# KittyMac/ponyc

Hardware: AMD Instinct MI355X
Metric: actor msgs/sec (node), message-ubench & ring (higher is better)
Workload: dtype u64; 1 GPU; message-ubench C2: 1,048,576 pingers per GPU x 5 initial pings, steady state; actors_per_gpu=1048576, actors_total=1048576, initial_pings=5, mailbox_cap=16, batch=100, parallelism=actor partition id % 1 over 1 rank(s), exchange=none

## Files before the change

### ponyc_amd/csrc/engine.hip

```cpp
#include <hip/hip_runtime.h>
#include <hip/hip_ext.h>
#include <hipcub/hipcub.hpp>
#include <rccl/rccl.h>

#include <algorithm>
#include <cstdio>
#include <cstdlib>
#include <cstring>
#include <atomic>
#include <condition_variable>
#include <map>
#include <mutex>
#include <new>
#include <thread>
#include <vector>

#include "../../include/gpu_actor_host.h"
#include "engine_dev.h"
#include "zone_dev.h"
#include "sparse_dev.h"
#include "hot_dev.h"
#include "step_entry.h"
#include "jit_host.h"
#include "dev_buf.h"
// ... 102 lines not shown

__global__ void __launch_bounds__(kLandThreads) k_spawn_land(const uint64_t* key, const uint64_t* arg,
  uint32_t n, const uint32_t* tstart, const unsigned long long* live, uint32_t cur)
{
  __shared__ uint32_t s_hist[kMaxZones];
  __shared__ uint32_t s_base[kMaxZones];
  LandRec r[kLandPer];
#pragma unroll
  for(int u = 0; u < kLandPer; ++u)
  {
    const uint64_t i = (uint64_t)blockIdx.x * kLandRecs + (uint64_t)u * kLandThreads + threadIdx.x;
    r[u].valid = false;
    if(i < n)
    {
      const uint64_t k = key[i];
      const uint32_t t = (uint32_t)(k >> 52);
      const TypeDev& T = c_types[t];
      const uint64_t slot = live[t] + (i - tstart[t]);
      if(slot < T.count)
      {
        r[u].valid = c_eng.nranks == 1 || (T.first + slot) % c_eng.nranks == c_eng.rank;
        r[u].to = T.first + (uint32_t)slot;
        r[u].w = (uint32_t)(((k >> 4) & 0xFFFFull) << 16) | (uint32_t)((k & 0xFu) << 12);
        r[u].from = (uint32_t)(k >> 20);
        r[u].arg = arg[i];
      }
      else if(c_eng.rank == 0)
        atomicAdd(&c_eng.stats[ST_DROPPED], 1ull);
    }
  }
  land_records(r, cur, s_hist, s_base);
}

__global__ void k_spawn_commit(const uint32_t* tcnt, unsigned long long* live)
{
  const uint32_t t = threadIdx.x;
  if(t >= GPU_ACTOR_MAX_TYPES || tcnt[t] == 0) return;
  const unsigned long long room = c_types[t].count - live[t];
  live[t] += tcnt[t] < room ? tcnt[t] : room;
}

__global__ void k_host_begin(uint64_t* step_word, uint64_t v)
{
  *step_word = v;
}

struct HostOff { uint32_t off[kHostShards + 1]; };
__global__ void __launch_bounds__(kBlock) k_host_compact(const uint64_t* key, HostOff o, uint32_t seg,
  uint64_t* key_out, uint32_t* idx_out)
{
  const uint32_t i = blockIdx.x * kBlock + threadIdx.x;
  if(i >= o.off[kHostShards]) return;
  uint32_t lo = 0, hi = kHostShards - 1;
  while(lo < hi)
  {
    const uint32_t mid = (lo + hi + 1) / 2;
    if(o.off[mid] <= i) lo = mid; else hi = mid - 1;
  }
  const uint32_t at = lo * seg + (i - o.off[lo]);
  key_out[i] = key[at];
  idx_out[i] = at;
}

__global__ void __launch_bounds__(kBlock) k_host_gather(const uint64_t* key, const uint32_t* idx,
  const uint4* rec, gpu_host_msg_t* out, uint32_t n, uint64_t base, uint32_t kshift)
{
  const uint32_t i = blockIdx.x * kBlock + threadIdx.x;
  if(i >= n) return;
  const uint64_t k = key[i];
  const uint4 r = rec[idx[i]];
  const uint64_t step = base + (k >> kshift);
  const uint32_t from = (uint32_t)((k & ((1ull << kshift) - 1ull)) >> 16);
  uint4* o = reinterpret_cast<uint4*>(out + i);
  o[0] = make_uint4((uint32_t)step, (uint32_t)(step >> 32), from, (uint32_t)(k & 0xFFFFull));
  o[1] = r;
}
static_assert(sizeof(gpu_host_msg_t) == 32, "gpu_host_msg_t is 32 B");

__global__ void k_host_lost(unsigned long long n)
{
  c_eng.stats[ST_DROPPED] += n;
}

__global__ void __launch_bounds__(kBlock) k_spill_need(const SpillRec* s, uint32_t n, uint32_t* need)
{
  const uint32_t i = blockIdx.x * kBlock + threadIdx.x;
  if(i >= n) return;
  atomicMax(&need[s[i].z], (s[i].tag & kSpillPosMask) + 1u);
}

__global__ void __launch_bounds__(kBlock) k_spill_place(const SpillRec* s, uint32_t n, uint32_t p)
{
  const uint32_t i = blockIdx.x * kBlock + threadIdx.x;
  if(i >= n) return;
  const SpillRec r = s[i];
  ZRec* base = (r.tag & kSpillCarry) ? c_eng.carry[p] : c_eng.land[p];
  base[c_eng.zoff[r.z] + (r.tag & kSpillPosMask)] = r.rec;
}

constexpr uint32_t kBigCopyCap = 4096;
constexpr uint32_t kBigCopyBlocks = 512;
__global__ void __launch_bounds__(kBlock) k_carry_big(uint32_t cur)
{
  const bool halt_now = c_eng.nranks == 1 ? (c_eng.spill_n[cur] != 0u || *c_eng.halt != 0u)
                                          : (*c_eng.spill_flag != 0u);
  if(halt_now) return;
  const unsigned long long v = c_eng.bigc_n[cur];
  const uint32_t n = min((uint32_t)(v >> 32), c_eng.bigc_cap);
  if(n == 0) return;
  const uint32_t total = c_eng.bigc[n - 1].base + c_eng.bigc[n - 1].rem;
  const uint32_t per = (total + gridDim.x - 1) / gridDim.x;
  const uint32_t c0 = blockIdx.x * per, c1 = min(c0 + per, total);
  if(c0 < c1)
  {
    uint32_t lo = 0, hi = n - 1;
    while(lo < hi)
    {
      const uint32_t mid = (lo + hi + 1) / 2;
      if(c_eng.bigc[mid].base <= c0) lo = mid; else hi = mid - 1;
    }
    for(uint32_t d = lo; d < n; ++d)
    {
      const BigCopy b = c_eng.bigc[d];
      if(b.base >= c1) break;
      const uint32_t j0 = c0 > b.base ? c0 - b.base : 0u;
      const uint32_t j1 = min(c1 - b.base, b.rem);
      for(uint32_t j = j0 + threadIdx.x; j < j1; j += kBlock)
      {
        const uint32_t k = b.from + j;
        const uint32_t q = k - b.ncc;
        const uint4 r = k < b.ncc ? *reinterpret_cast<const uint4*>(b.c + k)
                      : *reinterpret_cast<const uint4*>(b.p + (b.perm ? (uint32_t)(b.perm[q] & 0xFFFFFull) : q));
        *reinterpret_cast<uint4*>(b.dst + j) = r;
      }
    }
  }
}


namespace {

constexpr uint32_t kChunk = 16;
constexpr uint32_t kPendSlots = 4096;
constexpr uint32_t kPendPre = kPendSlots - 1;

struct HostType {
  bool registered = false, created = false;
  uint32_t words = 0, ht = 0, batch = 0, cap = 0;
  uint64_t params[GPU_ACTOR_MAX_PARAMS] = {};
  uint64_t first = 0, count = 0;
  uint32_t lfirst = 0, lcount = 0;
  uint64_t reserve = 0;
  int32_t priority = 0;
  DevBuf<uint64_t> d_state;
  DevBuf<uint64_t> d_prog;
  uint32_t prog_n = 0;
  bool prog_yields = false;
  std::vector<uint64_t> prog_host;
};

struct SpillStat {
  unsigned int spill_n[2];
  unsigned int halt;
  unsigned int pad;
  unsigned long long skipped;
};

struct HotLayout {
  size_t prep = 0;
  size_t slot = prep + kMaxZones;
  size_t cnt = slot + kMaxZones;
  size_t aux = cnt + (size_t)kMaxHot * kHotActors;
  size_t hist = aux + (size_t)kMaxHot * 3 * kHotActors;
  size_t bcnt = hist + kHotBins;
  size_t cur = bcnt + kHotBins;
  size_t bar = cur + kHotBins + kHotActors;
  size_t words = bar + 64;
};
constexpr HotLayout kHotLayout{};

struct Process {
  std::mutex mu;
  std::mutex wmu;
  std::thread worker;
  std::vector<std::thread> detached;
  std::atomic<bool> async_busy{false};
  std::atomic<bool> async_started{false};
  int async_rc = 0;
  uint64_t async_steps = 0;
  gpu_actor_alltoallv_fn xp_a2a = nullptr;
  gpu_actor_allreduce_fn xp_ar = nullptr;
  void* xp_ctx = nullptr;
};

struct Session {
  bool init = false;
  gpu_actor_config_t cfg{};
  int device = 0;
  hipStream_t stream = nullptr;
  HostType types[GPU_ACTOR_MAX_TYPES];
  uint32_t n_types = 0;
  uint64_t n_actors = 0;
  uint32_t n_local = 0;
  uint32_t n_zones = 0;
  uint64_t zone_records = 0;
  DevBuf<uint64_t> d_zoff;
  DevBuf<uint32_t> d_zcap;
  DevBuf<ZRec> d_land[2], d_carry[2];
  DevBuf<uint32_t> d_land_n[2], d_carry_n[2];
  DevBuf<ZRec> d_S;
  DevBuf<ORec> d_O;
  uint32_t par = 0;
  DevBuf<unsigned long long> d_stats;
  DevBuf<unsigned long long> d_pend;
  DevBuf<unsigned long long> d_pend_sh;
  DevBuf<unsigned long long> d_stats_sh;
  DevBuf<uint32_t> d_hot;
  bool hot_on = false;
  int hot_fits = -1;
  DevBuf<unsigned long long> d_dbg;
  PinBuf<gpu_msg_t> h_msgs;
  std::vector<gpu_msg_t> deferred;
  DevBuf<gpu_msg_t> d_msgs;
  uint64_t host_seq = 0;
  uint64_t steps_total = 0;
  int sticky = 0;
  jit::Module jit;
  uint64_t jit_set = 0;
  uint64_t jit_failed = 0;
  uint32_t jit_builds = 0;
  bool jit_used = false;
  TypeDev td_host[GPU_ACTOR_MAX_TYPES] = {};
  EngDev eng_host = {};
  bool consts_host = false;
  DevBuf<uint64_t> d_gups_list;
  DevBuf<unsigned int> d_gups_n;
  DevBuf<uint64_t> d_gups_jump;
  DevBuf<unsigned long long> d_gups_stat;
  uint64_t gups_jump_host[65] = {};
  int gups_type = -1;
  DevBuf<uint64_t> d_gups_send;
  DevBuf<uint64_t> d_gups_all;
  uint32_t gups_parts = 0;
  uint64_t gups_in_total = 0, gups_out_total = 0;
  uint64_t dev_epoch = 1, sstat_epoch = 0, sticky_epoch = 0;
  hipError_t last_hip = hipSuccess;
  std::vector<hipEvent_t> ev;
  double last_drain_ms = 0.0;
  ncclComm_t comm = nullptr;
  DevBuf<XRec> d_xout;
  DevBuf<XRec> d_xin;
  DevBuf<unsigned long long> d_xc;
  unsigned long long* d_xcount = nullptr;
  unsigned long long* d_xrecv = nullptr;
  PinBuf<unsigned long long> h_xc;
  DevBuf<unsigned int> d_spill_flag;
  uint32_t xcap = 0;
  DevBuf<XSpillRec> d_xspill;
  DevBuf<unsigned int> d_xspill_n;
  uint32_t xspill_cap = 0;
  std::vector<unsigned long long> h_xcount, h_xrecv;
  uint64_t remote_total = 0;
  bool peer_write = false;
  DevBuf<XRec> d_pin;
  XRec* peer_ptr[kMaxRanks] = {};
  DevBuf<unsigned long long> d_hx;
  PinBuf<uint8_t> h_sbuf, h_rbuf;
  uint32_t spawn_cap = 0;
  DevBuf<uint64_t> d_skey[2], d_sarg[2];
  DevBuf<unsigned int> d_spawn_n;
  DevBuf<uint32_t> d_tstart, d_tcnt;
  DevBuf<unsigned long long> d_live;
  DevBuf<uint8_t> d_sort_tmp;
  DevBuf<uint8_t> d_trig[2], d_trig_own[2];
  uint64_t trig_bytes = 0;
  bool trig_stale[2] = {false, false};
  DevBuf<uint32_t> d_muted_on;
  DevBuf<uint32_t> d_ztrig[2];
  DevBuf<unsigned int> d_trig_n;
  DevBuf<uint32_t> d_zplan;
  bool split_plan = true;
  bool fuse = true;
  uint32_t sidx = 0;
  DevBuf<BigCopy> d_bigc;
  DevBuf<unsigned long long> d_bigc_n;
  bool defer_big = false;
  DevBuf<SpillRec> d_spill[2];
  uint32_t spill_cap = 0;
  DevBuf<SpillStat> d_sstat;
  PinBuf<SpillStat> h_sstat;
  DevBuf<uint32_t> d_need;
  std::vector<uint32_t> zcap_min, zcap_host;
// ... 108 lines not shown
    (void)hipGetLastError();
    cached = 0;
    return false;
  }
  cached = (uint64_t)std::max(per_cu - 1, per_cu > 0 ? 1 : 0) * (uint64_t)cus >= kHotBlocks ? 1 : 0;
  return cached != 0;
}

constexpr uint32_t kGupsBlocks = 1024;
constexpr uint32_t kGupsPackBlocks = 256;
__global__ void __launch_bounds__(256) k_gups_apply();
__global__ void __launch_bounds__(256) k_gups_pack(uint64_t* out, unsigned long long* count);
__global__ void __launch_bounds__(256) k_gups_apply_ranks(const uint64_t* list, uint64_t n,
  uint64_t own_lo, uint64_t own_n);

int gups_setup(EngDev& e)
{
  g.gups_type = -1;
  e.gups_type = -1;
  const char* f = getenv("PONYC_AMD_GUPS_DEFER");
  if(f && atoi(f) == 0) return 0;
  int t_def = -1;
  for(uint32_t t = 0; t < GPU_ACTOR_MAX_TYPES && t_def < 0; ++t)
    if(g.types[t].created && g.types[t].ht == GPU_ACTOR_HT_GUPS_STREAMER && g.types[t].params[0] > 0 &&
       g.types[t].params[0] <= 0xFFFFFFFFull)
      t_def = (int)t;
  if(t_def < 0) return 0;
  const HostType& h = g.types[t_def];
  const uint64_t chunk = h.params[0];
  const uint64_t L = std::max<uint64_t>(16, (chunk + 63) / 64);
  const uint64_t parts = (chunk + L - 1) / L;
  const uint64_t cap = std::min<uint64_t>(std::max<uint64_t>(1ull << 22, 2ull * h.lcount), 1ull << 28);
  if(cap > g.d_gups_list.size())
  {
    HIPCK(hipStreamSynchronize(g.stream));
    HIPCK(g.d_gups_list.alloc(cap));
    g.d_gups_send.reset();
  }
  if(R() > 1 && !g.d_gups_send)
    HIPCK(g.d_gups_send.alloc(g.d_gups_list.size()));
  if(!g.d_gups_n)
  {
    HIPCK(g.d_gups_n.alloc(kGupsShards + 1));
    HIPCK(hipMemsetAsync(g.d_gups_n, 0, (kGupsShards + 1) * sizeof(unsigned int), g.stream));
    HIPCK(g.d_gups_jump.alloc(65));
    HIPCK(g.d_gups_stat.alloc(3 * kGupsBlocks));
    HIPCK(hipMemsetAsync(g.d_gups_stat, 0, 3 * kGupsBlocks * sizeof(unsigned long long), g.stream));
  }
  uint64_t jump[65] = {};
  for(uint64_t p = 0; p < parts; ++p) jump[p] = gpa::polyrand_xpow(p * L);
  jump[parts] = gpa::polyrand_xpow(chunk);
  if(memcmp(jump, g.gups_jump_host, sizeof(jump)) != 0)
  {
    HIPCK(hipStreamSynchronize(g.stream));
    memcpy(g.gups_jump_host, jump, sizeof(jump));
    HIPCK(hipMemcpyAsync(g.d_gups_jump, g.gups_jump_host, sizeof(jump), hipMemcpyHostToDevice,
      g.stream));
  }
  e.gups_list = g.d_gups_list; e.gups_n = g.d_gups_n; e.gups_jump = g.d_gups_jump;
  e.gups_stat = g.d_gups_stat;
  e.gups_seg = (uint32_t)(g.d_gups_list.size() / kGupsShards);
  {
    const char* sg = getenv("PONYC_AMD_GUPS_SEG");
    if(sg && atoi(sg) > 0) e.gups_seg = std::min<uint32_t>(e.gups_seg, (uint32_t)atoi(sg));
  }
  e.gups_l = (uint32_t)L; e.gups_parts = (uint32_t)parts;
  e.gups_type = t_def;
  g.gups_type = t_def;
  g.gups_parts = (uint32_t)parts;
  return 0;
}

int gups_apply_launch(hipEvent_t e1)
{
  if(g.gups_type < 0 || R() > 1) return 0;
  if(e1)
    hipExtLaunchKernelGGL(k_gups_apply, dim3(kGupsBlocks), dim3(256), 0, g.stream, nullptr, e1, 0u);
  else
    hipLaunchKernelGGL(k_gups_apply, dim3(kGupsBlocks), dim3(256), 0, g.stream);
  HIPCK(hipGetLastError());
  return 0;
}

int upload_types()
{
  TypeDev td[GPU_ACTOR_MAX_TYPES];
  memset(td, 0, sizeof(td));
  for(uint32_t t = 0; t < GPU_ACTOR_MAX_TYPES; ++t)
  {
    const HostType& h = g.types[t];
    TypeDev& d = td[t];
    if(!h.created) continue;
    d.first = (uint32_t)h.first; d.count = (uint32_t)h.count;
    d.lfirst = h.lfirst; d.lcount = h.lcount;
    d.ht = h.ht; d.words = h.words; d.batch = h.batch; d.cap = h.cap;
    d.reducible = reducible_ht(h.ht);
    d.prio = h.priority > 0 ? 1u : 0u;
    d.state = h.d_state;
    memcpy(d.params, h.params, sizeof(d.params));
    d.prog = h.d_prog;
    d.prog_n = h.prog_n;
    d.prog_pad = h.prog_yields ? 1u : 0u;
  }
  HIPCK(hipMemcpyToSymbolAsync(HIP_SYMBOL(c_types), td, sizeof(td), 0,
    hipMemcpyHostToDevice, g.stream));
  EngDev e;
  memset(&e, 0, sizeof(e));
  e.n_types = g.n_types; e.rank = rank(); e.nranks = R(); e.n_local = g.n_local;
  e.n_zones = g.n_zones; e.zoff = g.d_zoff; e.zcapz = g.d_zcap;
  e.n_ids = (uint32_t)std::min<uint64_t>(g.n_actors, 0xFFFFFFFFull);
  e.r_magic = R() > 1 ? ~0ull / R() + 1 : 0;
  for(int p = 0; p < 2; ++p)
  {
    e.land[p] = g.d_land[p]; e.carry[p] = g.d_carry[p];
    e.land_n[p] = g.d_land_n[p]; e.carry_n[p] = g.d_carry_n[p];
  }
  e.S = g.d_S; e.O = g.d_O;
  e.stats = g.d_stats; e.pend = g.d_pend;
  e.pend_sh = g.d_pend_sh; e.stats_sh = g.d_stats_sh;
  {
    uint32_t* h = g.d_hot;
    const HotLayout& L = kHotLayout;
    e.hot_prep = h + L.prep; e.hot_slot = h + L.slot; e.hot_cnt = h + L.cnt; e.hot_aux = h + L.aux;
    e.hot_hist = h + L.hist; e.hot_bcnt = h + L.bcnt; e.hot_cur = h + L.cur; e.hot_bar = h + L.bar;
  }
  e.xout = g.d_xout; e.xcount = g.d_xcount; e.xcap = g.xcap;
  e.peer_write = g.peer_write ? 1u : 0u;
  for(uint32_t p = 0; p < R() && p < kMaxRanks; ++p)
    e.xdst[p] = g.peer_write ? (g.peer_ptr[p] ? g.peer_ptr[p] + (size_t)rank() * g.xcap : nullptr)
                             : (g.d_xout ? g.d_xout + (size_t)p * g.xcap : nullptr);
  e.seq_max = R() > 1 ? kXSeqMax : kSeqMax;
  e.dbg = g.d_dbg;
  e.spawn_key = g.d_skey[0]; e.spawn_arg = g.d_sarg[0];
  e.spawn_n = g.d_spawn_n; e.spawn_cap = g.spawn_cap;
  for(int p = 0; p < 2; ++p)
  {
    e.trig[p] = g.d_trig[p];
    e.trig_own[p] = R() > 1 ? g.d_trig_own[p] : g.d_trig[p];
    e.ztrig[p] = g.d_ztrig[p];
  }
  e.muted_on = g.d_muted_on;
  e.spill_flag = g.d_spill_flag;
  e.trig_n = g.d_trig_n;
  e.spill[0] = g.d_spill[0]; e.spill[1] = g.d_spill[1];
  e.spill_n = g.d_sstat ? g.d_sstat->spill_n : nullptr;
  e.halt = g.d_sstat ? &g.d_sstat->halt : nullptr;
  e.skipped = g.d_sstat ? &g.d_sstat->skipped : nullptr;
  e.spill_cap = g.spill_cap;
  e.xspill = g.d_xspill; e.xspill_n = g.d_xspill_n; e.xspill_cap = g.xspill_cap;
  e.zbits = g.zbits;
  g.defer_big = defer_big_wanted();
  {
    const char* f = getenv("PONYC_AMD_HOT");
    g.hot_on = pick_step_entry().hot && (f ? atoi(f) != 0 : g.defer_big) && hot_resident();
    e.hot_on = g.hot_on ? 1u : 0u;
    const char* t = getenv("PONYC_AMD_HOT_TEST");
    e.hot_test = (t && atoi(t) != 0) ? 1u : 0u;
  }
  e.bigc = g.d_bigc; e.bigc_n = g.d_bigc_n; e.bigc_cap = kBigCopyCap;
  e.defer_big = g.defer_big ? 1u : 0u;
  {
    const char* f = getenv("PONYC_AMD_TWO_PASS");
    e.two_pass = (f && atoi(f) == 0) ? 0u : 1u;
    const char* sp = getenv("PONYC_AMD_SPLIT_PLAN");
    g.split_plan = !(sp && atoi(sp) == 0);
    const char* fu = getenv("PONYC_AMD_FUSE");
    g.fuse = !(fu && atoi(fu) == 0);
  }
  e.zplan = g.d_zplan;
  if(g.host_ports && g.host_seg)
  {
    uint64_t lo = ~0ull, hi = 0;
    for(uint32_t t = 0; t < GPU_ACTOR_MAX_TYPES; ++t)
    {
      const HostType& h = g.types[t];
      if(!h.created || h.ht != GPU_ACTOR_HT_HOST_PORT) continue;
      e.host_rng[e.host_nrng].first = (uint32_t)h.first;
      e.host_rng[e.host_nrng].count = (uint32_t)h.count;
      e.host_rng[e.host_nrng].type = t;
      e.host_nrng++;
      lo = std::min(lo, h.first);
      hi = std::max(hi, h.first + h.count);
    }
    e.host_first = e.host_nrng ? (uint32_t)lo : 0u;
    e.host_span = e.host_nrng ? (uint32_t)(hi - lo) : 0u;
    e.host_seg = g.host_seg;
    e.host_key = g.hl.d_host_key; e.host_rec = g.hl.d_host_rec; e.host_n = g.d_host_n;
    e.host_step = g.d_host_step;
  }
  {
    const int rc = gups_setup(e);
    if(rc) return rc;
  }
  HIPCK(hipMemcpyToSymbolAsync(HIP_SYMBOL(c_eng), &e, sizeof(e), 0,
    hipMemcpyHostToDevice, g.stream));
  for(const StepEntry& se : step_entries())
    HIPCK(se.upload(td, &e, g.stream));
  memcpy(g.td_host, td, sizeof(td));
  g.eng_host = e;
  g.consts_host = true;
  if(g.jit.mod)
  {
    HIPCK(hipMemcpyHtoDAsync(g.jit.types, g.td_host, sizeof(g.td_host), g.stream));
    HIPCK(hipMemcpyHtoDAsync(g.jit.eng, &g.eng_host, sizeof(g.eng_host), g.stream));
  }
  return 0;
}

int ensure_spill(uint64_t cap)
{
  cap = std::min<uint64_t>(cap, 0x7FFFFFFFull);
  if(cap <= g.spill_cap) return 0;
  g.spill_cap = 0;
  for(int p = 0; p < 2; ++p) HIPCK(g.d_spill[p].alloc(cap));
  g.spill_cap = (uint32_t)cap;
  return 0;
}

int relayout_zones(bool geometry = false);
StepEntry step_entry_for(bool z12);
bool step_fits(const StepEntry& se, uint64_t nb);
int upload_types();
int pend_read(uint32_t first, uint32_t n, std::vector<unsigned long long>& out);

inline uint64_t spill_cap_for_zones()
{
  return std::max<uint64_t>(1u << 20, g.zone_records / 4);
}

int read_sstat()
{
  HIPCK(hipMemcpyAsync(g.h_sstat, g.d_sstat, sizeof(SpillStat), hipMemcpyDeviceToHost,
    g.stream));
  HIPCK(hipStreamSynchronize(g.stream));
  g.sstat_epoch = g.dev_epoch;
  return 0;
}

inline bool spill_pending()
{
  return g.h_sstat->spill_n[0] || g.h_sstat->spill_n[1] || g.h_sstat->halt;
}

int fixup_spill()
{
  const SpillStat st = *g.h_sstat;
  g.dev_epoch++;
  if(R() == 1 && !st.spill_n[0] && !st.spill_n[1] && !st.halt) return 0;
  uint32_t n[2], most = 0;
  for(int p = 0; p < 2; ++p)
  {
    n[p] = std::min(st.spill_n[p], g.spill_cap);
    most = std::max(most, st.spill_n[p]);
  }
  if(n[0] || n[1])
  {
    const uint32_t nz = g.n_zones;
    HIPCK(hipMemsetAsync(g.d_need, 0, nz * sizeof(uint32_t), g.stream));
    for(int p = 0; p < 2; ++p)
      if(n[p])
        hipLaunchKernelGGL(k_spill_need, dim3(blocks_for(n[p])), dim3(kBlock), 0, g.stream,
          (const SpillRec*)g.d_spill[p], n[p], g.d_need);
    HIPCK(hipGetLastError());
    std::vector<uint32_t> need(nz);
    HIPCK(hipMemcpyAsync(need.data(), g.d_need, nz * sizeof(uint32_t), hipMemcpyDeviceToHost,
      g.stream));
    HIPCK(hipStreamSynchronize(g.stream));
    bool grow = false;
    for(uint32_t z = 0; z < nz; ++z)
      if(need[z] > g.zcap_host[z])
      {
        const uint64_t want = std::max<uint64_t>(2ull * g.zcap_host[z], need[z] + need[z] / 2);
        g.zcap_min[z] = (uint32_t)std::min<uint64_t>((want + 15) & ~15ull, kSpillPosMask);
        grow = true;
      }
    if(grow)
    {
      int rc = relayout_zones();
      if(rc) return rc;
      rc = upload_types();
      if(rc) return rc;
    }
    for(int p = 0; p < 2; ++p)
      if(n[p])
        hipLaunchKernelGGL(k_spill_place, dim3(blocks_for(n[p])), dim3(kBlock), 0, g.stream,
          (const SpillRec*)g.d_spill[p], n[p], (uint32_t)p);
    HIPCK(hipGetLastError());
  }
  HIPCK(hipMemsetAsync(g.d_sstat, 0, sizeof(SpillStat), g.stream));
  HIPCK(hipMemsetAsync(g.d_spill_flag, 0, sizeof(unsigned int), g.stream));
  HIPCK(hipStreamSynchronize(g.stream));
  memset(g.h_sstat, 0, sizeof(SpillStat));
  g.fixups++;
  const uint64_t want = std::max<uint64_t>(spill_cap_for_zones(),
                                           most > g.spill_cap ? 2ull * most : 0ull);
  if(want > g.spill_cap)
  {
    const int rc = ensure_spill(want);
    if(rc) return rc;
    return upload_types();
  }
  return 0;
}

uint32_t pick_zone_bits(uint64_t n)
{
  const uint64_t rb = R() > 1 ? R() : 0;
  const uint64_t nz11 = (n + 2047) / 2048, nz12 = (n + 4095) / 4096;
  if(const char* f = getenv("PONYC_AMD_ZONE_BITS"))
    return atoi(f) == 12 ? 12u : 11u;
  return (nz11 + rb > 640 && step_fits(step_entry_for(true), nz12 + rb)) ? 12u : 11u;
}

bool zones_empty()
{
  if(g.n_zones == 0) return true;
  std::vector<uint32_t> v(g.n_zones);
  for(int p = 0; p < 2; ++p)
    for(const uint32_t* src : {g.d_land_n[p].get(), g.d_carry_n[p].get()})
    {
      if(hipMemcpy(v.data(), src, g.n_zones * sizeof(uint32_t), hipMemcpyDeviceToHost) != hipSuccess)
        return false;
      for(uint32_t x : v)
        if(x) return false;
    }
  return true;
}

int relayout_zones(bool geometry)
{
  bool fresh = false;
  {
    const uint32_t want = pick_zone_bits((g.n_actors + R() - 1) / R());
    if(geometry && want != g.zbits && g.steps_total == 0 && g.sparse_launches == 0)
    {
      HIPCK(hipStreamSynchronize(g.stream));
      bool empty = zones_empty();
      if(R() > 1)
      {
        const unsigned long long mine = empty ? 0ull : 1ull;
        HIPCK(hipMemcpyAsync(g.d_pend + kPendPre, &mine, sizeof(mine), hipMemcpyHostToDevice,
          g.stream));
        std::vector<unsigned long long> pv;
        const int rc = pend_read(kPendPre, 1, pv);
        if(rc) return rc;
        empty = pv[0] == 0;
      }
      if(empty)
      {
        g.zbits = want;
        g.zcap_min.clear();
        fresh = true;
      }
    }
  }
  const uint32_t za = zone_actors();
  const uint32_t nz = (uint32_t)((g.n_local + za - 1) / za);
  if(nz > kMaxZones) return GPU_ACTOR_ERANGE;
  std::vector<uint64_t> cap64(nz, 0);
  for(const HostType& t : g.types)
  {
    if(!t.created || reducible_ht(t.ht)) continue;
    for(uint64_t L = t.lfirst; L < (uint64_t)t.lfirst + t.lcount; )
    {
      const uint64_t z = L / za;
      const uint64_t hi = std::min<uint64_t>((z + 1) * za, (uint64_t)t.lfirst + t.lcount);
      cap64[z] += (hi - L) * t.cap;
      L = hi;
    }
  }
  std::vector<uint32_t> cap(nz);
  std::vector<uint64_t> off(nz);
  uint64_t total = 0;
  if(g.zcap_min.size() < nz) g.zcap_min.resize(nz, 0);
  for(uint32_t z = 0; z < nz; ++z)
  {
    cap64[z] = std::max<uint64_t>(cap64[z], g.zcap_min[z]);
    if(cap64[z] > (uint64_t)kSpillPosMask) return GPU_ACTOR_ERANGE;
    cap[z] = (uint32_t)cap64[z];
    off[z] = total;
    total += (cap[z] + 15u) & ~15u;
  }
  const size_t recs = std::max<uint64_t>(total, 16), nzn = std::max<size_t>(nz, 1);
  DevBuf<uint64_t> d_off;
  DevBuf<uint32_t> d_cap, ln[2], cn[2], mo;
  DevBuf<ZRec> land[2], carry[2], S;
  DevBuf<ORec> O;
  HIPCK(d_off.alloc(nzn));
  HIPCK(d_cap.alloc(nzn));
  HIPCK(hipMemcpyAsync(d_off, off.data(), nz * sizeof(uint64_t), hipMemcpyHostToDevice, g.stream));
  HIPCK(hipMemcpyAsync(d_cap, cap.data(), nz * sizeof(uint32_t), hipMemcpyHostToDevice, g.stream));
  for(int p = 0; p < 2; ++p)
  {
    HIPCK(land[p].alloc(recs));
    HIPCK(carry[p].alloc(recs));
    HIPCK(ln[p].alloc(nzn));
    HIPCK(cn[p].alloc(nzn));
    HIPCK(hipMemsetAsync(ln[p], 0, nzn * sizeof(uint32_t), g.stream));
    HIPCK(hipMemsetAsync(cn[p], 0, nzn * sizeof(uint32_t), g.stream));
    if(g.n_zones && !fresh)
    {
      hipLaunchKernelGGL(k_zone_copy, dim3(g.n_zones), dim3(kBlock), 0, g.stream,
        (const ZRec*)g.d_land[p], g.d_zoff, g.d_zcap, land[p], (const uint64_t*)d_off);
      hipLaunchKernelGGL(k_zone_copy, dim3(g.n_zones), dim3(kBlock), 0, g.stream,
        (const ZRec*)g.d_carry[p], g.d_zoff, g.d_zcap, carry[p], (const uint64_t*)d_off);
      HIPCK(hipGetLastError());
      HIPCK(hipMemcpyAsync(ln[p], g.d_land_n[p], g.n_zones * sizeof(uint32_t),
        hipMemcpyDeviceToDevice, g.stream));
      HIPCK(hipMemcpyAsync(cn[p], g.d_carry_n[p], g.n_zones * sizeof(uint32_t),
        hipMemcpyDeviceToDevice, g.stream));
    }
    HIPCK(hipStreamSynchronize(g.stream));
  }
  HIPCK(S.alloc(3 * recs));
  HIPCK(O.alloc(recs));
  const uint64_t slots = (uint64_t)nz * za;
  if(slots > g.d_muted_on.size())
  {
    HIPCK(mo.alloc(slots));
    HIPCK(hipMemsetAsync(mo, 0, slots * sizeof(uint32_t), g.stream));
    if(g.d_muted_on)
    {
      HIPCK(hipMemcpyAsync(mo, g.d_muted_on, g.d_muted_on.size() * sizeof(uint32_t),
        hipMemcpyDeviceToDevice, g.stream));
      HIPCK(hipStreamSynchronize(g.stream));
    }
    g.d_muted_on.swap(mo);
  }
  for(int p = 0; p < 2; ++p)
  {
    g.d_land[p].swap(land[p]); g.d_carry[p].swap(carry[p]);
    g.d_land_n[p].swap(ln[p]); g.d_carry_n[p].swap(cn[p]);
  }
  g.d_S.swap(S);
  g.d_O.swap(O);
  g.d_zoff.swap(d_off);
  g.d_zcap.swap(d_cap);
  g.zone_records = total;
  g.n_zones = nz;
  g.zcap_host = cap;
  return 0;
}

uint32_t required_words(uint32_t ht)
{
  switch(ht)
  {
    case GPU_ACTOR_HT_RING: return 4;
    case GPU_ACTOR_HT_PINGER: return 3;
    case GPU_ACTOR_HT_PINGER_DET: return 2;
    case GPU_ACTOR_HT_FANIN_SENDER: return 4;
    case GPU_ACTOR_HT_FANIN_ANALYZER: return 2;
    case GPU_ACTOR_HT_GUPS_STREAMER: return 2;
    case GPU_ACTOR_HT_GUPS_UPDATER: return 1;
    case GPU_ACTOR_HT_STORM: return 2;
    case GPU_ACTOR_HT_FIFO_SRC: return 3;
    case GPU_ACTOR_HT_FIFO_SINK: return 11;
    case GPU_ACTOR_HT_SPREADER: return 5;
    case GPU_ACTOR_HT_PROGRAM: return 8;
    case GPU_ACTOR_HT_HOST_PORT: return 1;
    default: return 0;
  }
}

__global__ void __launch_bounds__(kBlock) k_fold(uint32_t first, uint32_t n)
{
  for(uint32_t s = first + threadIdx.x; s < first + n; s += kBlock)
  {
    unsigned long long* sh = c_eng.pend_sh + (size_t)s * kShards;
    unsigned long long v = 0;
    for(uint32_t k = 0; k < kShards; ++k) { v += sh[k]; sh[k] = 0; }
    if(v) c_eng.pend[s] += v;
  }
  for(uint32_t i = threadIdx.x; i < ST_COUNT; i += kBlock)
  {
    unsigned long long* sh = c_eng.stats_sh + (size_t)i * kShards;
    unsigned long long v = 0;
    for(uint32_t k = 0; k < kShards; ++k) { v += sh[k]; sh[k] = 0; }
    if(v) c_eng.stats[i] += v;
  }
}

int fold_counters(uint32_t first, uint32_t n)
{
  hipLaunchKernelGGL(k_fold, dim3(1), dim3(kBlock), 0, g.stream, first, n);
  HIPCK(hipGetLastError());
  return 0;
}

int pend_clear(uint32_t first, uint32_t n)
{
  HIPCK(hipMemsetAsync(g.d_pend + first, 0, n * sizeof(unsigned long long), g.stream));
  HIPCK(hipMemsetAsync(g.d_pend_sh + (size_t)first * kShards, 0,
    (size_t)n * kShards * sizeof(unsigned long long), g.stream));
  return 0;
}

void sticky_from(const unsigned long long* st)
{
  if(st[ST_DROPPED] || st[ST_XCHG_OVERFLOW]) g.sticky = GPU_ACTOR_EMAILBOX;
  else if(st[ST_SEQ_OVERFLOW]) g.sticky = GPU_ACTOR_ERANGE;
}

int check_sticky()
{
  if(R() == 1 && g.sticky_epoch == g.dev_epoch) return g.sticky;
  unsigned long long st[ST_COUNT];
  {
    const int rc = fold_counters(0, 0);
    if(rc) return rc;
  }
  HIPCK(hipMemcpyAsync(st, g.d_stats, sizeof(st), hipMemcpyDeviceToHost, g.stream));
  HIPCK(hipStreamSynchronize(g.stream));
  g.sticky_epoch = g.dev_epoch;
  sticky_from(st);
  return g.sticky;
}

__global__ void k_spill_flag(unsigned int* flag)
{
  *flag = c_eng.spill_n[0] + c_eng.spill_n[1];
}

__global__ void __launch_bounds__(256) k_gups_apply()
{
  __shared__ uint32_t s_pre[kGupsShards + 1];
  if(threadIdx.x < kGupsShards)
  {
    uint32_t c = min(__atomic_load_n(&c_eng.gups_n[threadIdx.x], __ATOMIC_RELAXED), c_eng.gups_seg);
    for(int off = 1; off < (int)kGupsShards; off <<= 1)
    {
      const uint32_t o = __shfl_up(c, off);
      if((int)threadIdx.x >= off) c += o;
    }
    s_pre[threadIdx.x + 1] = c;
    if(threadIdx.x == 0) s_pre[0] = 0;
  }
  __syncthreads();
  const uint32_t n = s_pre[kGupsShards];
  const TypeDev& S = c_types[c_eng.gups_type];
  const uint64_t chunk = S.params[0], shift = S.params[1], mask = S.params[2];
  const uint32_t ubase = (uint32_t)S.params[3];
  const uint32_t L = c_eng.gups_l, parts = c_eng.gups_parts, per_wave = 64u / parts;
  const uint32_t lane = threadIdx.x & 63u, sub = lane / parts, p = lane - sub * parts;
  const uint64_t jump = c_eng.gups_jump[p];
  const uint64_t first = (uint64_t)p * L;
  const uint32_t cnt = first < chunk ? (uint32_t)min<uint64_t>(L, chunk - first) : 0u;
  const uint64_t wave = (uint64_t)blockIdx.x * (blockDim.x >> 6) + (threadIdx.x >> 6);
  const uint64_t waves = (uint64_t)gridDim.x * (blockDim.x >> 6);
  uint32_t u_first = 0, u_count = 0, u_lfirst = 0, u_lcount = 0;
  uint64_t* u_state = nullptr;
  uint64_t u_mask = 0;
  uint32_t made = 0, issued = 0;
  for(uint64_t e0 = wave * per_wave; e0 < n; e0 += waves * per_wave)
  {
    const uint64_t e = e0 + sub;
    const bool live = sub < per_wave && e < n;
    uint64_t v = 0;
    if(live)
    {
      uint32_t lo = 0, hi = kGupsShards;
      while(hi - lo > 1u)
      {
        const uint32_t mid = (lo + hi) >> 1;
        if(s_pre[mid] <= e) lo = mid; else hi = mid;
      }
      v = c_eng.gups_list[(size_t)lo * c_eng.gups_seg + (e - s_pre[lo])];
    }
    if(live && p) v = polyrand_mulmod(v, jump);
    for(uint32_t j = 0; j < L; ++j)
    {
      unsigned long long* w = nullptr;
      if(live && j < cnt)
      {
        (void)polyrand_next(v);
        ++made;
        const uint32_t to = ubase + (uint32_t)((v >> shift) & mask);
        if(to - u_first >= u_count)
        {
          const int t = type_of_global(to);
          if(t >= 0)
          {
            const TypeDev& U = c_types[t];
            u_first = U.first; u_count = U.count; u_lfirst = U.lfirst; u_lcount = U.lcount;
            u_state = U.state; u_mask = U.params[0] - 1;
          }
        }
        if(to - u_first < u_count)
          w = reinterpret_cast<unsigned long long*>(&u_state[(v & u_mask) * u_lcount + (to - u_lfirst)]);
      }
      const uint64_t wa = reinterpret_cast<uint64_t>(w);
      uint64_t left = __ballot(w != nullptr);
      for(int round = 0; round < 2 && left; ++round)
      {
        const uint32_t lead = (uint32_t)__ffsll((long long)left) - 1u;
        const uint64_t lw = __shfl(wa, (int)lead);
        const uint64_t peers = __ballot(((left >> lane) & 1ull) && wa == lw);
        uint64_t r = ((peers >> lane) & 1ull) ? v : 0ull;
        if(__popcll(peers) > 1)
          for(int off = 32; off; off >>= 1) r ^= __shfl_xor(r, off);
        if(lane == lead && r != 0)
        {
          atomicXor(w, (unsigned long long)r);
          ++issued;
// ... 72 lines not shown
  const uint64_t first = (uint64_t)p * L;
  const uint32_t cnt = first < chunk ? (uint32_t)min<uint64_t>(L, chunk - first) : 0u;
  const uint64_t wave = (uint64_t)blockIdx.x * (blockDim.x >> 6) + (threadIdx.x >> 6);
  const uint64_t waves = (uint64_t)gridDim.x * (blockDim.x >> 6);
  uint32_t u_first = 0, u_count = 0, u_lfirst = 0, u_lcount = 0;
  uint64_t* u_state = nullptr;
  uint64_t u_mask = 0;
  uint32_t made = 0, issued = 0, far = 0;
  for(uint64_t e0 = wave * per_wave; e0 < n; e0 += waves * per_wave)
  {
    const uint64_t e = e0 + sub;
    const bool live = sub < per_wave && e < n;
    const uint32_t peer = e - own_lo >= own_n ? 1u : 0u;
    uint64_t v = live ? list[e] : 0ull;
    if(live && p) v = polyrand_mulmod(v, jump);
    for(uint32_t j = 0; j < L; ++j)
    {
      unsigned long long* w = nullptr;
      if(live && j < cnt)
      {
        (void)polyrand_next(v);
        const uint32_t to = ubase + (uint32_t)((v >> shift) & mask);
        if(!is_remote(to))
        {
          ++made;
          far += peer;
          if(to - u_first >= u_count)
          {
            const int t = type_of_global(to);
            if(t >= 0)
            {
              const TypeDev& U = c_types[t];
              u_first = U.first; u_count = U.count; u_lfirst = U.lfirst; u_lcount = U.lcount;
              u_state = U.state; u_mask = U.params[0] - 1;
            }
          }
          if(to - u_first < u_count)
            w = reinterpret_cast<unsigned long long*>(
              &u_state[(v & u_mask) * u_lcount + (rdiv(to) - u_lfirst)]);
        }
      }
      const uint64_t wa = reinterpret_cast<uint64_t>(w);
      uint64_t left = __ballot(w != nullptr);
      for(int round = 0; round < 2 && left; ++round)
      {
        const uint32_t lead = (uint32_t)__ffsll((long long)left) - 1u;
        const uint64_t lw = __shfl(wa, (int)lead);
        const uint64_t peers = __ballot(((left >> lane) & 1ull) && wa == lw);
        uint64_t r = ((peers >> lane) & 1ull) ? v : 0ull;
        if(__popcll(peers) > 1)
          for(int off = 32; off; off >>= 1) r ^= __shfl_xor(r, off);
        if(lane == lead && r != 0)
        {
          atomicXor(w, (unsigned long long)r);
          ++issued;
        }
        left &= ~peers;
      }
      if(((left >> lane) & 1ull) && v != 0)
      {
        atomicXor(w, (unsigned long long)v);
        ++issued;
      }
    }
  }
  __shared__ uint32_t s_sum[3];
  if(threadIdx.x < 3) s_sum[threadIdx.x] = 0;
  __syncthreads();
  if(made) atomicAdd(&s_sum[0], made);
  if(issued) atomicAdd(&s_sum[1], issued);
  if(far) atomicAdd(&s_sum[2], far);
  __syncthreads();
  if(threadIdx.x == 0)
  {
    c_eng.gups_stat[blockIdx.x] += s_sum[0];
    c_eng.gups_stat[kGupsBlocks + blockIdx.x] += s_sum[1];
    c_eng.gups_stat[2 * kGupsBlocks + blockIdx.x] += s_sum[2];
  }
}

__global__ void k_spill_local(unsigned long long* out)
{
  *out = (unsigned long long)c_eng.spill_n[0] + c_eng.spill_n[1] + *c_eng.halt +
         (c_eng.nranks > 1 ? *c_eng.spill_flag : 0u);
}

__global__ void k_xprep()
{
  const unsigned int xs = *c_eng.xspill_n;
  if(xs <= c_eng.xspill_cap) return;
  const uint32_t p = threadIdx.x;
  if(p < c_eng.nranks)
    c_eng.xcount[p] = min(c_eng.xcount[p], (unsigned long long)c_eng.xcap);
  if(p == 0) atomicAdd(&c_eng.stats[ST_XCHG_OVERFLOW], (unsigned long long)c_eng.xspill_cap);
}

__global__ void __launch_bounds__(kBlock) k_xspill_place(uint32_t n)
{
  const uint32_t i = blockIdx.x * kBlock + threadIdx.x;
  if(i >= n) return;
  const XSpillRec r = c_eng.xspill[i];
  xrec_put(c_eng.xdst[r.peer] + r.pos, r.rec);
}

int alloc_xspill(uint32_t cap)
{
  g.xspill_cap = 0;
  HIPCK(g.d_xspill.alloc(cap));
  g.xspill_cap = cap;
  return 0;
}

int peer_room(uint64_t max_send, uint64_t xs);
int exchange_room(uint64_t max_send, uint64_t total_recv, uint64_t xs)
{
  if(g.peer_write) return peer_room(max_send, xs);
  const bool lost = xs > g.xspill_cap;
  if(max_send > g.xcap || lost)
  {
    uint64_t cap = std::max<uint64_t>(2ull * g.xcap, max_send + max_send / 2);
    cap = std::min<uint64_t>((cap + 63) & ~63ull, 0x40000000ull);
    DevBuf<XRec> nx;
    HIPCK(nx.alloc((size_t)R() * cap));
    HIPCK(hipMemcpy2DAsync(nx, cap * sizeof(XRec), g.d_xout, (size_t)g.xcap * sizeof(XRec),
      (size_t)g.xcap * sizeof(XRec), R(), hipMemcpyDeviceToDevice, g.stream));
    HIPCK(hipStreamSynchronize(g.stream));
    g.d_xout = std::move(nx);
    g.xcap = (uint32_t)cap;
    const int rc = upload_types();
    if(rc) return rc;
  }
  if(xs)
  {
    if(!lost)
    {
      hipLaunchKernelGGL(k_xspill_place, dim3(blocks_for(xs)), dim3(kBlock), 0, g.stream,
        (uint32_t)xs);
      HIPCK(hipGetLastError());
    }
    HIPCK(hipMemsetAsync(g.d_xspill_n, 0, sizeof(unsigned int), g.stream));
    if(xs > g.xspill_cap / 2)
    {
      HIPCK(hipStreamSynchronize(g.stream));
      const int rc = alloc_xspill((uint32_t)std::min<uint64_t>(4ull * std::max<uint64_t>(xs,
        g.xspill_cap), 1ull << 27));
      if(rc) return rc;
      const int rc2 = upload_types();
      if(rc2) return rc2;
    }
  }
  if(total_recv > g.d_xin.size())
  {
    const uint64_t cap = std::max<uint64_t>(2ull * g.d_xin.size(), total_recv + total_recv / 2);
    HIPCK(hipStreamSynchronize(g.stream));
    HIPCK(g.d_xin.alloc(cap));
  }
  return 0;
}

enum XcType { XC_U8 = 0, XC_U32 = 1, XC_U64 = 2 };

int stage_room(uint64_t sbytes, uint64_t rbytes)
{
  if(sbytes > g.h_sbuf.size()) HIPCK(g.h_sbuf.alloc(std::max<uint64_t>(sbytes, 2 * g.h_sbuf.size())));
  if(rbytes > g.h_rbuf.size()) HIPCK(g.h_rbuf.alloc(std::max<uint64_t>(rbytes, 2 * g.h_rbuf.size())));
  return 0;
}
// ... 554 lines not shown
  HIPCK(hipMemsetAsync(g.d_host_n, 0, kHostShards * sizeof(unsigned int), g.stream));
  HIPCK(hipStreamSynchronize(g.stream));
  if(g.host_fn)
    g.host_fn(g.host_ctx, g.hl.h_host_out, keep);
  else
  {
    if(g.hostq_head == g.hostq.size()) { g.hostq.clear(); g.hostq_head = 0; }
    try { g.hostq.insert(g.hostq.end(), g.hl.h_host_out.get(), g.hl.h_host_out + keep); }
    catch(...) { return GPU_ACTOR_ENOMEM; }
  }
  return 0;
}

int step_after_launch(uint32_t slot, hipEvent_t e0, hipEvent_t e1);
int jit_ensure(const StepEntry& se)
{
  const char* f = getenv("PONYC_AMD_JIT");
  if((f && atoi(f) == 0) || !g.consts_host) return 0;
  const bool z12 = g.zbits == 12;
  std::vector<jit::Prog> progs;
  uint32_t mask = 0;
  bool all_prog = true;
  for(uint32_t t = 0; t < GPU_ACTOR_MAX_TYPES; ++t)
  {
    const HostType& h = g.types[t];
    if(!h.created || reducible_ht(h.ht)) continue;
    mask |= 1u << h.ht;
    if(h.ht != GPU_ACTOR_HT_PROGRAM || h.prog_host.empty()) all_prog = false;
    else progs.push_back({t, h.prog_host});
  }
  int kind = 0;
  uint64_t want = jit::fnv1a(z12 ? "z12" : "z11");
  if(all_prog && !progs.empty() && g.split_plan)
  {
    kind = 1;
    for(const jit::Prog& p : progs)
      want = jit::fnv1a(std::string(reinterpret_cast<const char*>(p.code.data()), p.code.size() * 8),
                        jit::fnv1a(std::to_string(p.type), want));
  }
  else if(se.kernel == step_entry_for_any(z12).kernel && mask)
  {
    kind = 2;
    want = jit::fnv1a("mix" + std::to_string(mask), want);
  }
  if(!kind) return 0;
  if(g.jit.mod && g.jit_set == want) return kind;
  if(g.jit_failed == want) return 0;
  jit::unload(g.jit);
  hipDeviceProp_t prop;
  if(hipGetDeviceProperties(&prop, g.device) != hipSuccess) { (void)hipGetLastError(); return 0; }
  std::string arch = prop.gcnArchName;
  arch = arch.substr(0, arch.find(':'));
  std::string log;
  const int rc = kind == 1 ? jit::build(progs, z12, arch, g.jit, log)
                           : jit::build_mix(mask, z12, arch, g.jit, log);
  if(getenv("PONYC_AMD_JIT_LOG"))
    fprintf(stderr, "gpu_actor jit: %s %s%s (rc %d) %s\n", kind == 1 ? "programs" : "mix",
            kind == 2 ? ("mask " + std::to_string(mask) + " ").c_str() : "", z12 ? "z12" : "z11", rc,
            log.c_str());
  if(rc != 0)
  {
    g.jit_failed = want;
    return 0;
  }
  g.jit_set = want;
  g.jit_builds++;
  if(hipMemcpyHtoDAsync(g.jit.types, g.td_host, sizeof(g.td_host), g.stream) != hipSuccess ||
     hipMemcpyHtoDAsync(g.jit.eng, &g.eng_host, sizeof(g.eng_host), g.stream) != hipSuccess)
  {
    (void)hipGetLastError();
    jit::unload(g.jit);
    g.jit_failed = want;
    return 0;
  }
  return kind;
}

int launch_step(uint32_t slot, hipEvent_t e0, hipEvent_t e1)
{
  if(g.n_zones == 0) return 0;
  g.dev_epoch++;
  const StepEntry se = pick_step_entry();
  if(se.stub) return GPU_ACTOR_EINVAL;
  const uint64_t nb = g.n_zones + (R() > 1 ? R() : 0);
  if(!step_fits(se, nb)) return GPU_ACTOR_ERANGE;
  const size_t dyn = step_dyn_bytes(se, nb);
  if(g.host_ports)
  {
    if(!g.host_seg) return GPU_ACTOR_ENOMEM;
    if(!g.host_dirty) { g.host_base = g.sidx; g.host_dirty = true; }
    hipLaunchKernelGGL(k_host_begin, dim3(1), dim3(1), 0, g.stream, g.d_host_step,
      (uint64_t)(g.sidx - g.host_base) << g.host_kshift);
    HIPCK(hipGetLastError());
  }
  g.jit_used = false;
  const int jk = jit_ensure(se);
  if(jk && g.jit.static_lds + dyn <= kLdsPerWorkgroup)
  {
    g.jit_used = true;
    uint32_t a_cur = g.par, a_slot = slot, a_sidx = g.sidx;
    void* args[] = {&a_cur, &a_slot, &a_sidx};
    if(e0) HIPCK(hipEventRecord(e0, g.stream));
    if(jk == 2 && g.hot_on)
      hipLaunchKernelGGL(k_hot, dim3(kHotBlocks), dim3(kHotThreads), 5u * zone_actors() * sizeof(uint32_t),
        g.stream, g.par, g.sidx);
    HIPCK(hipModuleLaunchKernel(g.jit.plan, g.n_zones, 1, 1, se.threads, 1, 1, (unsigned)dyn, g.stream,
      args, nullptr));
    if(jk == 1)
      HIPCK(hipModuleLaunchKernel(g.jit.rest, g.n_zones, 1, 1, se.threads, 1, 1, (unsigned)dyn, g.stream,
        args, nullptr));
    if(g.defer_big)
      hipLaunchKernelGGL(k_carry_big, dim3(kBigCopyBlocks), dim3(kBlock), 0, g.stream, g.par);
    const int grc = gups_apply_launch(nullptr);
    if(grc) return grc;
    if(e1 && !(g.gups_type >= 0 && R() > 1)) HIPCK(hipEventRecord(e1, g.stream));
    return step_after_launch(slot, e0, e1);
  }
  const bool fused = se.plan && g.split_plan && g.fuse && se.fused;
  const bool split = se.plan && g.split_plan && !fused;
  step_kernel_t kern = fused ? se.fused : split ? se.plan : se.kernel;
  const size_t hot_lds = 5u * zone_actors() * sizeof(uint32_t);
  if(e0)
  {
    const bool gups = g.gups_type >= 0;
    const bool more = split || g.defer_big || gups;
    if(g.hot_on)
      hipExtLaunchKernelGGL(k_hot, dim3(kHotBlocks), dim3(kHotThreads), (uint32_t)hot_lds, g.stream,
        e0, nullptr, 0u, g.par, g.sidx);
    hipExtLaunchKernelGGL(kern, dim3(g.n_zones), dim3(se.threads), (uint32_t)dyn, g.stream,
      g.hot_on ? nullptr : e0, more ? nullptr : e1, 0u, g.par, slot, g.sidx);
    if(split)
      hipExtLaunchKernelGGL(se.rest, dim3(g.n_zones), dim3(se.threads), (uint32_t)dyn, g.stream,
        nullptr, (g.defer_big || gups) ? nullptr : e1, 0u, g.par, slot, g.sidx);
    if(g.defer_big)
      hipExtLaunchKernelGGL(k_carry_big, dim3(kBigCopyBlocks), dim3(kBlock), 0, g.stream,
        nullptr, gups ? nullptr : e1, 0u, g.par);
    HIPCK(hipGetLastError());
    const int grc = gups_apply_launch(e1);
    if(grc) return grc;
  }
  else
  {
    if(g.hot_on)
      hipLaunchKernelGGL(k_hot, dim3(kHotBlocks), dim3(kHotThreads), hot_lds, g.stream, g.par, g.sidx);
    hipLaunchKernelGGL(kern, dim3(g.n_zones), dim3(se.threads), dyn, g.stream, g.par, slot, g.sidx);
    if(split)
      hipLaunchKernelGGL(se.rest, dim3(g.n_zones), dim3(se.threads), dyn, g.stream, g.par, slot, g.sidx);
    if(g.defer_big)
      hipLaunchKernelGGL(k_carry_big, dim3(kBigCopyBlocks), dim3(kBlock), 0, g.stream, g.par);
    HIPCK(hipGetLastError());
    const int grc = gups_apply_launch(nullptr);
    if(grc) return grc;
  }
  HIPCK(hipGetLastError());
  return step_after_launch(slot, e0, e1);
}

int gups_gather_apply(hipEvent_t e1)
{
  const uint32_t n = R();
  const unsigned long long* cnt = g.h_xc + 2 * n + 3;
  std::vector<uint64_t> off(n);
  uint64_t total = 0;
  for(uint32_t p = 0; p < n; ++p)
  {
    off[p] = total;
// ... 563 lines not shown
  const unsigned long long live_ull = live;
  HIPCK(hipMemcpyAsync(g.d_live + type_id, &live_ull, sizeof(live_ull), hipMemcpyHostToDevice,
    g.stream));
  if(t.reserve)
  {
    HIPCK(hipStreamSynchronize(g.stream));
    const uint32_t cap = g.spawn_cap + (uint32_t)t.reserve;
    for(int p = 0; p < 2; ++p)
    {
      HIPCK(g.d_skey[p].alloc((size_t)cap * R()));
      HIPCK(g.d_sarg[p].alloc((size_t)cap * R()));
    }
    g.spawn_cap = cap;
    rc = upload_types();
    if(rc) return rc;
  }
  HIPCK(hipStreamSynchronize(g.stream));
  if(first_id) *first_id = t.first;
  return 0;
}

GPU_ACTOR_API int gpu_actor_type_reserve(uint32_t type_id, uint64_t n)
{
  std::lock_guard<std::mutex> lk(gp.mu);
  if(!g.init) return GPU_ACTOR_ESTATE;
  if(type_id >= GPU_ACTOR_MAX_TYPES || !g.types[type_id].registered ||
    g.types[type_id].created) return GPU_ACTOR_EINVAL;
  if(n > g.cfg.max_actors) return GPU_ACTOR_ERANGE;
  g.types[type_id].reserve = n;
  return 0;
}

GPU_ACTOR_API int gpu_actor_type_live(uint32_t type_id, uint64_t* live)
{
  std::lock_guard<std::mutex> lk(gp.mu);
  if(!g.init) return GPU_ACTOR_ESTATE;
  if(type_id >= GPU_ACTOR_MAX_TYPES || !live || !g.types[type_id].created)
    return GPU_ACTOR_EINVAL;
  unsigned long long v = 0;
  HIPCK(hipMemcpyAsync(&v, g.d_live + type_id, sizeof(v), hipMemcpyDeviceToHost, g.stream));
  HIPCK(hipStreamSynchronize(g.stream));
  *live = v;
  return 0;
}

GPU_ACTOR_API int gpu_actor_alloc_msgs(uint64_t n, gpu_msg_t** buf)
{
  std::lock_guard<std::mutex> lk(gp.mu);
  if(!g.init) return GPU_ACTOR_ESTATE;
  if(!buf) return GPU_ACTOR_EINVAL;
  if(n > g.h_msgs.size()) HIPCK(g.h_msgs.alloc(n));
  *buf = g.h_msgs;
  return 0;
}

GPU_ACTOR_API int gpu_actor_sendv(const gpu_msg_t* first, uint64_t n)
{
  std::lock_guard<std::mutex> lk(gp.mu);
  if(!g.init) return GPU_ACTOR_ESTATE;
  return sendv_locked(first, n);
}

GPU_ACTOR_API int gpu_actor_send(uint64_t to, uint32_t behaviour, uint64_t arg)
{
  std::lock_guard<std::mutex> lk(gp.mu);
  if(!g.init) return GPU_ACTOR_ESTATE;
  gpu_msg_t m;
  m.to = (uint32_t)to; m.behaviour = behaviour; m.arg = arg;
  if(to >= g.n_actors || !host_msg_ok(m)) return GPU_ACTOR_EINVAL;
  if(g.host_seq + g.deferred.size() + 1 >= (1ull << 40)) return GPU_ACTOR_ERANGE;
  try { g.deferred.push_back(m); } catch(...) { return GPU_ACTOR_ENOMEM; }
  return 0;
}

bool sparse_ok()
{
  const char* e = getenv("GPA_NO_SPARSE");
  return !(e && atoi(e) != 0) && R() == 1 && g.spawn_cap == 0 && g.n_zones > 0 && !g.host_ports;
}

int run_sparse(uint64_t max_steps, SparseCtl& out)
{
  g.dev_epoch++;
  bool prog = false, gups = false;
  for(const HostType& t : g.types)
  {
    prog |= t.created && t.ht == GPU_ACTOR_HT_PROGRAM;
    gups |= t.created && t.ht == GPU_ACTOR_HT_GUPS_STREAMER;
  }
#define GPA_SPARSE_LAUNCH(P, G)                                                         \
  hipLaunchKernelGGL((k_sparse<P, G>), dim3(1), dim3(kSpThreads), 0, g.stream, g.par,   \
    (unsigned long long)max_steps, g.d_ctl, g.sidx)
  if(prog && gups) GPA_SPARSE_LAUNCH(true, true);
  else if(prog) GPA_SPARSE_LAUNCH(true, false);
  else if(gups) GPA_SPARSE_LAUNCH(false, true);
  else GPA_SPARSE_LAUNCH(false, false);
#undef GPA_SPARSE_LAUNCH
  HIPCK(hipGetLastError());
  {
    const int rc = gups_apply_launch(nullptr);
    if(rc) return rc;
  }
  HIPCK(hipMemcpyAsync(g.h_ctl, g.d_ctl, sizeof(SparseCtl), hipMemcpyDeviceToHost, g.stream));
  HIPCK(hipMemcpyAsync(g.h_sstat, g.d_sstat, sizeof(SpillStat), hipMemcpyDeviceToHost,
    g.stream));
  HIPCK(hipStreamSynchronize(g.stream));
  out = *g.h_ctl;
  g.par = out.par;
  g.sidx += (uint32_t)out.steps;
  g.sparse_launches++;
  g.sparse_steps += out.steps;
  return 0;
}

int pending_now(unsigned long long& out)
{
  int rc = pend_clear(kPendPre, 1);
  if(rc) return rc;
  rc = launch_pending(kPendPre);
  if(rc) return rc;
  std::vector<unsigned long long> pv;
  rc = pend_read(kPendPre, 1, pv);
  if(rc) return rc;
  out = pv[0];
  return 0;
}

int settle_spills()
{
  if(R() == 1)
  {
    if(g.sstat_epoch == g.dev_epoch) return spill_pending() ? fixup_spill() : 0;
    const int rc = read_sstat();
    if(rc) return rc;
    return spill_pending() ? fixup_spill() : 0;
  }
  hipLaunchKernelGGL(k_spill_local, dim3(1), dim3(1), 0, g.stream, g.d_pend + kPendPre);
  HIPCK(hipGetLastError());
  HIPCK(hipMemcpyAsync(g.h_sstat, g.d_sstat, sizeof(SpillStat), hipMemcpyDeviceToHost,
    g.stream));
  std::vector<unsigned long long> pv;
  const int rc = pend_read(kPendPre, 1, pv);
  if(rc) return rc;
  return pv[0] ? fixup_spill() : 0;
}

int run_locked(uint64_t max_steps, uint64_t* steps_done)
{
  if(!g.init) return GPU_ACTOR_ESTATE;
  {
    const int frc = observe();
    if(frc) return frc;
  }
  uint64_t done = 0;
  if(g.n_zones)
  {
    int rc = settle_spills();
    if(rc) return rc;
    unsigned long long before = 0;
    rc = pending_now(before);
    if(rc) return rc;
    std::vector<unsigned long long> pv;
    std::vector<uint32_t> par_at(kChunk + 1), sidx_at(kChunk + 1);
    const bool sp = sparse_ok();
    while(before > 0 && (max_steps == 0 || done < max_steps))
    {
// ... 352 lines not shown
  rc = host_alloc();
  if(rc)
  {
    g.host_reserve = old;
    if(host_alloc() != 0)
    {
      (void)upload_types();
      return GPU_ACTOR_ENOMEM;
    }
  }
  const int urc = upload_types();
  return rc ? rc : urc;
}

GPU_ACTOR_API int gpu_actor_recv(gpu_host_msg_t* out, uint64_t cap, uint64_t* n)
{
  std::lock_guard<std::mutex> lk(gp.mu);
  if(!g.init) return GPU_ACTOR_ESTATE;
  if(!n || (cap && !out)) return GPU_ACTOR_EINVAL;
  *n = 0;
  const int rc = observe();
  if(rc) return rc;
  const uint64_t k = std::min<uint64_t>(cap, g.hostq.size() - g.hostq_head);
  if(k) memcpy(out, g.hostq.data() + g.hostq_head, k * sizeof(gpu_host_msg_t));
  g.hostq_head += k;
  if(g.hostq_head == g.hostq.size())
  {
    g.hostq.clear();
    g.hostq_head = 0;
  }
  *n = k;
  return 0;
}

GPU_ACTOR_API int gpu_actor_recv_pending(uint64_t* n)
{
  std::lock_guard<std::mutex> lk(gp.mu);
  if(!g.init) return GPU_ACTOR_ESTATE;
  if(!n) return GPU_ACTOR_EINVAL;
  *n = 0;
  const int rc = observe();
  if(rc) return rc;
  *n = g.hostq.size() - g.hostq_head;
  return 0;
}

GPU_ACTOR_API int gpu_actor_host_notify(gpu_actor_host_fn fn, void* ctx)
{
  std::lock_guard<std::mutex> lk(gp.mu);
  if(!g.init) return GPU_ACTOR_ESTATE;
  g.host_fn = fn;
  g.host_ctx = fn ? ctx : nullptr;
  return 0;
}

GPU_ACTOR_API int gpu_actor_debug_info(uint64_t* out, uint64_t n)
{
  std::lock_guard<std::mutex> lk(gp.mu);
  if(!g.init || !out) return GPU_ACTOR_ESTATE;
  unsigned int tn[3] = {0, 0, 0};
  if(g.d_trig_n)
  {
    HIPCK(hipMemcpyAsync(tn, g.d_trig_n, sizeof(tn), hipMemcpyDeviceToHost, g.stream));
    HIPCK(hipStreamSynchronize(g.stream));
  }
  uint32_t hb[4] = {0, 0, 0, 0};
  if(g.d_hot)
  {
    HIPCK(hipMemcpyAsync(hb, hot_bar_words(), sizeof(hb), hipMemcpyDeviceToHost, g.stream));
    HIPCK(hipStreamSynchronize(g.stream));
  }
  uint64_t gu[3] = {0, 0, 0};
  {
    const int rc = gups_stat_read(gu);
    if(rc) return rc;
  }
  unsigned long long st[ST_COUNT];
  {
    const int rc = fold_counters(0, 0);
    if(rc) return rc;
  }
  HIPCK(hipMemcpyAsync(st, g.d_stats, sizeof(st), hipMemcpyDeviceToHost, g.stream));
  HIPCK(hipStreamSynchronize(g.stream));
  const uint64_t v[21] = {g.fixups, g.sparse_launches, g.sparse_steps, g.zone_records, g.spill_cap,
                          g.n_zones, tn[0], tn[1], tn[2], g.zbits, hb[3], g.hot_on ? 1u : 0u,
                          g.jit_used ? 1u : 0u, g.jit_builds, gu[0], gu[1], g.peer_write ? 1u : 0u,
                          g.gups_in_total, g.gups_out_total, gu[2], st[ST_PLAN_ZONES]};
  for(uint64_t i = 0; i < n && i < 21; ++i) out[i] = v[i];
  return 0;
}

GPU_ACTOR_API void gpu_actor_debug_live_buffers(uint64_t out[2])
{
  if(!out) return;
  out[0] = buf_live.count.load();
  out[1] = buf_live.bytes.load();
}

GPU_ACTOR_API int gpu_actor_debug_jit_compile(const uint32_t* types, const uint64_t* words,
  const uint32_t* lens, uint32_t nprog, int z12, const char* arch)
{
  if(!types || !words || !lens || nprog == 0 || nprog > GPU_ACTOR_MAX_TYPES) return GPU_ACTOR_EINVAL;
  std::vector<jit::Prog> progs;
  uint64_t off = 0;
  for(uint32_t k = 0; k < nprog; ++k)
  {
    if(lens[k] <= GPU_ACTOR_PROG_ENTRIES || lens[k] > jit::kMaxWords) return GPU_ACTOR_EINVAL;
    progs.push_back({types[k], std::vector<uint64_t>(words + off, words + off + lens[k])});
    off += lens[k];
  }
  const std::string src = jit::unit_source(progs, z12 != 0);
  const std::string a = arch && *arch ? arch : "gfx950";
  std::string log;
  const std::string co = jit::code_object(src, a, jit::key_of(src, a), log);
  if(co.empty())
  {
    fprintf(stderr, "gpu_actor jit: %s\n", log.c_str());
    return GPU_ACTOR_EINVAL;
  }
  return 0;
}

GPU_ACTOR_API int64_t gpu_actor_debug_jit_source(const uint32_t* types, const uint64_t* words,
  const uint32_t* lens, uint32_t nprog, int z12, char* buf, uint64_t cap)
{
  if(!types || !words || !lens || nprog == 0 || nprog > GPU_ACTOR_MAX_TYPES) return GPU_ACTOR_EINVAL;
  std::vector<jit::Prog> progs;
  uint64_t off = 0;
  for(uint32_t k = 0; k < nprog; ++k)
  {
    if(lens[k] <= GPU_ACTOR_PROG_ENTRIES || lens[k] > jit::kMaxWords) return GPU_ACTOR_EINVAL;
    progs.push_back({types[k], std::vector<uint64_t>(words + off, words + off + lens[k])});
    off += lens[k];
  }
  const std::string src = jit::unit_source(progs, z12 != 0);
  if(buf && src.size() < cap) memcpy(buf, src.c_str(), src.size() + 1);
  return (int64_t)src.size();
}

GPU_ACTOR_API int gpu_actor_debug_jit_compile_mix(uint32_t mask, int z12, const char* arch)
{
  if(mask == 0) return GPU_ACTOR_EINVAL;
  const std::string src = jit::mix_source(mask, z12 != 0);
  const std::string a = arch && *arch ? arch : "gfx950";
  std::string log;
  if(jit::code_object(src, a, jit::key_of(src, a), log).empty())
  {
    fprintf(stderr, "gpu_actor jit: %s\n", log.c_str());
    return GPU_ACTOR_EINVAL;
  }
  return 0;
}

GPU_ACTOR_API int gpu_actor_debug_stamps(uint64_t* out, uint64_t n)
{
  std::lock_guard<std::mutex> lk(gp.mu);
  if(!g.init || !out) return GPU_ACTOR_ESTATE;
  n = std::min<uint64_t>(n, (uint64_t)kMaxZones * kDbgSlots);
  HIPCK(hipMemcpyAsync(out, g.d_dbg, n * sizeof(uint64_t), hipMemcpyDeviceToHost, g.stream));
  HIPCK(hipStreamSynchronize(g.stream));
  return 0;
}

GPU_ACTOR_API int gpu_actor_debug_rccl_selftest(uint64_t* out, uint64_t n)
{
  std::lock_guard<std::mutex> lk(gp.mu);
  if(!g.init || !out || n < 23) return GPU_ACTOR_EINVAL;
  if(R() != 1 || g.comm || gp.xp_ar || gp.xp_a2a) return GPU_ACTOR_ESTATE;
  ncclComm_t comm = nullptr;
  int dev = g.device;
  NCCLCK(ncclCommInitAll(&comm, 1, &dev));
// ... 45 lines not shown
```

### ponyc_amd/csrc/engine_dev.h

```cpp
#pragma once
#ifndef __HIPCC_RTC__
#include <hip/hip_runtime.h>
#endif
#include <stdint.h>
#ifdef __HIPCC_RTC__
#include "gpu_actor.h"
#else
#include "../../include/gpu_actor.h"
#endif
#include "rng_dev.h"

namespace gpa {

constexpr int      kBlock = 256;
constexpr int      kWaves = kBlock / 64;
#ifndef GPA_ZONE_BITS
#define GPA_ZONE_BITS 11
#endif
#ifndef GPA_ZONE_THREADS
#define GPA_ZONE_THREADS 512
#endif
constexpr int      kZoneBits = GPA_ZONE_BITS;
static_assert(kZoneBits <= 12, "to_local is 12 bits of a ZRec's w0");
constexpr uint32_t kZone = 1u << kZoneBits;
constexpr uint32_t kZoneMask = kZone - 1;
constexpr int      kZoneThreads = GPA_ZONE_THREADS;
constexpr int      kZoneWaves = kZoneThreads / 64;
constexpr uint32_t kMaxZones = 4096;
constexpr uint32_t kMaxRanks = 64;
constexpr uint32_t kHostFrom = 0xFF000000u;
constexpr uint32_t kSeqMax = 0xFFFEu;
constexpr uint32_t kSeqApply = 0xFFFFu;
constexpr uint32_t kFanLds = 256;
constexpr uint32_t kDbgSlots = 24;

enum Stat : int {
  ST_DELIVERED = 0, ST_SENT = 1, ST_DROPPED = 2, ST_REMOTE_OUT = 3, ST_REMOTE_IN = 4,
  ST_SEQ_OVERFLOW = 5, ST_XCHG_OVERFLOW = 6, ST_ACTIVE = 7,
  ST_ATOMICS = 8,
  ST_PLAN_ZONES = 9,
  ST_BY_TYPE = 16, ST_COUNT = 32
};

struct ZRec {
  uint32_t w0;
  uint32_t from;
  uint64_t arg;
};

struct ORec {
  uint32_t to;
  uint32_t w;
  uint64_t arg;
};

struct XRec {
  uint32_t w0;
  uint32_t w1;
  uint64_t arg;
};
struct SpillRec {
  ZRec     rec;
  uint32_t z;
  uint32_t tag;
  uint32_t pad[2];
};
static_assert(sizeof(SpillRec) == 32, "SpillRec is 32 B");
constexpr uint32_t kSpillCarry = 1u << 30;
constexpr uint32_t kSpillPosMask = kSpillCarry - 1;
constexpr unsigned long long kPendSkipped = ~0ull;

constexpr uint32_t kXSeqApply = 0x3FFFu;
constexpr uint32_t kXSeqMax = 0x3FFEu;
static_assert(sizeof(XRec) == 16, "XRec is 16 B");
struct XSpillRec {
  XRec     rec;
  uint32_t peer;
  uint32_t pos;
  uint32_t pad[2];
};
static_assert(sizeof(XSpillRec) == 32, "XSpillRec is 32 B");

__device__ __forceinline__ uint64_t zkey(const ZRec& r)
{
  return ((uint64_t)r.from << 16) | (r.w0 >> 16);
}

struct TypeDev {
  uint32_t first, count;
  uint32_t lfirst, lcount;
  uint32_t ht, words, batch, cap;
  uint32_t reducible, prio;
  uint64_t* state;
  uint64_t  params[GPU_ACTOR_MAX_PARAMS];
  const uint64_t* prog;
  uint32_t  prog_n, prog_pad;
};

struct BigCopy {
  const ZRec* c;
  const ZRec* p;
  ZRec* dst;
  const uint64_t* perm;
  uint32_t ncc, from, rem, base;
};
static_assert(sizeof(BigCopy) == 48, "BigCopy is 48 B");

struct EngDev {
  uint32_t n_types, rank, nranks, n_local;
  uint32_t n_zones;
  uint32_t n_ids;
  uint64_t r_magic;
  const uint64_t* zoff;
  const uint32_t* zcapz;
  ZRec* land[2];
  ZRec* carry[2];
  uint32_t* land_n[2];
  uint32_t* carry_n[2];
  ZRec* S;
  ORec* O;
  unsigned long long* stats;
  unsigned long long* pend;
  XRec*  xout;
  unsigned long long* xcount;
  uint32_t xcap;
  uint32_t seq_max;
  unsigned long long* dbg;
  uint64_t* spawn_key;
  uint64_t* spawn_arg;
  unsigned int* spawn_n;
  uint32_t spawn_cap, pad3;
  uint8_t* trig[2];
  uint8_t* trig_own[2];
  uint32_t* muted_on;
  unsigned int* spill_flag;
  uint32_t* ztrig[2];
  unsigned int* trig_n;
  SpillRec* spill[2];
  unsigned int* spill_n;
  unsigned int* halt;
  unsigned long long* skipped;
  uint32_t spill_cap, pad4;
  XSpillRec* xspill;
  unsigned int* xspill_n;
  uint32_t xspill_cap, pad5;
  uint32_t zbits, pad6;
  BigCopy* bigc;
  unsigned long long* bigc_n;
  uint32_t bigc_cap, defer_big;
  uint32_t two_pass, pad7;
  uint32_t* zplan;
  unsigned long long* pend_sh;
  unsigned long long* stats_sh;
  uint32_t hot_on, hot_test;
  uint32_t* hot_prep;
  uint32_t* hot_slot;
  uint32_t* hot_cnt;
  uint32_t* hot_aux;
  uint32_t* hot_hist;
  uint32_t* hot_bcnt;
  uint32_t* hot_cur;
  uint32_t* hot_bar;
  uint64_t* gups_list;
  unsigned int* gups_n;
  const uint64_t* gups_jump;
  unsigned long long* gups_stat;
  uint32_t gups_seg, gups_l, gups_parts;
  int32_t gups_type;
  XRec* xdst[kMaxRanks];
  uint32_t peer_write, pad9;
  uint32_t host_first, host_span;
  uint32_t host_nrng, host_seg;
  struct HostRng { uint32_t first, count, type, pad; } host_rng[GPU_ACTOR_MAX_TYPES];
  uint64_t* host_key;
  uint4* host_rec;
  unsigned int* host_n;
  const uint64_t* host_step;
};
constexpr uint32_t kHostShards = 64;
constexpr uint32_t kGupsShards = 64;
constexpr uint32_t kShards = 32;
constexpr uint32_t kHotMin = 32768;


__constant__ TypeDev c_types[GPU_ACTOR_MAX_TYPES];
__constant__ EngDev  c_eng;

__device__ __forceinline__ uint32_t rdiv(uint32_t x)
{
  return c_eng.nranks == 1 ? x : (uint32_t)__umul64hi(c_eng.r_magic, (uint64_t)x);
}

__device__ __forceinline__ uint32_t rmod(uint32_t x)
{
  return x - rdiv(x) * c_eng.nranks;
}

__device__ __forceinline__ int type_of_local(uint32_t L)
{
  for(uint32_t t = 0; t < c_eng.n_types; ++t)
    if(L - c_types[t].lfirst < c_types[t].lcount) return (int)t;
  return -1;
}

__device__ __forceinline__ int type_of_global(uint32_t id)
{
  for(uint32_t t = 0; t < c_eng.n_types; ++t)
    if(id - c_types[t].first < c_types[t].count) return (int)t;
  return -1;
}

__device__ __forceinline__ uint32_t zone_capacity(uint32_t z)
{
  return c_eng.zcapz[z];
}

__device__ __forceinline__ uint32_t zone_cap_s(uint32_t z)
{
  return __builtin_amdgcn_readfirstlane(c_eng.zcapz[z]);
}

__device__ __forceinline__ uint64_t zone_off_s(uint32_t z)
{
  const uint64_t o = c_eng.zoff[z];
  return ((uint64_t)__builtin_amdgcn_readfirstlane((uint32_t)(o >> 32)) << 32) |
         __builtin_amdgcn_readfirstlane((uint32_t)o);
}

__device__ __forceinline__ uint32_t zone_of_local(uint32_t L) { return L >> c_eng.zbits; }
__device__ __forceinline__ uint32_t slot_in_zone(uint32_t L) { return L & ((1u << c_eng.zbits) - 1u); }

__device__ __forceinline__ uint32_t bucket_of(uint32_t to)
{
  const uint32_t R = c_eng.nranks;
  if(R > 1)
  {
    const uint32_t owner = rmod(to);
    if(owner != c_eng.rank) return c_eng.n_zones + owner;
  }
  return zone_of_local(rdiv(to));
}

__device__ __forceinline__ XRec xpack(uint32_t to, uint32_t w, uint32_t from, uint64_t arg)
{
  const uint32_t seq = (w >> 16) == kSeqApply ? kXSeqApply : (w >> 16);
  XRec x;
  x.w0 = (seq >> 9) << 27 | ((w >> 12) & 0xFu) << 23 | rdiv(to);
  x.w1 = (seq & 0x1FFu) << 23 | rdiv(from);
  x.arg = arg;
  return x;
}

struct ActorBase {
  uint32_t self;
  uint32_t li;
  uint32_t src_local;
  uint32_t seq;
  uint32_t sent;
  uint32_t applied;
  int      applied_type;
  int      type;
// ... 43 lines not shown
  const uint32_t li = rdiv(to) - T.lfirst;
  switch(T.ht)
  {
    case GPU_ACTOR_HT_FANIN_ANALYZER:
      atomicAdd(reinterpret_cast<unsigned long long*>(&T.state[li]), 1ull);
      atomicXor(reinterpret_cast<unsigned long long*>(&T.state[(size_t)T.lcount + li]),
        (unsigned long long)arg);
      break;
    case GPU_ACTOR_HT_GUPS_UPDATER: {
      const uint64_t k = arg & (T.params[0] - 1);
      if(arg != 0)
        atomicXor(reinterpret_cast<unsigned long long*>(&T.state[k * T.lcount + li]),
          (unsigned long long)arg);
      break;
    }
    default:
      break;
  }
  (void)beh;
}

__device__ __forceinline__ void pend_add_z(uint32_t slot, uint32_t z, unsigned long long v)
{
  atomicAdd(&c_eng.pend_sh[(size_t)slot * kShards + (z & (kShards - 1u))], v);
}
__device__ __forceinline__ void stat_add_z(int idx, uint32_t z, unsigned long long v)
{
  atomicAdd(&c_eng.stats_sh[(size_t)idx * kShards + (z & (kShards - 1u))], v);
}

__device__ __forceinline__ void spill_rec(uint32_t p, uint32_t kind, uint32_t z, uint32_t pos,
  const uint4& v)
{
  const unsigned int i = atomicAdd(&c_eng.spill_n[p], 1u);
  if(i < c_eng.spill_cap)
  {
    uint32_t* d = reinterpret_cast<uint32_t*>(c_eng.spill[p] + i);
    *reinterpret_cast<uint4*>(d) = v;
    *reinterpret_cast<uint4*>(d + 4) = make_uint4(z, pos | kind, 0u, 0u);
  }
  else
    atomicAdd(&c_eng.stats[ST_DROPPED], 1ull);
}

__device__ __forceinline__ void xrec_put(XRec* d, const XRec& x)
{
  if(c_eng.peer_write)
  {
    uint64_t* q = reinterpret_cast<uint64_t*>(d);
    __hip_atomic_store(q, (uint64_t)x.w1 << 32 | x.w0, __ATOMIC_RELAXED, __HIP_MEMORY_SCOPE_SYSTEM);
    __hip_atomic_store(q + 1, x.arg, __ATOMIC_RELAXED, __HIP_MEMORY_SCOPE_SYSTEM);
  }
  else
    *d = x;
}

__device__ __forceinline__ XRec xrec_get(const XRec* s)
{
  if(!c_eng.peer_write) return *s;
  const uint64_t* q = reinterpret_cast<const uint64_t*>(s);
  const uint64_t a = __hip_atomic_load(q, __ATOMIC_RELAXED, __HIP_MEMORY_SCOPE_SYSTEM);
  XRec x;
  x.w0 = (uint32_t)a;
  x.w1 = (uint32_t)(a >> 32);
  x.arg = __hip_atomic_load(q + 1, __ATOMIC_RELAXED, __HIP_MEMORY_SCOPE_SYSTEM);
  return x;
}

__device__ __forceinline__ uint32_t xout_store(uint32_t peer, uint32_t pos, const XRec& x)
{
  if(pos < c_eng.xcap)
  {
    xrec_put(c_eng.xdst[peer] + pos, x);
    return 0;
  }
  const unsigned int i = atomicAdd(c_eng.xspill_n, 1u);
  if(i >= c_eng.xspill_cap) return 1;
  uint32_t* d = reinterpret_cast<uint32_t*>(c_eng.xspill + i);
  *reinterpret_cast<uint4*>(d) = make_uint4(x.w0, x.w1, (uint32_t)x.arg, (uint32_t)(x.arg >> 32));
  *reinterpret_cast<uint4*>(d + 4) = make_uint4(peer, pos, 0u, 0u);
  return 0;
}

__device__ __forceinline__ void land_store(uint32_t p, uint32_t z, uint32_t pos, const uint4& v)
{
  if(pos < zone_capacity(z))
    *reinterpret_cast<uint4*>(c_eng.land[p] + c_eng.zoff[z] + pos) = v;
  else
    spill_rec(p, 0u, z, pos, v);
}

__device__ __forceinline__ void send_direct(uint32_t nxt, uint32_t self, uint32_t to, uint32_t w, uint64_t arg)
{
  const uint32_t R = c_eng.nranks;
  const uint32_t nz = c_eng.n_zones;
  const uint32_t b = bucket_of(to);
  if(b < nz)
  {
    const uint32_t pos = atomicAdd(&c_eng.land_n[nxt][b], 1u);
    uint4 v;
    v.x = w | slot_in_zone(rdiv(to));
    v.y = self;
    v.z = (uint32_t)arg;
    v.w = (uint32_t)(arg >> 32);
    land_store(nxt, b, pos, v);
  }
  else
  {
    const unsigned long long pos = atomicAdd(&c_eng.xcount[b - nz], 1ull);
    if(pos > 0x3FFFFFFFull || xout_store(b - nz, (uint32_t)pos, xpack(to, w, self, arg)))
      atomicAdd(&c_eng.stats[ST_XCHG_OVERFLOW], 1ull);
  }
}

__device__ __forceinline__ void outbox_put(ZoneCtx& a, uint32_t to, uint32_t w, uint64_t arg)
{
  const uint32_t idx = atomicAdd(a.s_nout, 1u);
  if(idx >= a.ocap)
  {
    send_direct(a.nxt, a.self, to, w, arg);
    return;
  }
  ORec r;
  r.to = to; r.w = w | a.src_local; r.arg = arg;
  *reinterpret_cast<uint4*>(a.out + idx) = *reinterpret_cast<const uint4*>(&r);
  atomicAdd(&a.s_hist[bucket_of(to)], 1u);
}

template <class A>
__device__ __forceinline__ void send_serial(A& a, uint32_t to, uint32_t beh, uint64_t arg)
{
  a.sent++;
  if constexpr(!A::kPlain)
    if(a.seq >= c_eng.seq_max)
    {
      atomicAdd(&c_eng.stats[ST_SEQ_OVERFLOW], 1ull);
      return;
    }
  a.put(to, (a.seq << 16) | (beh << 12), arg);
  a.seq++;
  if constexpr(!A::kPlain)
    if(a.trig && !a.prev_o && !a.mute_hit && to != a.self && a.trig[to] != 0)
    {
      a.mute_hit = 1;
      a.mute_to = to;
    }
}

template <class A>
__device__ __forceinline__ void actor_yield(A& a)
{
  a.yield_req = 1;
}

template <class A>
__device__ __forceinline__ void spawn_actor(A& a, uint32_t type, uint32_t beh, uint64_t arg)
{
  a.sent++;
  if(a.seq >= c_eng.seq_max)
  {
    atomicAdd(&c_eng.stats[ST_SEQ_OVERFLOW], 1ull);
    return;
  }
  const unsigned int pos = atomicAdd(c_eng.spawn_n, 1u);
  if(pos < c_eng.spawn_cap)
  {
    c_eng.spawn_key[pos] = ((uint64_t)type << 52) | ((uint64_t)a.self << 20) |
                           ((uint64_t)a.seq << 4) | (beh & 0xFu);
    c_eng.spawn_arg[pos] = arg;
  }
  else
    atomicAdd(&c_eng.stats[ST_DROPPED], 1ull);
  a.seq++;
}

__device__ __forceinline__ bool is_remote(uint32_t to)
{
  return c_eng.nranks > 1 && rmod(to) != c_eng.rank;
}

template <class A>
__device__ __forceinline__ bool send_host(A& a, uint32_t to, uint32_t beh, uint64_t arg)
// ... 424 lines not shown
```

### ponyc_amd/csrc/sparse_dev.h

```cpp
#pragma once
#include "engine_dev.h"

namespace gpa {

constexpr int kSpThreads = 1024;
constexpr int kSpWaves = kSpThreads / 64;
#ifndef GPA_SP_CAP
#define GPA_SP_CAP 1024
#endif
constexpr uint32_t kSpCap = GPA_SP_CAP;

enum SpReason : uint32_t { SP_QUIESCENT = 0, SP_MAX_STEPS = 1, SP_DENSE = 2 };

struct SparseCtl {
  unsigned long long steps;
  unsigned long long pending;
  uint32_t reason;
  uint32_t par;
};

struct SpList {
  uint64_t* K;
  uint32_t* W;
  uint64_t* A;
};

__shared__ uint32_t sp_cnt[2];

static_assert(kSpCap <= 1024, "packed rank counts hold 10-bit fields");
static_assert(kSpCap <= kSpThreads, "one record per thread in the distinct-receiver check");
constexpr uint32_t kSpHashBits = 13;
constexpr uint32_t kSpHash = 1u << kSpHashBits;

constexpr uint32_t kSpNoRun = 1u;
struct SpType {
  uint32_t lfirst, lcount, batch, flags;
};

__device__ __forceinline__ int sp_type(const SpType* ti, uint32_t n_types, uint32_t L)
{
  for(uint32_t t = 0; t < n_types; ++t)
    if(L - ti[t].lfirst < ti[t].lcount) return (int)t;
  return -1;
}

struct SparseCtx : ActorBase {
  static constexpr bool kHostPorts = false;
  SpList nx;
  uint32_t q;
  uint32_t* s_over;
  uint32_t nxt;
  __device__ __forceinline__ void put(uint32_t to, uint32_t w, uint64_t arg)
  {
    const uint32_t i = atomicAdd(&sp_cnt[__builtin_amdgcn_readfirstlane(q)], 1u);
    if(i < kSpCap)
    {
      nx.K[i] = ((uint64_t)rdiv(to) << 32) | self; nx.W[i] = w; nx.A[i] = arg;
    }
    else
    {
      *s_over = 1u;
      send_direct(nxt, self, to, w, arg);
    }
  }
};

__device__ void sp_land(const SpList& l, uint32_t n, uint32_t p)
{
  for(uint32_t i = threadIdx.x; i < n; i += kSpThreads)
  {
    const uint32_t L = (uint32_t)(l.K[i] >> 32);
    const uint32_t z = zone_of_local(L);
    const uint32_t pos = atomicAdd(&c_eng.land_n[p][z], 1u);
    uint4 v;
    v.x = l.W[i] | slot_in_zone(L);
    v.y = (uint32_t)l.K[i];
    v.z = (uint32_t)l.A[i];
    v.w = (uint32_t)(l.A[i] >> 32);
    land_store(p, z, pos, v);
  }
}

template <int HT>
__device__ __forceinline__ void sp_drain(const TypeDev& T, SparseCtx& a, const SpList& s,
  uint32_t i, uint32_t g)
{
  constexpr int NW = HT_Words<HT>::W;
  uint64_t st[NW];
#pragma unroll
  for(int k = 0; k < NW; ++k) st[k] = T.state[(size_t)k * T.lcount + a.li];
  for(uint32_t k = 0; k < g; ++k)
    handle(HtTag<HT>{}, T, a, st, (s.W[i + k] >> 12) & 0xFu, s.A[i + k]);
#pragma unroll
  for(int k = 0; k < NW; ++k) T.state[(size_t)k * T.lcount + a.li] = st[k];
}

template <bool kProg, bool kGups>
__device__ __forceinline__ void sp_dispatch(const TypeDev& Tref, SparseCtx& a, const SpList& S,
  uint32_t i, uint32_t g, uint32_t L)
{
  const TypeDev T = Tref;
  a.li = L - T.lfirst;
  switch(T.ht)
  {
#define SPCASE(HT) case HT: sp_drain<HT>(T, a, S, i, g); break;
    SPCASE(GPU_ACTOR_HT_RING)
    SPCASE(GPU_ACTOR_HT_PINGER)
    SPCASE(GPU_ACTOR_HT_PINGER_DET)
    SPCASE(GPU_ACTOR_HT_FANIN_SENDER)
    case GPU_ACTOR_HT_GUPS_STREAMER:
      if constexpr(kGups) sp_drain<GPU_ACTOR_HT_GUPS_STREAMER>(T, a, S, i, g);
      break;
    SPCASE(GPU_ACTOR_HT_STORM)
    SPCASE(GPU_ACTOR_HT_FIFO_SRC)
    SPCASE(GPU_ACTOR_HT_FIFO_SINK)
    case GPU_ACTOR_HT_PROGRAM:
      if constexpr(kProg) sp_drain<GPU_ACTOR_HT_PROGRAM>(T, a, S, i, g);
      break;
#undef SPCASE
    default: break;
  }
}

__device__ __forceinline__ uint32_t sp_block_excl_scan(uint32_t v, uint32_t* s_tmp, uint32_t& total)
{
  const uint32_t lane = threadIdx.x & 63, wv = threadIdx.x >> 6;
  uint32_t incl = v;
#pragma unroll
  for(int off = 1; off < 64; off <<= 1)
  {
    const uint32_t u = (uint32_t)__shfl_up((int)incl, off);
    if(lane >= (uint32_t)off) incl += u;
  }
  if(lane == 63) s_tmp[wv] = incl;
  __syncthreads();
  uint32_t base = 0, tot = 0;
  for(int w = 0; w < kSpWaves; ++w)
  {
    const uint32_t x = s_tmp[w];
    if(w < (int)wv) base += x;
    tot += x;
  }
  __syncthreads();
  total = tot;
  return base + incl - v;
}

template <bool kProg, bool kGups>
__global__ void __launch_bounds__(kSpThreads) k_sparse(uint32_t cur, unsigned long long max_steps,
  SparseCtl* ctl, uint32_t sidx)
{
  __shared__ uint64_t bK[3][kSpCap], bA[3][kSpCap];
  __shared__ uint32_t bW[3][kSpCap];
  __shared__ uint32_t s_zpre[kMaxZones + 1];
  __shared__ uint32_t s_tmp[kSpWaves];
  __shared__ uint32_t s_over;
  __shared__ uint32_t s_acc[kSpThreads];
  __shared__ SpType s_tinfo[GPU_ACTOR_MAX_TYPES];
  __shared__ uint32_t s_hcnt[kSpHash];
  __shared__ unsigned long long s_agg[kSpWaves];
  __shared__ unsigned long long s_bytype[GPU_ACTOR_MAX_TYPES];
  __shared__ unsigned long long s_red[kSpWaves][4];

  const uint32_t tid = threadIdx.x, lane = tid & 63, wv = tid >> 6;
  const uint32_t nz = c_eng.n_zones;
  const uint32_t n_types = c_eng.n_types;
  if(tid < GPU_ACTOR_MAX_TYPES)
  {
    s_bytype[tid] = 0;
    const TypeDev& T = c_types[tid];
    s_tinfo[tid].lfirst = T.lfirst;
    s_tinfo[tid].lcount = T.lcount;
    s_tinfo[tid].batch = T.batch;
    s_tinfo[tid].flags = (T.reducible || T.ht == GPU_ACTOR_HT_SPREADER ||
                          (T.ht == GPU_ACTOR_HT_PROGRAM && (!kProg || (T.prog_pad & 1u))) ||
                          (T.ht == GPU_ACTOR_HT_GUPS_STREAMER && !kGups) ||
                          (T.ht == GPU_ACTOR_HT_FIFO_SINK && T.params[1] != 0)) ? kSpNoRun : 0u;
  }
  if(tid == 0) { sp_cnt[0] = 0; sp_cnt[1] = 0; s_over = 0; }
  s_acc[tid] = 0;
  for(uint32_t h = tid; h < kSpHash; h += kSpThreads) s_hcnt[h] = 0;

  const uint32_t per = (nz + kSpThreads - 1) / kSpThreads;
  const uint32_t z0 = min(tid * per, nz), z1 = min(z0 + per, nz);
  uint32_t mine = 0;
  int carried = 0;
  for(uint32_t z = z0; z < z1; ++z)
  {
    const uint32_t c = min(c_eng.land_n[cur][z], zone_capacity(z));
    s_zpre[z] = c;
    mine += c;
    carried |= c_eng.carry_n[cur][z] != 0u;
  }
  uint32_t total = 0;
  uint32_t run = sp_block_excl_scan(mine, s_tmp, total);
  for(uint32_t z = z0; z < z1; ++z) { const uint32_t c = s_zpre[z]; s_zpre[z] = run; run += c; }
  if(tid == 0) s_zpre[nz] = total;
  const bool pending_fixup = c_eng.spill_n[cur] != 0u || *c_eng.halt != 0u ||
                             c_eng.trig_n[sidx % 3u] != 0u;
  if(__syncthreads_or(carried) || total > kSpCap || pending_fixup)
  {
    if(tid == 0)
    {
      ctl->steps = 0; ctl->pending = total; ctl->reason = SP_DENSE; ctl->par = cur;
    }
    return;
  }
  for(uint32_t i = tid; i < total; i += kSpThreads)
  {
    uint32_t lo = 0, hi = nz;
    while(hi - lo > 1) { const uint32_t m = (lo + hi) >> 1; if(s_zpre[m] <= i) lo = m; else hi = m; }
    const uint4 v = *reinterpret_cast<const uint4*>(c_eng.land[cur] + c_eng.zoff[lo] + (i - s_zpre[lo]));
    const uint32_t zm = (1u << c_eng.zbits) - 1u;
    bK[0][i] = ((uint64_t)((lo << c_eng.zbits) + (v.x & zm)) << 32) | v.y;
    bW[0][i] = v.x & ~zm;
    bA[0][i] = ((uint64_t)v.w << 32) | v.z;
  }
  for(uint32_t z = z0; z < z1; ++z) c_eng.land_n[cur][z] = 0;
  for(uint32_t z = z0; z < z1; ++z)
    if(c_eng.ztrig[cur ^ 1u][z])
    {
      const uint32_t zs = 1u << c_eng.zbits;
      const uint32_t L0 = z * zs, nact = min(zs, c_eng.n_local - L0);
      for(uint32_t i = 0; i < nact; ++i) c_eng.trig_own[cur ^ 1u][L0 + i] = 0;
      c_eng.ztrig[cur ^ 1u][z] = 0;
    }
  __syncthreads();

  uint32_t la = 0, lb = 1;
  uint32_t n = total;
  unsigned long long steps = 0;
  uint32_t reason = SP_QUIESCENT;
  unsigned long long delivered = 0, sent = 0, active = 0, applied = 0;
  int bt_t = 0;
  unsigned long long bt_n = 0;
  const SpList S{bK[2], bW[2], bA[2]};
  uint32_t q = 0;
#ifdef GPA_STAMPS
  unsigned long long ph[4] = {0, 0, 0, 0};
  unsigned long long tk = __builtin_amdgcn_s_memtime();
#define SP_STAMP(k) do { const unsigned long long t_ = __builtin_amdgcn_s_memtime(); ph[k] += t_ - tk; tk = t_; } while(0)
#else
#define SP_STAMP(k) do {} while(0)
#endif
  for(;;)
  {
    if(n == 0) { reason = SP_QUIESCENT; break; }
    if(max_steps && steps >= max_steps) { reason = SP_MAX_STEPS; break; }
    const SpList Acur{bK[la], bW[la], bA[la]};
    const SpList Bnxt{bK[lb], bW[lb], bA[lb]};
    uint32_t hb = 0;
    int dense1 = 0;
    bool coll = false;
    if(tid < n)
    {
      const uint32_t L = (uint32_t)(Acur.K[tid] >> 32);
      hb = (L * 0x9E3779B1u) >> (32 - kSpHashBits);
      coll = atomicAdd(&s_hcnt[hb], 1u) != 0u;
      const int t = sp_type(s_tinfo, n_types, L);
      dense1 = (t < 0 || (s_tinfo[t].flags & kSpNoRun) || 1u >= s_tinfo[t].batch) ? 1 : 0;
    }
    const bool any_cd = __syncthreads_or(coll || dense1);
    const bool distinct = !(any_cd && __syncthreads_or(coll));
    if(tid < n) s_hcnt[hb] = 0;
    int dense = 0;
    uint32_t h_r = 0, h_g = 0;
    const SpList* Srun = &S;
    if(distinct)
    {
      if(tid == 0) sp_cnt[q ^ 1u] = 0;
      if(tid < n) { h_r = tid; h_g = 1; }
      dense = any_cd ? 1 : 0;
      Srun = &Acur;
    }
    else
    {
    {
      const uint32_t P = min(16u, max(1u, kSpThreads / n));
      const uint32_t span = (n + P - 1) / P;
      for(uint32_t task = tid; task < n * P; task += kSpThreads)
      {
        const uint32_t p = task / n, i = task - p * n;
        const uint64_t ki = Acur.K[i];
        const uint32_t li = (uint32_t)(ki >> 32);
        const uint32_t wi = Acur.W[i] >> 16;
        const uint32_t j0 = p * span, j1 = min(n, j0 + span);
        uint32_t lt = 0, same = 0, ltsame = 0;
        uint32_t j = j0;
        for(; j + 4 <= j1; j += 4)
        {
          uint64_t kj[4];
          uint32_t wj[4];
#pragma unroll
          for(int u = 0; u < 4; ++u) { kj[u] = Acur.K[j + u]; wj[u] = Acur.W[j + u] >> 16; }
#pragma unroll
          for(int u = 0; u < 4; ++u)
          {
            const uint32_t b = (uint32_t)(kj[u] < ki) | ((uint32_t)(kj[u] == ki) & (uint32_t)(wj[u] < wi));
            const uint32_t sm = (uint32_t)((uint32_t)(kj[u] >> 32) == li);
            lt += b; same += sm; ltsame += b & sm;
          }
// ... 120 lines not shown
```

### ponyc_amd/csrc/step_entry.h

```cpp
#pragma once
#include <hip/hip_runtime.h>
#include <stdint.h>

typedef void (*step_kernel_t)(uint32_t, uint32_t, uint32_t);

struct StepEntry {
  step_kernel_t kernel;
  hipError_t (*upload)(const void* types, const void* eng, hipStream_t s);
  bool stub;
  uint32_t zone_bits;
  uint32_t threads;
  uint32_t sort_work;
  uint32_t bucket_words;
  bool hot;
  step_kernel_t plan, rest, fused;
};

namespace gpa {

StepEntry step_entry_any();
StepEntry step_entry_ring();
StepEntry step_entry_pinger();
StepEntry step_entry_pinger_det();
StepEntry step_entry_fanin_sender();
StepEntry step_entry_gups_streamer();
StepEntry step_entry_storm();
StepEntry step_entry_spreader();
StepEntry step_entry_fifo_pair();
StepEntry step_entry_program();

}
```

### ponyc_amd/csrc/step_tu.h

```cpp
#define GPA_STEP_TU 1
#include "zone_dev.h"
#include "step_entry.h"

namespace gpa {

#if defined(GPA_STEP_ONLY) && (GPA_STEP_ONLY != GPA_STEP_HT)
#define GPA_STEP_STUB 1
template <int HT> __global__ void k_step_stub(uint32_t, uint32_t, uint32_t) {}
template __global__ void k_step_stub<GPA_STEP_HT>(uint32_t, uint32_t, uint32_t);
#else
#define GPA_STEP_STUB 0
template __global__ void k_step<GPA_STEP_HT, 0>(uint32_t, uint32_t, uint32_t);
template <int HT, int PM> constexpr step_kernel_t split_kernel()
{
  if constexpr(PM == 3 && !(HT >= 0 && two_pass<HT>()))
    return nullptr;
  else if constexpr(HT >= 0 && (two_pass<HT>() || HT == GPU_ACTOR_HT_PINGER_DET || HT == GPU_ACTOR_HT_STORM ||
                                HT == GPU_ACTOR_HT_PROGRAM ||
                                HT == kHtFifoPair))
    return k_step<HT, PM>;
  else return nullptr;
}
#endif

namespace {
hipError_t step_upload(const void* types, const void* eng, hipStream_t s)
{
  const hipError_t e = hipMemcpyToSymbolAsync(HIP_SYMBOL(c_types), types,
    sizeof(TypeDev) * GPU_ACTOR_MAX_TYPES, 0, hipMemcpyHostToDevice, s);
  if(e != hipSuccess) return e;
  return hipMemcpyToSymbolAsync(HIP_SYMBOL(c_eng), eng, sizeof(EngDev), 0, hipMemcpyHostToDevice, s);
}
}

#if GPA_STEP_STUB
StepEntry GPA_STEP_ENTRY() { return { k_step_stub<GPA_STEP_HT>, step_upload, true, (uint32_t)kZoneBits,
                                      (uint32_t)kZoneThreads, kSortWork, 4u, false, nullptr, nullptr, nullptr }; }
#else
StepEntry GPA_STEP_ENTRY() { return { k_step<GPA_STEP_HT, 0>, step_upload, false, (uint32_t)kZoneBits,
                                      (uint32_t)kZoneThreads, kSortWork,
                                      dp_table<GPA_STEP_HT>() ? 6u : 4u,
                                      GPA_STEP_HT < 0 || GPA_STEP_HT == kHtFifoPair,
                                      split_kernel<GPA_STEP_HT, 1>(), split_kernel<GPA_STEP_HT, 2>(),
                                      split_kernel<GPA_STEP_HT, 3>() }; }
#endif

}
```

### ponyc_amd/csrc/zone_dev.h

```cpp
#pragma once
#include "engine_dev.h"

namespace gpa {

#ifdef GPA_STAMPS
#define GPA_STAMP(k)                                                         \
  do { if(threadIdx.x == 0) c_eng.dbg[z * kDbgSlots + (k)] = __builtin_amdgcn_s_memtime(); } while(0)
#define GPA_ACC(k, t0)                                                        \
  do { if(threadIdx.x == 0) c_eng.dbg[z * kDbgSlots + (k)] += __builtin_amdgcn_s_memtime() - (t0); } while(0)
#else
#define GPA_STAMP(k) do {} while(0)
#endif

constexpr int kUnroll = 8;
constexpr uint32_t kCarryRun = 256;
#ifndef GPA_IDX_CAP
#define GPA_IDX_CAP 16384
#endif
#ifndef GPA_TILE
#define GPA_TILE 4096
#endif
#ifndef GPA_EMIT_UNROLL
#define GPA_EMIT_UNROLL 4
#endif
// ... 88 lines not shown
    uint32_t x = lane < (uint32_t)kZoneWaves ? t[lane] : 0u;
    x = wave_incl_scan(x, lane);
    if(lane < (uint32_t)kZoneWaves) t[lane] = x;
  }
  __syncthreads();
  uint32_t ra = (wv ? s_tmp2[wv - 1] : 0u) + ia - sa;
  uint32_t rb = (wv ? s_tmp2[kZoneWaves + wv - 1] : 0u) + ib - sb;
#pragma unroll
  for(uint32_t k = 0; k < per; ++k)
  {
    off[tid * per + k] = ra; ra += va[k];
    aux[tid * per + k] = rb; rb += vb[k];
  }
  __syncthreads();
}

__device__ uint32_t block_scan_n(const uint32_t* in, uint32_t* out, uint32_t n, uint32_t* s_tmp)
{
  const uint32_t tid = threadIdx.x, lane = tid & 63, wv = tid >> 6;
  const uint32_t per = (n + kZoneThreads - 1) / kZoneThreads;
  const uint32_t lo = min(tid * per, n), hi = min(lo + per, n);
  uint32_t sum = 0;
  for(uint32_t i = lo; i < hi; ++i) sum += in[i];
  const uint32_t incl = wave_incl_scan(sum, lane);
  if(lane == 63) s_tmp[wv] = incl;
  lds_sync();
  if(wv == 0)
  {
    uint32_t x = lane < (uint32_t)kZoneWaves ? s_tmp[lane] : 0u;
    x = wave_incl_scan(x, lane);
    if(lane < (uint32_t)kZoneWaves) s_tmp[lane] = x;
  }
  lds_sync();
  uint32_t run = (wv ? s_tmp[wv - 1] : 0u) + incl - sum;
  for(uint32_t i = lo; i < hi; ++i) { const uint32_t v = in[i]; out[i] = run; run += v; }
  const uint32_t total = s_tmp[kZoneWaves - 1];
  lds_sync();
  return total;
}

template <int kMinRun = 0>
__device__ __forceinline__ uint32_t agg_add(uint32_t* ctr, uint32_t key, bool valid)
{
  const uint32_t lane = __lane_id();
  const uint64_t lt = lane ? (~0ull >> (64 - lane)) : 0ull;
  uint64_t active = __ballot(valid);
  uint32_t res = 0;
  for(int it = 0; it < 4 && active; ++it)
  {
    const int leader = __ffsll((long long)active) - 1;
    const uint32_t k = __builtin_amdgcn_readlane(key, leader);
    const uint64_t peers = __ballot(valid && key == k) & active;
    if(kMinRun > 0 && __popcll(peers) < kMinRun) break;
    uint32_t base = 0;
    if((int)lane == leader) base = atomicAdd(&ctr[k], (uint32_t)__popcll(peers));
    base = (uint32_t)__shfl((int)base, leader);
    if((peers >> lane) & 1ull) res = base + (uint32_t)__popcll(peers & lt);
    active &= ~peers;
  }
  if((active >> lane) & 1ull) res = atomicAdd(&ctr[key], 1u);
  return res;
}

template <int kMinRun = 0>
__device__ __forceinline__ void agg_count(uint32_t* ctr, uint32_t key, bool valid)
{
  const uint32_t lane = __lane_id();
  uint64_t active = __ballot(valid);
  for(int it = 0; it < 4 && active; ++it)
  {
    const int leader = __ffsll((long long)active) - 1;
    const uint32_t k = __builtin_amdgcn_readlane(key, leader);
    const uint64_t peers = __ballot(valid && key == k) & active;
    if(kMinRun > 0 && __popcll(peers) < kMinRun) break;
    if((int)lane == leader) atomicAdd(&ctr[k], (uint32_t)__popcll(peers));
    active &= ~peers;
  }
  if((active >> lane) & 1ull) atomicAdd(&ctr[key], 1u);
}

__device__ __forceinline__ void st16(uint4* p, const uint4& v)
{
  p->x = v.x; p->y = v.y; p->z = v.z; p->w = v.w;
}
__device__ __forceinline__ uint4 ld16(const uint4* p)
{
  uint4 v;
  v.x = p->x; v.y = p->y; v.z = p->z; v.w = p->w;
  return v;
}

__device__ __forceinline__ ZRec ld_rec(const ZRec* p)
{
  const uint4 v = *reinterpret_cast<const uint4*>(p);
  ZRec r;
  r.w0 = v.x; r.from = v.y; r.arg = ((uint64_t)v.w << 32) | v.z;
  return r;
}

struct AccIdx {
  uint16_t* idx;
  const ZRec* C;
  const ZRec* Ld;
  uint32_t nc_zone;
  __device__ __forceinline__ ZRec rec(uint32_t j) const
  {
    const uint32_t i = idx[j];
    return i < nc_zone ? ld_rec(C + i) : ld_rec(Ld + (i - nc_zone));
  }
  __device__ void sort(uint32_t lo, uint32_t g)
  {
    for(uint32_t i = 1; i < g; ++i)
    {
      const uint16_t x = idx[lo + i];
      const uint64_t kx = zkey(rec(lo + i));
      uint32_t j = i;
      while(j > 0 && zkey(rec(lo + j - 1)) > kx)
      {
        idx[lo + j] = idx[lo + j - 1];
        --j;
      }
      idx[lo + j] = x;
    }
  }
};

struct AccS {
  ZRec* p;
  const ZRec* c;
  uint32_t nc;
  const uint64_t* perm = nullptr;
  const uint4* stg = nullptr;
  uint32_t nst = 0;
  __device__ __forceinline__ ZRec rec(uint32_t j) const
  {
    if(j < nst)
    {
      const uint4 v = stg[j];
      ZRec r;
      r.w0 = v.x; r.from = v.y; r.arg = ((uint64_t)v.w << 32) | v.z;
      return r;
    }
    if(j < nc) return ld_rec(c + j);
    return ld_rec(p + (perm ? (uint32_t)(perm[j - nc] & 0xFFFFFull) : j - nc));
  }
  __device__ void sort(uint32_t lo, uint32_t g)
  {
    ZRec* q = p + (lo - nc);
    for(uint32_t i = 1; i < g; ++i)
    {
      const ZRec x = q[i];
      const uint64_t kx = zkey(x);
      uint32_t j = i;
      while(j > 0)
      {
        const ZRec y = q[j - 1];
        if(zkey(y) <= kx) break;
        q[j] = y;
        --j;
      }
      q[j] = x;
    }
  }
};

constexpr uint32_t kStageMin = 32;
// ... 594 lines not shown
  if(idx)
  {
    for(uint32_t j0 = 0; j0 < g; j0 += kZoneThreads * kUnroll)
    {
      uint64_t x[kUnroll];
#pragma unroll
      for(int u = 0; u < kUnroll; ++u)
      {
        const uint32_t j = j0 + u * kZoneThreads + tid;
        x[u] = j < g ? ia[j] : 0ull;
      }
#pragma unroll
      for(int u = 0; u < kUnroll; ++u)
      {
        const uint32_t j = j0 + u * kZoneThreads + tid;
        if(j < g) idx[nc + j] = (uint16_t)(x[u] & pm);
      }
    }
  }
  __syncthreads();
  return true;
}

template <int HT, class Acc>
__device__ __forceinline__ uint32_t zone_actor(const TypeDev& T, ZoneCtx& a, Acc acc, uint32_t n,
  uint32_t nc, bool stays, bool presorted)
{
  if(stays)
  {
    if(n - nc > 1 && !presorted) acc.sort(nc, n - nc);
    return 0;
  }
  return drain_zone<HT>(T, a, acc, n, nc, presorted);
}

template <int HT> __host__ __device__ constexpr bool two_pass()
{
  return HT == GPU_ACTOR_HT_PINGER;
}
template <int HT> __host__ __device__ constexpr int plan_words()
{
  if constexpr(HT >= 0 && two_pass<HT>()) return HT_Words<HT>::W; else return 1;
}
template <int HT> __host__ __device__ constexpr uint64_t plan_const_arg()
{
  static_assert(HT == GPU_ACTOR_HT_PINGER, "only the pinger's sends carry a constant");
  return kPingerPingArg;
}
constexpr uint32_t kRounds = kZone / kZoneThreads;
static_assert(kRounds == 4, "two rounds per packed count word, two words");
constexpr uint32_t kClasses = 16;

constexpr uint32_t kPlanTile = kTile * (uint32_t)(sizeof(uint4) / sizeof(uint2));
constexpr uint32_t kSuper = 2;
constexpr uint32_t kPerSuper = kRounds / kSuper;

__device__ __forceinline__ uint4 tile_rec16(const uint4& r, uint64_t) { return r; }
__device__ __forceinline__ uint4 tile_rec16(const uint2& r, uint64_t arg)
{
  return make_uint4(r.x, r.y, (uint32_t)arg, (uint32_t)(arg >> 32));
}

__device__ __forceinline__ uint32_t emit_rec(const uint4& r, uint32_t b, uint32_t pos, uint32_t L0,
  uint32_t nz, uint32_t nxt)
{
  const uint32_t from = (L0 + (r.y & kZoneMask)) * c_eng.nranks + c_eng.rank;
  if(b < nz)
  {
    uint4 v;
    v.x = (r.y & ~kZoneMask) | (rdiv(r.x) & kZoneMask);
    v.y = from;
    v.z = r.z;
    v.w = r.w;
    if(pos < zone_capacity(b))
      st16(reinterpret_cast<uint4*>(c_eng.land[nxt] + c_eng.zoff[b] + pos), v);
    else
      spill_rec(nxt, 0u, b, pos, v);
    return 0;
  }
  return xout_store(b - nz, pos, xpack(r.x, r.y & ~kZoneMask, from, ((uint64_t)r.w << 32) | r.z));
}

constexpr uint32_t kDirect = 0x80000000u;
__device__ __forceinline__ uint32_t chunk_dst(uint32_t b, uint32_t base, uint32_t h, uint32_t nz)
{
  if(b < nz)
  {
    const uint64_t o = c_eng.zoff[b] + base;
    if(base + h <= c_eng.zcapz[b] && o + h <= 0x7FFFFFFFull) return (uint32_t)o | kDirect;
  }
  return base;
}

__device__ __forceinline__ uint32_t emit_at(const uint4& r, uint32_t b, uint32_t d, uint32_t rel,
  uint32_t L0, uint32_t nz, uint32_t nxt)
{
  if(d & kDirect)
  {
    uint4 v;
    v.x = (r.y & ~kZoneMask) | (rdiv(r.x) & kZoneMask);
    v.y = (L0 + (r.y & kZoneMask)) * c_eng.nranks + c_eng.rank;
    v.z = r.z;
    v.w = r.w;
    st16(reinterpret_cast<uint4*>(c_eng.land[nxt] + ((d & ~kDirect) + rel)), v);
    return 0;
  }
  return emit_rec(r, b, d + rel, L0, nz, nxt);
}

#ifndef GPA_PLAIN_CTX
#define GPA_PLAIN_CTX 1
#endif
struct PlanCtx : ActorBase {
  static constexpr bool kPlain = GPA_PLAIN_CTX;
  uint32_t* rh;
  uint32_t inc;
  __device__ __forceinline__ void put(uint32_t to, uint32_t w, uint64_t arg)
  {
    atomicAdd(&rh[bucket_of(to)], inc);
  }
};

template <class Rec, uint64_t kArg = 0>
struct TileCtx : ActorBase {
  static constexpr bool kPlain = GPA_PLAIN_CTX;
  Rec* tile;
  uint32_t* cur;
  const uint32_t* st;
  const uint32_t* bs;
  uint32_t sh, inc;
  uint32_t L0, nz, nxt, xover;
  uint32_t tcap;
  __device__ __forceinline__ void put(uint32_t to, uint32_t w, uint64_t arg)
  {
    const uint32_t b = bucket_of(to);
    const uint32_t idx = (atomicAdd(&cur[b], inc) >> sh) & 0xFFFFu;
    Rec r;
    r.x = to; r.y = w | src_local;
    if constexpr(sizeof(Rec) == sizeof(uint4)) { r.z = (uint32_t)arg; r.w = (uint32_t)(arg >> 32); }
    if(idx < tcap)
      tile[idx] = r;
    else
      xover += emit_at(tile_rec16(r, kArg), b, bs[b], idx - ((st[b] >> sh) & 0xFFFFu), L0, nz, nxt);
  }
};

template <int NW>
__device__ __forceinline__ uint32_t plan_reserve(const uint32_t* rh, uint32_t* bs, uint32_t nb,
  uint32_t nz, uint32_t nxt, uint32_t tid)
{
  uint32_t n_atom = 0;
  for(uint32_t b = tid; b < nb; b += kZoneThreads)
  {
    uint32_t h = 0;
#pragma unroll
    for(int k = 0; k < NW; ++k)
    {
      const uint32_t w = rh[k * nb + b];
      h += (w & 0xFFFFu) + (w >> 16);
    }
    uint32_t base = 0;
    if(h)
    {
      ++n_atom;
      if(b < nz)
        base = atomicAdd(&c_eng.land_n[nxt][b], h);
      else
        base = (uint32_t)atomicAdd(&c_eng.xcount[b - nz], (unsigned long long)h);
    }
    bs[b] = chunk_dst(b, base, h, nz);
  }
  return n_atom;
}

template <int NW>
__device__ __forceinline__ void plan_scan(uint32_t* rh, uint32_t* cur, uint32_t nb, uint32_t* tmp2,
  uint32_t tid, uint32_t (&tot)[NW])
{
  static_assert(NW <= 2, "tmp2 holds two rows of wave totals");
  const uint32_t lane = tid & 63, wv = tid >> 6;
  const uint32_t per = (nb + kZoneThreads - 1) / kZoneThreads;
  const uint32_t lo = min(tid * per, nb), hi = min(lo + per, nb);
  uint32_t a[NW], ia[NW], ra[NW];
#pragma unroll
  for(int k = 0; k < NW; ++k) a[k] = 0;
  for(uint32_t b = lo; b < hi; ++b)
#pragma unroll
    for(int k = 0; k < NW; ++k) a[k] += rh[k * nb + b];
#pragma unroll
  for(int k = 0; k < NW; ++k)
  {
    ia[k] = wave_incl_scan(a[k], lane);
    if(lane == 63) tmp2[k * kZoneWaves + wv] = ia[k];
  }
  lds_sync();
  if(wv < (uint32_t)NW)
  {
    uint32_t* t = tmp2 + wv * kZoneWaves;
    uint32_t x = lane < (uint32_t)kZoneWaves ? t[lane] : 0u;
    x = wave_incl_scan(x, lane);
    if(lane < (uint32_t)kZoneWaves) t[lane] = x;
  }
  lds_sync();
#pragma unroll
  for(int k = 0; k < NW; ++k) ra[k] = (wv ? tmp2[k * kZoneWaves + wv - 1] : 0u) + ia[k] - a[k];
  for(uint32_t b = lo; b < hi; ++b)
#pragma unroll
    for(int k = 0; k < NW; ++k)
    {
      const uint32_t v = rh[k * nb + b];
      rh[k * nb + b] = ra[k]; cur[k * nb + b] = ra[k]; ra[k] += v;
    }
#pragma unroll
  for(int k = 0; k < NW; ++k) tot[k] = tmp2[(k + 1) * kZoneWaves - 1];
  lds_sync();
}

template <class Rec, uint64_t kArg = 0>
__device__ __forceinline__ uint32_t plan_emit(const Rec* tile, uint32_t m, const uint32_t* rst,
  const uint32_t* bsr, uint32_t* bsw, uint32_t sh, uint32_t tr, uint32_t nb, uint32_t L0,
  uint32_t nz, uint32_t nxt, uint32_t tid)
{
  uint32_t xover = 0;
  constexpr uint32_t kEU = GPA_EMIT_UNROLL;
  for(uint32_t q0 = 0; q0 < m; q0 += kEU * kZoneThreads)
  {
    Rec rec[kEU];
#pragma unroll
    for(uint32_t u = 0; u < kEU; ++u)
    {
      const uint32_t q = q0 + u * kZoneThreads + tid;
      if(q < m) rec[u] = tile[q];
    }
#pragma unroll
    for(uint32_t u = 0; u < kEU; ++u)
    {
      const uint32_t q = q0 + u * kZoneThreads + tid;
      if(q < m)
      {
        const uint32_t b = bucket_of(rec[u].x);
        xover += emit_at(tile_rec16(rec[u], kArg), b, bsr[b], q - ((rst[b] >> sh) & 0xFFFFu), L0, nz, nxt);
      }
    }
  }
  if(bsw)
    for(uint32_t b = tid; b < nb; b += kZoneThreads)
    {
      const uint32_t s0 = (rst[b] >> sh) & 0xFFFFu;
      const uint32_t s1 = b + 1 < nb ? (rst[b + 1] >> sh) & 0xFFFFu : tr;
      bsw[b] = bsr[b] + (s1 - s0);
    }
  return xover;
}

__device__ __forceinline__ uint16_t* dp_index(uint4* pool, uint32_t nl)
{
  return reinterpret_cast<uint16_t*>(pool + kTile) - ((nl + 7u) & ~7u);
}
__device__ __forceinline__ uint32_t dp_tile_cap(uint32_t nl)
{
  return (uint32_t)(kTile * sizeof(uint4) - ((nl + 7u) & ~7u) * sizeof(uint16_t)) / (uint32_t)sizeof(uint4);
}

template <int HTS> struct ZoneLds {
  uint4 pool[kTile];
  uint32_t tmp[kZoneWaves + 1];
  uint32_t tmp2[2 * kZoneWaves];
  uint32_t nout;
  uint32_t nmix;
  uint32_t tot;
  uint32_t ph[kClasses];
  unsigned long long agg[kZoneWaves];
  unsigned long long bytype[GPU_ACTOR_MAX_TYPES];
  __attribute__((aligned(16))) uint8_t tb[kZone];
  uint32_t ntrig;
  uint32_t bigbits[kZone / 32];
  uint32_t red3[3];
  uint32_t big[kMaxBig];
  uint32_t nbig;
  uint32_t stn;
  union {
    struct { uint32_t stl[kMaxStage], stc[kMaxStage], sto[kMaxStage + 1]; } st;
    unsigned long long red[kZoneWaves][6];
  } u;
  unsigned long long fan[((HTS < 0 && ((GPA_MIX_MASK >> GPU_ACTOR_HT_FANIN_SENDER) & 1u)) ||
                          HTS == GPU_ACTOR_HT_FANIN_SENDER) ? 2 * kFanLds : 1];
};
template <int HTS> __device__ __forceinline__ ZoneLds<HTS>& zone_lds()
{
  __shared__ ZoneLds<HTS> lds;
  return lds;
}

template <int HTS, int PM>
__device__ __forceinline__ bool zone_step(const uint32_t z, uint32_t cur, uint32_t pend_slot,
  uint32_t sidx)
{
  ZoneLds<HTS>& Z = zone_lds<HTS>();
  uint4* const s_pool = Z.pool;
  static_assert(4 * kZone * sizeof(uint32_t) + kIdxCap * sizeof(uint16_t) <= sizeof(uint4) * kTile,
                "LDS pool too small");
  uint32_t* const s_cnt = reinterpret_cast<uint32_t*>(s_pool);
  uint32_t* const s_off = s_cnt + kZone;
  uint32_t* const s_ccnt = s_off + kZone;
  uint32_t* const s_aux = s_ccnt + kZone;
  uint16_t* const s_idx = reinterpret_cast<uint16_t*>(s_aux + kZone);
  uint32_t* const s_cst = reinterpret_cast<uint32_t*>(s_idx);
  extern __shared__ uint32_t s_dyn[];
  auto& s_tmp = Z.tmp;
  auto& s_tmp2 = Z.tmp2;
  auto& s_nout = Z.nout;
  auto& s_nmix = Z.nmix;
  auto& s_tot = Z.tot;
  auto& s_ph = Z.ph;
  auto& s_agg = Z.agg;
  auto& s_red = Z.u.red;
  auto& s_bytype = Z.bytype;
  auto& s_tb = Z.tb;
  auto& s_ntrig = Z.ntrig;
  auto& s_bigbits = Z.bigbits;
  auto& s_red3 = Z.red3;
  auto& s_big = Z.big;
  auto& s_nbig = Z.nbig;
  auto& s_stn = Z.stn;
  auto& s_stl = Z.u.st.stl;
  auto& s_stc = Z.u.st.stc;
  auto& s_sto = Z.u.st.sto;
  auto& s_fan = Z.fan;
  constexpr bool kFan = (HTS < 0 && ((GPA_MIX_MASK >> GPU_ACTOR_HT_FANIN_SENDER) & 1u)) ||
                        HTS == GPU_ACTOR_HT_FANIN_SENDER;

  const uint32_t tid = threadIdx.x, lane = tid & 63, wv = tid >> 6;
  static_assert(PM == 0 || HTS >= 0, "split launches are for one-table engines");
  constexpr bool kPlanSplit = HTS >= 0 && two_pass<HTS>();
  constexpr bool kSimple = PM == 1 && !kPlanSplit;
  constexpr bool kDP = kSimple && dp_table<HTS>();
  bool dp = false;
  if constexpr(PM == 2)
    if(__builtin_amdgcn_readfirstlane(c_eng.zplan[z]) == sidx + 1u) return false;
  const bool halt_now = c_eng.nranks == 1 ? (c_eng.spill_n[cur] != 0u || *c_eng.halt != 0u)
                                          : (*c_eng.spill_flag != 0u);
  if(halt_now)
  {
    if(PM != 1 && z == 0 && tid == 0)
    {
      *c_eng.halt = 1u;
      c_eng.pend[pend_slot] = kPendSkipped;
      atomicAdd(c_eng.skipped, 1ull);
    }
    return false;
  }
#ifdef GPA_STAMPS
  if(tid == 0)
  {
    c_eng.dbg[z * kDbgSlots + 11] = __builtin_amdgcn_s_memrealtime();
    c_eng.dbg[z * kDbgSlots + 12] = 0;
  }
#endif
  if(tid < GPU_ACTOR_MAX_TYPES) s_bytype[tid] = 0;
  if(tid < kClasses) s_ph[tid] = 0;
  if constexpr(kFan)
    for(uint32_t j = tid; j < 2 * kFanLds; j += kZoneThreads) s_fan[j] = 0;
  const uint32_t nxt = cur ^ 1u;
  const uint32_t L0 = z * kZone;
  const uint32_t nact = min(kZone, c_eng.n_local - L0);
  const uint32_t R = c_eng.nranks, me = c_eng.rank;
  const uint32_t nz = c_eng.n_zones;
  const uint32_t nb = nz + (R > 1 ? R : 0u);
  constexpr bool SR = HTS != GPU_ACTOR_HT_PINGER_DET;
  auto rfl = [](uint32_t v) __attribute__((always_inline)) {
    return SR ? __builtin_amdgcn_readfirstlane(v) : v;
  };
  const uint32_t cap = SR ? zone_cap_s(z) : zone_capacity(z);
  const uint64_t zo = SR ? zone_off_s(z) : c_eng.zoff[z];
  uint32_t* s_hist = s_dyn;
  uint32_t* s_base = s_dyn + nb;

  const uint32_t ztc = rfl(c_eng.ztrig[cur][z]);
  const uint32_t ztn = rfl(c_eng.ztrig[nxt][z]);
  const bool gate = rfl(c_eng.trig_n[sidx % 3u]) != 0u;
  if(z == 0 && tid == 0)
  {
    c_eng.trig_n[(sidx + 2u) % 3u] = 0u;
    c_eng.bigc_n[cur ^ 1u] = 0ull;
  }
  if constexpr(PM == 1)
    if(gate || ztc != 0u || (kPlanSplit && c_eng.two_pass == 0u)) return false;
  uint8_t* const tb_out = c_eng.trig_own[nxt];

  for(uint32_t i = tid; i < kZone; i += kZoneThreads) { s_cnt[i] = 0; s_ccnt[i] = 0; }
  for(uint32_t b = tid; b < (kDP ? 2u : 1u) * nb; b += kZoneThreads) s_hist[b] = 0;
  if(tid == 0) { s_nout = 0; s_ntrig = 0; s_nmix = 0; s_tot = 0; }
  __syncthreads();
  GPA_STAMP(0);

  const uint32_t nc = min(rfl(c_eng.carry_n[cur][z]), cap);
  const uint32_t nl = min(rfl(c_eng.land_n[cur][z]), cap);
  if(nc + nl == 0 && ztc == 0)
  {
    if constexpr(PM == 1) return false;
    if(tid == 0) c_eng.carry_n[nxt][z] = 0;
    if(ztn)
    {
      for(uint32_t i = tid; i < nact; i += kZoneThreads) tb_out[(L0 + i) * R + me] = 0;
      if(tid == 0) c_eng.ztrig[nxt][z] = 0;
    }
    return false;
  }
  if constexpr(kSimple)
    if(nc != 0u || nl > kIdxCap) return false;
  if(ztc)
    for(uint32_t i = tid; i < kZone; i += kZoneThreads)
      s_tb[i] = i < nact ? c_eng.trig[cur][(L0 + i) * R + me] : (uint8_t)0;
  else
    for(uint32_t i = tid; i < kZone / 4; i += kZoneThreads)
      reinterpret_cast<uint32_t*>(s_tb)[i] = 0;
  const ZRec* C = c_eng.carry[cur] + zo;
  const ZRec* Ld = c_eng.land[cur] + zo;
  const bool use_idx = kSimple || nc + nl <= kIdxCap;
  constexpr bool kHotTables = !kSimple && (HTS < 0 || HTS == kHtFifoPair);
  const bool hot = kHotTables && c_eng.hot_on &&
                   __builtin_amdgcn_readfirstlane(c_eng.hot_prep[z]) == sidx + 1u;
  const uint32_t* const hot_cnt =
    c_eng.hot_cnt + (size_t)__builtin_amdgcn_readfirstlane(hot ? c_eng.hot_slot[z] : 0u) * 4096u;
  uint32_t nmix = 0;
  const uint32_t nrun = (nc + kCarryRun - 1) / kCarryRun;
  const bool sampled = !kSimple && nc > kIdxCap && nrun <= kIdxCap / 2;
  uint32_t* const s_mix = reinterpret_cast<uint32_t*>(s_idx);
  if(sampled)
  {
    for(uint32_t k = tid; k < nrun; k += kZoneThreads)
    {
      const uint32_t lo = k * kCarryRun, hi = min(lo + kCarryRun, nc);
      const uint32_t a0 = C[lo].w0 & kZoneMask, a1 = C[hi - 1].w0 & kZoneMask;
      if(a0 == a1)
        atomicAdd(&s_ccnt[a0], hi - lo);
      else
        s_mix[atomicAdd(&s_nmix, 1u)] = k;
    }
    __syncthreads();
    nmix = s_nmix;
  }
  const uint32_t ncount = sampled ? nmix * kCarryRun : nc;
  for(uint32_t base = 0; base < ncount; base += kZoneThreads * kUnroll)
  {
    uint32_t w[kUnroll];
#pragma unroll
    for(int u = 0; u < kUnroll; ++u)
    {
      const uint32_t j = base + u * kZoneThreads + tid;
      const uint32_t i = sampled ? s_mix[min(j, ncount - 1) / kCarryRun] * kCarryRun + j % kCarryRun : j;
      w[u] = (j < ncount && i < nc) ? C[i].w0 : 0xFFFFFFFFu;
    }
#pragma unroll
    for(int u = 0; u < kUnroll; ++u)
      agg_count(s_ccnt, w[u] & kZoneMask, w[u] != 0xFFFFFFFFu);
  }
  int tz = -1;
  for(uint32_t t = 0; t < c_eng.n_types; ++t)
    if(L0 >= c_types[t].lfirst && L0 + nact <= c_types[t].lfirst + c_types[t].lcount)
      tz = (int)t;
  tz = __builtin_amdgcn_readfirstlane(tz);
  if constexpr(PM == 1)
    if(tz < 0) return false;
  constexpr int kPW = plan_words<HTS>();
  uint64_t st[kRounds][kPW];
  if constexpr(HTS >= 0 && two_pass<HTS>())
    if(PM != 2 && !gate && ztc == 0 && tz >= 0)
    {
      const TypeDev& T = c_types[tz];
#pragma unroll
      for(uint32_t r = 0; r < kRounds; ++r)
      {
        const uint32_t i = r * kZoneThreads + tid;
#pragma unroll
        for(int k = 0; k < kPW; ++k)
          st[r][k] = i < nact ? T.state[(size_t)k * T.lcount + (L0 + i - T.lfirst)] : 0ull;
      }
    }
  uint32_t wr[kIdxPer];
  if constexpr(kDP)
  {
    constexpr int kDpChunk = 8;
    static_assert(kIdxPer % kDpChunk == 0, "dp count chunks");
    const TypeDev& T = c_types[tz];
    PlanCtx pc;
    pc.reset_common();
    pc.type = tz;
#pragma unroll
    for(int u0 = 0; u0 < kIdxPer; u0 += kDpChunk)
    {
      uint4 rr[kDpChunk];
#pragma unroll
      for(int v = 0; v < kDpChunk; ++v)
      {
        const uint32_t i = (u0 + v) * kZoneThreads + tid;
        if(i < nl) rr[v] = ld16(reinterpret_cast<const uint4*>(Ld + i));
        else rr[v].x = 0xFFFFFFFFu;
      }
#pragma unroll
      for(int v = 0; v < kDpChunk; ++v)
      {
        wr[u0 + v] = rr[v].x;
        if(rr[v].x == 0xFFFFFFFFu) continue;
        const uint32_t act = rr[v].x & kZoneMask;
        wr[u0 + v] = (atomicAdd(&s_cnt[act], 1u) << kZoneBits) | act;
        const uint32_t rd = act / kZoneThreads;
        pc.rh = s_hist + (rd >> 1) * nb;
        pc.inc = (rd & 1u) ? 0x10000u : 1u;
        pc.self = (L0 + act) * R + me;
        pc.li = L0 + act - T.lfirst;
        pc.src_local = act;
        uint64_t junk[HT_Words<HTS>::W] = {};
        handle(HtTag<HTS>{}, T, pc, junk, (rr[v].x >> 12) & 0xFu,
               ((uint64_t)rr[v].w << 32) | rr[v].z);
      }
    }
  }
  else if(use_idx)
  {
#pragma unroll
    for(int u = 0; u < kIdxPer; ++u)
    {
      const uint32_t i = u * kZoneThreads + tid;
      wr[u] = i < nl ? Ld[i].w0 : 0xFFFFFFFFu;
    }
#pragma unroll
    for(int u = 0; u < kIdxPer; ++u)
      if(wr[u] != 0xFFFFFFFFu)
      {
        const uint32_t act = wr[u] & kZoneMask;
        wr[u] = (atomicAdd(&s_cnt[act], 1u) << kZoneBits) | act;
      }
  }
  else if(hot)
    for(uint32_t i = tid; i < kZone; i += kZoneThreads)
    {
      s_cnt[i] = hot_cnt[i];
      const_cast<uint32_t*>(hot_cnt)[i] = 0;
    }
  else
  for(uint32_t base = 0; base < nl; base += kZoneThreads * kUnroll)
  {
    uint32_t w[kUnroll];
#pragma unroll
    for(int u = 0; u < kUnroll; ++u)
    {
      const uint32_t i = base + u * kZoneThreads + tid;
      w[u] = i < nl ? Ld[i].w0 : 0xFFFFFFFFu;
    }
#pragma unroll
    for(int u = 0; u < kUnroll; ++u)
      agg_count<8>(s_cnt, w[u] & kZoneMask, w[u] != 0xFFFFFFFFu);
  }
  __syncthreads();
  GPA_STAMP(1);
  bool took_mail = false;
  auto take_mail = [&]() __attribute__((always_inline)) { took_mail = true; };
  if constexpr(PM != 1) take_mail();


  bool fast = false, plan = false;
  uint32_t own_n[kRounds], pk[kRounds], prk[kRounds];
  if constexpr(HTS >= 0 && order_free<HTS>())
    if(!gate && ztc == 0 && tz >= 0)
    {
      const uint32_t bt = c_types[tz].prio ? 0xFFFFFFFFu : c_types[tz].batch;
      int over = 0;
      uint32_t tot = 0;
#pragma unroll
      for(uint32_t r = 0; r < kRounds; ++r)
      {
        const uint32_t i = r * kZoneThreads + tid;
        const uint32_t c = s_cnt[i] + s_ccnt[i];
        over |= c > bt;
        tot += c;
        if constexpr(two_pass<HTS>())
          if(PM != 2)
          {
            own_n[r] = i < nact ? c : 0u;
            pk[r] = kClasses - 1u - min(own_n[r], kClasses - 1u);
            prk[r] = agg_add(s_ph, pk[r], true);
          }
      }
      GPA_STAMP(13);
      tot = (uint32_t)min(wave_sum((unsigned long long)tot), 0xFFFFFFFFull);
      if(lane == 0 && tot) atomicAdd(&s_tot, tot);
      fast = !__syncthreads_or(over);
      GPA_STAMP(14);
      if constexpr(two_pass<HTS>())
        plan = PM != 2 && fast && s_tot < c_eng.seq_max && c_eng.two_pass != 0u;
    }
  if constexpr(PM == 1)
  {
    if constexpr(kPlanSplit)
    {
      if(!plan) return false;
    }
    else
    {
      int big = 0;
      for(uint32_t i = tid; i < kZone; i += kZoneThreads) big |= s_cnt[i] > kBigGroup;
      if(__syncthreads_or(big)) return false;
      if constexpr(kDP)
      {
        const uint32_t bt = c_types[tz].prio ? 0xFFFFFFFFu : c_types[tz].batch;
        if(tid == 0) { s_stn = 0; s_sto[0] = 0; }
        __syncthreads();
        int over = 0;
        for(uint32_t i = tid; i < kZone; i += kZoneThreads)
        {
          const uint32_t c = s_cnt[i];
          over |= c > bt;
          if(c > small_regs<HTS>())
          {
            const uint32_t k = atomicAdd(&s_stn, 1u);
            if(k < kMaxStage) s_stl[k] = i;
            atomicAdd(&s_sto[0], c);
          }
        }
        __syncthreads();
        over |= s_stn > kMaxStage || s_sto[0] > (uint32_t)kZoneThreads;
        dp = !__syncthreads_or(over);
        if(!dp) return false;
      }
    }
    take_mail();
  }
  ZRec* Sz = c_eng.S + 3 * zo;
  uint64_t* const perm_s = reinterpret_cast<uint64_t*>(Sz + 2 * cap);
  if(fast)
  {
    for(uint32_t i = tid; i < kZone; i += kZoneThreads) s_cnt[i] += s_ccnt[i];
    for(uint32_t k = tid; k < kZone / 32; k += kZoneThreads) s_bigbits[k] = 0;
    __syncthreads();
  }
  else
  {
  block_scan_zone_pair(s_cnt, s_ccnt, s_off, s_aux, s_tmp2);
  GPA_STAMP(2);

  if(use_idx)
    for(uint32_t i0 = 0; i0 < nc; i0 += kZoneThreads * kUnroll)
    {
      uint32_t w[kUnroll];
#pragma unroll
      for(int u = 0; u < kUnroll; ++u)
      {
        const uint32_t i = i0 + u * kZoneThreads + tid;
        w[u] = i < nc ? C[i].w0 : 0u;
      }
#pragma unroll
      for(int u = 0; u < kUnroll; ++u)
      {
        const uint32_t i = i0 + u * kZoneThreads + tid;
        if(i >= nc) continue;
        const uint32_t a = w[u] & kZoneMask;
        s_idx[s_off[a] + (i - s_aux[a])] = (uint16_t)i;
      }
    }
  if(use_idx)
  {
    uint16_t* const s_ix = dp ? dp_index(s_pool, nl) : s_idx;
#pragma unroll
    for(int u = 0; u < kIdxPer; ++u)
      if(wr[u] != 0xFFFFFFFFu)
      {
        const uint32_t act = wr[u] & kZoneMask;
        s_ix[s_off[act] + s_ccnt[act] + (wr[u] >> kZoneBits)] = (uint16_t)(nc + u * kZoneThreads + tid);
      }
  }
  else
  {
    __syncthreads();
    for(uint32_t i = tid; i < kZone; i += kZoneThreads)
// ... 92 lines not shown
  };


  uint32_t delivered = 0, active = 0, sent = 0, applied = 0;
  uint32_t n_atom = 0, dropped = 0, xover = 0;
  uint32_t ncout = 0;
  ZoneCtx a;
  a.reset_common();
  if constexpr(HTS >= 0 && two_pass<HTS>())
    if(plan)
    {
      constexpr int NW = HT_Words<HTS>::W;
      const TypeDev T = c_types[tz];
      constexpr uint64_t kArg = plan_const_arg<HTS>();
      uint32_t* const s_rh = s_dyn;
      uint32_t* const s_cur = s_dyn + nb;
      uint32_t* const s_bs = s_dyn + 2 * nb;
      uint2* const tile = reinterpret_cast<uint2*>(s_pool);
      for(uint32_t b = tid; b < nb; b += kZoneThreads) s_rh[b] = 0;
      constexpr bool kStageApart =
        kZone * sizeof(uint32_t) + NW * kZone * sizeof(uint64_t) + kZone * sizeof(uint16_t)
          <= kTile * sizeof(uint4);
      uint64_t* const s_stage = reinterpret_cast<uint64_t*>(s_pool) + (kStageApart ? kZone / 2 : 0);
      uint16_t* const s_perm = reinterpret_cast<uint16_t*>(s_pool + kTile) - kZone;
      static_assert(NW * kZone * sizeof(uint64_t) + kZone * sizeof(uint16_t) <= kTile * sizeof(uint4),
                    "two-pass state stage and permutation fit the pool");
      if(wv == 0)
      {
        const uint32_t c = lane < kClasses ? s_ph[lane] : 0u;
        const uint32_t x = wave_incl_scan(c, lane) - c;
        if(lane < kClasses) s_ph[lane] = x;
      }
      lds_sync();
#pragma unroll
      for(uint32_t r = 0; r < kRounds; ++r)
        s_perm[s_ph[pk[r]] + prk[r]] = (uint16_t)(r * kZoneThreads + tid);
      lds_sync();
      uint32_t ai[kRounds], nm[kRounds];
#pragma unroll
      for(uint32_t r = 0; r < kRounds; ++r)
      {
        const uint32_t j = (r & 1u) ? (uint32_t)kZoneWaves - 1u - wv : wv;
        const uint32_t blk = 8u * (j >> 1) + ((j & 1u) ? 7u - r : r);
        ai[r] = s_perm[64u * blk + lane];
        nm[r] = s_cnt[ai[r]];
      }
      if constexpr(!kStageApart)
        lds_sync();
#pragma unroll
      for(uint32_t r = 0; r < kRounds; ++r)
#pragma unroll
        for(int k = 0; k < NW; ++k)
          s_stage[k * kZone + r * kZoneThreads + tid] = st[r][k];
      lds_sync();
#pragma unroll
      for(uint32_t r = 0; r < kRounds; ++r)
#pragma unroll
        for(int k = 0; k < NW; ++k)
          st[r][k] = s_stage[k * kZone + ai[r]];
#ifdef GPA_STAMPS
      GPA_STAMP(8);
      if(tid == 0) { c_eng.dbg[z * kDbgSlots + 9] = 0; c_eng.dbg[z * kDbgSlots + 10] = 0; }
#endif
#pragma unroll
      for(uint32_t r = 0; r < kRounds; ++r)
      {
        if(!nm[r]) continue;
        const uint32_t i = ai[r];
        PlanCtx pc;
        pc.reset_common();
        pc.li = L0 + i - T.lfirst;
        pc.self = (L0 + i) * R + me;
        pc.src_local = i;
        pc.type = tz;
        pc.rh = s_rh;
        pc.inc = (r / kPerSuper) ? 0x10000u : 1u;
        uint64_t sc[NW];
#pragma unroll
        for(int k = 0; k < NW; ++k) sc[k] = st[r][k];
        for(uint32_t j = 0; j < nm[r]; ++j) handle(HtTag<HTS>{}, T, pc, sc, 0u, 0ull);
      }
      lds_sync();
      GPA_STAMP(3);
      n_atom += plan_reserve<1>(s_rh, s_bs, nb, nz, nxt, tid);
      GPA_STAMP(5);
#ifdef GPA_STAMPS
      const unsigned long long t_scan = __builtin_amdgcn_s_memtime();
#endif
      uint32_t tot[1];
      plan_scan<1>(s_rh, s_cur, nb, s_tmp2, tid, tot);
#ifdef GPA_STAMPS
      GPA_ACC(9, t_scan);
#endif
      TileCtx<uint2, kArg> tc;
      tc.reset_common();
      tc.tile = tile;
      tc.tcap = kPlanTile;
      tc.L0 = L0; tc.nz = nz; tc.nxt = nxt; tc.xover = 0;
      uint32_t dz = 0;
#ifdef GPA_STAMPS
      unsigned long long emit_clk = 0, t_emit = 0;
#endif
      tc.cur = s_cur;
      tc.st = s_rh;
      tc.type = tz;
#pragma unroll
      for(uint32_t q = 0; q < kSuper; ++q)
      {
        const uint32_t sh = q * 16u;
        const uint32_t tr = (tot[0] >> sh) & 0xFFFFu;
        const uint32_t* const bsr = s_bs + q * nb;
        uint32_t* const bsw = q + 1 < kSuper ? s_bs + (q ^ 1u) * nb : nullptr;
        tc.bs = bsr;
        tc.sh = sh; tc.inc = 1u << sh;
#ifdef GPA_STAMPS
        const unsigned long long t_hand = __builtin_amdgcn_s_memtime();
#endif
#pragma unroll
        for(uint32_t r = q * kPerSuper; r < (q + 1) * kPerSuper; ++r)
          if(nm[r])
          {
            const uint32_t i = ai[r];
            const uint32_t L = L0 + i;
            tc.li = L - T.lfirst;
            tc.self = L * R + me;
            tc.src_local = i;
            tc.seq = 0;
            for(uint32_t j = 0; j < nm[r]; ++j) handle(HtTag<HTS>{}, T, tc, st[r], 0u, 0ull);
            const bool full = T.prio ? (nm[r] % T.batch == 0u) : nm[r] == T.batch;
            s_tb[i] = full ? 1u : 0u;
            if(full) atomicAdd(&s_ntrig, 1u);
            delivered += nm[r];
            active += 1;
            dz += nm[r];
          }
        lds_sync();
#ifdef GPA_STAMPS
        GPA_ACC(10, t_hand);
        t_emit = __builtin_amdgcn_s_memtime();
#endif
        xover += plan_emit<uint2, kArg>(tile, min(tr, kPlanTile), s_rh, bsr, bsw, sh, tr, nb, L0, nz,
                                        nxt, tid);
        lds_sync();
#ifdef GPA_STAMPS
        emit_clk += __builtin_amdgcn_s_memtime() - t_emit;
#endif
      }
#pragma unroll
      for(uint32_t r = 0; r < kRounds; ++r)
#pragma unroll
        for(int k = 0; k < NW; ++k)
          s_stage[k * kZone + ai[r]] = st[r][k];
      lds_sync();
#pragma unroll
      for(uint32_t r = 0; r < kRounds; ++r)
      {
        const uint32_t i = r * kZoneThreads + tid;
        if(own_n[r])
#pragma unroll
          for(int k = 0; k < NW; ++k)
            T.state[(size_t)k * T.lcount + (L0 + i - T.lfirst)] = s_stage[k * kZone + i];
      }
#ifdef GPA_STAMPS
      if(tid == 0) c_eng.dbg[z * kDbgSlots + 2] = emit_clk;
#endif
      sent = tc.sent;
      xover += tc.xover;
// ... 341 lines not shown
      constexpr uint32_t kStride = kZoneThreads * kH;
      auto load_half = [&](ZRec (&r)[kH], uint32_t j0) __attribute__((always_inline)) {
#pragma unroll
        for(int uu = 0; uu < kH; ++uu)
        {
          const uint32_t j = j0 + uu * kZoneThreads + tid;
          if(j < rem)
            r[uu] = use_idx ? AccIdx{s_idx + s_off[i], C, Ld, nc}.rec(n - rem + j)
                            : acc_s(i).rec(n - rem + j);
        }
      };
      auto store_half = [&](const ZRec (&r)[kH], uint32_t j0) __attribute__((always_inline)) {
#pragma unroll
        for(int uu = 0; uu < kH; ++uu)
        {
          const uint32_t j = j0 + uu * kZoneThreads + tid;
          if(j >= rem) continue;
          uint4 u;
          u.x = r[uu].w0; u.y = r[uu].from; u.z = (uint32_t)r[uu].arg; u.w = (uint32_t)(r[uu].arg >> 32);
          const uint32_t pos = co + j;
          if(pos < cap)
            *reinterpret_cast<uint4*>(cout + pos) = u;
          else
            spill_rec(nxt, kSpillCarry, z, pos, u);
        }
      };
      ZRec ra[kH], rb[kH];
      load_half(ra, 0);
      for(uint32_t j0 = 0; j0 < rem; j0 += 2 * kStride)
      {
        load_half(rb, j0 + kStride);
        store_half(ra, j0);
        load_half(ra, j0 + 2 * kStride);
        store_half(rb, j0 + kStride);
      }
    }
  }
  }
  if(tid == 0) c_eng.carry_n[nxt][z] = ncout;
  const uint32_t ntrig = s_ntrig;
  if(ntrig || ztn)
  {
    if(R == 1)
      for(uint32_t i = tid; i < kZone / 4; i += kZoneThreads)
      {
        if(4 * i < nact)
          reinterpret_cast<uint32_t*>(tb_out + L0)[i] = reinterpret_cast<const uint32_t*>(s_tb)[i];
      }
    else
      for(uint32_t i = tid; i < nact; i += kZoneThreads) tb_out[(L0 + i) * R + me] = s_tb[i];
    if(tid == 0)
    {
      c_eng.ztrig[nxt][z] = ntrig;
      if(ntrig) atomicAdd(&c_eng.trig_n[(sidx + 1u) % 3u], ntrig);
    }
  }
  __syncthreads();
  GPA_STAMP(4);
  if(tid < GPU_ACTOR_MAX_TYPES && s_bytype[tid])
    stat_add_z(ST_BY_TYPE + tid, z, s_bytype[tid]);
  if constexpr(kFan)
    if(a.fan)
    {
      const TypeDev& F = c_types[a.fan_t];
      for(uint32_t j = tid; j < kFanLds && j < F.lcount; j += kZoneThreads)
        if(s_fan[j])
        {
          atomicAdd(reinterpret_cast<unsigned long long*>(&F.state[j]), s_fan[j]);
          atomicXor(reinterpret_cast<unsigned long long*>(&F.state[(size_t)F.lcount + j]),
            s_fan[kFanLds + j]);
        }
    }

  if(!(PM == 1 && kPlanSplit) && !plan && !dp)
  {
  uint32_t* s_tcnt = s_dyn + 2 * nb;
  uint32_t* s_tst = s_dyn + 3 * nb;
  for(uint32_t b = tid; b < nb; b += kZoneThreads)
  {
    const uint32_t h = s_hist[b];
    if(h)
    {
      ++n_atom;
      const uint32_t base = b < nz ? atomicAdd(&c_eng.land_n[nxt][b], h)
                                   : (uint32_t)atomicAdd(&c_eng.xcount[b - nz], (unsigned long long)h);
      s_base[b] = chunk_dst(b, base, h, nz);
    }
    s_tcnt[b] = 0;
  }
  __syncthreads();
  GPA_STAMP(5);
  const uint32_t nout = min(s_nout, cap);
  const ORec* Oz = c_eng.O + zo;
  auto emit = [&](const uint4& r, uint32_t b, uint32_t rel) __attribute__((always_inline)) {
    xover += emit_at(r, b, s_base[b], rel, L0, nz, nxt);
  };
  if(nout <= kZoneThreads)
  {
    if(tid < nout)
    {
      const uint4 r = ld16(reinterpret_cast<const uint4*>(Oz + tid));
      const uint32_t b = bucket_of(r.x);
      emit(r, b, atomicAdd(&s_tcnt[b], 1u));
    }
  }
  else
  for(uint32_t t0 = 0; t0 < nout; t0 += kTile)
  {
    const uint32_t m = min(kTile, nout - t0);
    uint4 ov[kTilePer];
    uint32_t bk[kTilePer], rk[kTilePer];
#pragma unroll
    for(int u = 0; u < kTilePer; ++u)
    {
      const uint32_t i = min(u * kZoneThreads + tid, m - 1);
      ov[u] = ld16(reinterpret_cast<const uint4*>(Oz + t0 + i));
    }
#pragma unroll
    for(int u = 0; u < kTilePer; ++u)
    {
      const uint32_t i = u * kZoneThreads + tid;
      if(i < m)
      {
        bk[u] = bucket_of(ov[u].x);
        rk[u] = atomicAdd(&s_tcnt[bk[u]], 1u);
      }
    }
    lds_sync();
    (void)block_scan_n(s_tcnt, s_tst, nb, s_tmp);
#pragma unroll
    for(int u = 0; u < kTilePer; ++u)
    {
      const uint32_t i = u * kZoneThreads + tid;
      if(i < m) s_pool[s_tst[bk[u]] + rk[u]] = ov[u];
    }
    lds_sync();
    for(uint32_t p = tid; p < m; p += kZoneThreads)
    {
      const uint4 r = s_pool[p];
      const uint32_t b = bucket_of(r.x);
      emit(r, b, p - s_tst[b]);
    }
    lds_sync();
    for(uint32_t b = tid; b < nb; b += kZoneThreads)
    {
      s_base[b] += s_tcnt[b];
      s_tcnt[b] = 0;
    }
    lds_sync();
  }
  }

  unsigned long long v[6] = { delivered + applied, sent, active, dropped, xover, n_atom };
#pragma unroll
  for(int k = 0; k < 6; ++k)
  {
    v[k] = wave_sum(v[k]);
    if(lane == 0) s_red[wv][k] = v[k];
  }
  __syncthreads();
  GPA_STAMP(6);
  if(tid < 6)
  {
    unsigned long long tot = 0;
    for(int w = 0; w < kZoneWaves; ++w) tot += s_red[w][tid];
    const int idx = tid == 0 ? ST_DELIVERED : tid == 1 ? ST_SENT : tid == 2 ? ST_ACTIVE
                  : tid == 3 ? ST_DROPPED : tid == 4 ? ST_XCHG_OVERFLOW : ST_ATOMICS;
    if(tot) stat_add_z(idx, z, tot);
  }
  if(plan && tid == 6) stat_add_z(ST_PLAN_ZONES, z, 1ull);
  if(took_mail && tid == 0)
  {
    if(nc + nl) pend_add_z(pend_slot, z, (unsigned long long)(nc + nl));
    c_eng.carry_n[cur][z] = 0;
    c_eng.land_n[cur][z] = 0;
    if constexpr(PM == 1) c_eng.zplan[z] = sidx + 1u;
  }
#ifdef GPA_STAMPS
  if(tid == 0) c_eng.dbg[z * kDbgSlots + 12] = __builtin_amdgcn_s_memrealtime();
#endif
  return true;
}


template <int HTS>
__device__ __noinline__ void zone_step_rest(uint32_t z, uint32_t cur, uint32_t pend_slot, uint32_t sidx)
{
  zone_step<HTS, 2>(z, cur, pend_slot, sidx);
}

template <int HTS, int PM>
__global__ void __launch_bounds__(kZoneThreads, 4) k_step(uint32_t cur, uint32_t pend_slot,
  uint32_t sidx)
{
  if constexpr(PM != 3)
    zone_step<HTS, PM>(blockIdx.x, cur, pend_slot, sidx);
  else if(!zone_step<HTS, 1>(blockIdx.x, cur, pend_slot, sidx))
  {
    __syncthreads();
    zone_step_rest<HTS>(blockIdx.x, cur, pend_slot, sidx);
  }
}

#ifndef GPA_STEP_TU
__global__ void __launch_bounds__(kBlock) k_pending(uint32_t cur, uint32_t slot)
{
  __shared__ unsigned long long s_red[kWaves];
  const uint32_t z = blockIdx.x * kBlock + threadIdx.x;
  unsigned long long p = 0;
  if(z < c_eng.n_zones)
  {
    const uint32_t cap = zone_capacity(z);
    p = min(c_eng.carry_n[cur][z], cap) + min(c_eng.land_n[cur][z], cap);
  }
  p = wave_sum(p);
  if(__lane_id() == 0) s_red[threadIdx.x >> 6] = p;
  __syncthreads();
  if(threadIdx.x == 0)
  {
    unsigned long long tot = 0;
    for(int w = 0; w < kWaves; ++w) tot += s_red[w];
    if(tot) atomicAdd(&c_eng.pend[slot], tot);
  }
}

#endif

constexpr int kLandThreads = 1024;
constexpr int kLandPer = 8;
constexpr uint32_t kLandRecs = kLandThreads * kLandPer;

struct LandRec {
  bool valid;
  uint32_t to, w, from;
  uint64_t arg;
};

__device__ __forceinline__ void land_records(LandRec (&r)[kLandPer], uint32_t cur,
  uint32_t* s_hist, uint32_t* s_base)
{
  const uint32_t nz = c_eng.n_zones;
  for(uint32_t b = threadIdx.x; b < nz; b += kLandThreads) s_hist[b] = 0;
  __syncthreads();
  uint32_t zt[kLandPer], rk[kLandPer];
#pragma unroll
  for(int u = 0; u < kLandPer; ++u)
    if(r[u].valid)
    {
      zt[u] = zone_of_local(rdiv(r[u].to));
      rk[u] = atomicAdd(&s_hist[zt[u]], 1u);
    }
  __syncthreads();
  for(uint32_t b = threadIdx.x; b < nz; b += kLandThreads)
    if(s_hist[b]) s_base[b] = atomicAdd(&c_eng.land_n[cur][b], s_hist[b]);
  __syncthreads();
#pragma unroll
  for(int u = 0; u < kLandPer; ++u)
    if(r[u].valid)
    {
      const uint32_t pos = s_base[zt[u]] + rk[u];
      uint4 v;
      v.x = r[u].w | slot_in_zone(rdiv(r[u].to));
      v.y = r[u].from;
      v.z = (uint32_t)r[u].arg;
      v.w = (uint32_t)(r[u].arg >> 32);
      land_store(cur, zt[u], pos, v);
    }
}

#ifndef GPA_STEP_TU
__global__ void __launch_bounds__(kLandThreads) k_inject(const gpu_msg_t* msgs, uint64_t n,
  uint64_t hseq_base, uint32_t cur)
{
  __shared__ uint32_t s_hist[kMaxZones];
  __shared__ uint32_t s_base[kMaxZones];
  LandRec r[kLandPer];
#pragma unroll
  for(int u = 0; u < kLandPer; ++u)
  {
    const uint64_t i = (uint64_t)blockIdx.x * kLandRecs + (uint64_t)u * kLandThreads + threadIdx.x;
    r[u].valid = false;
    if(i < n)
    {
      const gpu_msg_t m = msgs[i];
      const uint64_t hseq = hseq_base + i;
      if(!is_remote(m.to))
      {
        const int t = type_of_global(m.to);
        if(t >= 0 && c_types[t].reducible)
        {
          reducible_apply_local(m.to, m.behaviour, m.arg);
          atomicAdd(&c_eng.stats[ST_DELIVERED], 1ull);
          atomicAdd(&c_eng.stats[ST_BY_TYPE + t], 1ull);
        }
        else if(t >= 0)
        {
          r[u].valid = true;
          r[u].to = m.to;
          r[u].w = ((uint32_t)(hseq & 0xFFFFull) << 16) | ((m.behaviour & 0xFu) << 12);
          r[u].from = kHostFrom | (uint32_t)(hseq >> 16);
          r[u].arg = m.arg;
        }
      }
    }
  }
  land_records(r, cur, s_hist, s_base);
}

__global__ void __launch_bounds__(kLandThreads) k_xinject(const XRec* in, uint64_t n, uint32_t cur,
  const unsigned long long* rcnt, uint64_t stride)
{
  __shared__ uint32_t s_hist[kMaxZones];
  __shared__ uint32_t s_base[kMaxZones];
  __shared__ unsigned long long s_app[GPU_ACTOR_MAX_TYPES];
  __shared__ unsigned long long s_roff[kMaxRanks];
  const uint32_t R = c_eng.nranks, me = c_eng.rank;
  if(threadIdx.x < GPU_ACTOR_MAX_TYPES) s_app[threadIdx.x] = 0;
  if(threadIdx.x == 0)
  {
    unsigned long long acc = 0;
    for(uint32_t p = 0; p < R; ++p)
    {
      s_roff[p] = acc;
      acc += rcnt[p];
    }
  }
  __syncthreads();
  LandRec r[kLandPer];
#pragma unroll
  for(int u = 0; u < kLandPer; ++u)
  {
    const uint64_t i = (uint64_t)blockIdx.x * kLandRecs + (uint64_t)u * kLandThreads + threadIdx.x;
    r[u].valid = false;
    if(i < n)
    {
      uint32_t src = 0;
      for(uint32_t p = 1; p < R; ++p)
// ... 32 lines not shown
```

### ponyc_amd/engine.py

```python
from __future__ import annotations

import ctypes
import os
import threading

import numpy as np

_HERE = os.path.dirname(os.path.abspath(__file__))
LIB_PATH = os.environ.get("PONYC_AMD_LIB", os.path.join(_HERE, "libgpuactor.so"))

MSG_DTYPE = np.dtype([("to", "<u4"), ("behaviour", "<u4"), ("arg", "<u8")])
MAX_TYPES = 16

HT_RING, HT_PINGER, HT_PINGER_DET, HT_FANIN_SENDER, HT_FANIN_ANALYZER = 1, 2, 3, 4, 5
HT_GUPS_STREAMER, HT_GUPS_UPDATER, HT_STORM, HT_FIFO_SRC, HT_FIFO_SINK = 6, 7, 8, 9, 10
RING_SET, RING_PASS = 0, 1
PINGER_PING = 0
FANIN_SEND_MSGS, FANIN_MSG = 0, 0
GUPS_APPLY, GUPS_UPDATE = 0, 0
STORM_TOKEN, STORM_STORM = 0, 1
FIFO_BURST, FIFO_PUSH = 0, 0
HT_SPREADER = 11
HT_PROGRAM = 12
SPREADER_SPREAD, SPREADER_RESULT = 0, 1
# ... 279 lines not shown

    def busy(self) -> bool:
        return bool(self.lib.gpu_actor_busy())

    def run_fixed(self, n: int) -> None:
        _ck("gpu_actor_run_fixed", self.lib.gpu_actor_run_fixed(n))

    def sync(self) -> None:
        _ck("gpu_actor_sync", self.lib.gpu_actor_sync())

    def last_drain_ms(self) -> float:
        return float(self.lib.gpu_actor_last_drain_ms())

    def local_count(self, type_id: int) -> int:
        first, count, r, n = self.first[type_id], self.count[type_id], self.rank, self.n_ranks

        def below(x):
            return (x - r + n - 1) // n if x > r else 0
        return below(first + count) - below(first)

    def state_read(self, type_id: int, first: int = 0, n: int | None = None) -> np.ndarray:
        if n is None:
            n = self.local_count(type_id) - first
        words = self.words[type_id]
        out = np.zeros((words, n), dtype=np.uint64)
        _ck("gpu_actor_state_read",
            self.lib.gpu_actor_state_read(type_id, first, n, out.ctypes.data_as(ctypes.c_void_p)))
        return out

    def state_write(self, type_id: int, values: np.ndarray, first: int = 0) -> None:
        arr = np.ascontiguousarray(values, dtype=np.uint64)
        n = arr.shape[1]
        _ck("gpu_actor_state_write",
            self.lib.gpu_actor_state_write(type_id, first, n, arr.ctypes.data_as(ctypes.c_void_p)))

    def counts(self) -> dict:
        c = Counts()
        _ck("gpu_actor_counts", self.lib.gpu_actor_counts(ctypes.byref(c)))
        return {
            "steps": c.steps, "delivered": c.delivered, "sent": c.sent,
            "pending": c.pending, "dropped": c.dropped, "remote": c.remote,
            "active": c.active,
            "delivered_by_type": [c.delivered_by_type[i] for i in range(MAX_TYPES)],
            "atomics": c.atomics,
        }

    def host_reserve(self, n: int) -> None:
        _ck("gpu_actor_host_reserve", self.lib.gpu_actor_host_reserve(n))

    def recv_pending(self) -> int:
        n = ctypes.c_uint64(0)
        _ck("gpu_actor_recv_pending", self.lib.gpu_actor_recv_pending(ctypes.byref(n)))
        return n.value

    def recv(self, cap: int | None = None) -> np.ndarray:
        if cap is None:
            cap = self.recv_pending()
        out = np.zeros(cap, dtype=HOST_MSG_DTYPE)
        n = ctypes.c_uint64(0)
        _ck("gpu_actor_recv",
            self.lib.gpu_actor_recv(out.ctypes.data_as(ctypes.c_void_p), cap, ctypes.byref(n)))
        return out[:n.value]

    def host_notify(self, fn) -> None:
        if fn is None:
            _ck("gpu_actor_host_notify", self.lib.gpu_actor_host_notify(HOST_FN(), None))
            self._host_thunk = None
            return

        def _cb(_ctx, msgs, n):
            try:
                buf = (ctypes.c_uint8 * (int(n) * HOST_MSG_DTYPE.itemsize)).from_address(msgs)
                fn(np.frombuffer(buf, dtype=HOST_MSG_DTYPE).copy())
            except Exception as e:
                print(f"gpu_actor host_notify callback failed: {e!r}")
        thunk = HOST_FN(_cb)
        _ck("gpu_actor_host_notify", self.lib.gpu_actor_host_notify(thunk, None))
        self._host_thunk = thunk

    def debug_info(self) -> dict:
        keys = ["fixups", "sparse_launches", "sparse_steps", "zone_records", "spill_cap", "zones",
                "trig_n0", "trig_n1", "trig_n2", "zone_bits", "hot_missed", "hot_on", "jit",
                "jit_builds", "gups_updates", "gups_atomics", "peer_write",
                "gups_chunks_in", "gups_chunks_out", "gups_remote"]
        out = (ctypes.c_uint64 * len(keys))()
        fn = self.lib.gpu_actor_debug_info
        fn.argtypes = [ctypes.c_void_p, ctypes.c_uint64]
        fn.restype = ctypes.c_int
        _ck("gpu_actor_debug_info", fn(out, len(keys)))
        return {k: int(out[i]) for i, k in enumerate(keys)}

    def stream(self) -> int:
        return int(self.lib.gpu_actor_stream() or 0)

    def shutdown(self) -> None:
        if self.alive:
            _ck("gpu_actor_shutdown", self.lib.gpu_actor_shutdown())
            self.alive = False
            if not getattr(_IN_CALLBACK, "active", False):
                self._thunks.clear()
            if self._xp is not None:
                self.lib.gpu_actor_set_transport(ALLTOALLV_FN(), ALLREDUCE_FN(), None)
                self._xp = None

    def __enter__(self):
        return self

    def __exit__(self, *exc):
        self.shutdown()


def live_buffers() -> tuple[int, int]:
    fn = load_library().gpu_actor_debug_live_buffers
    fn.argtypes = [ctypes.POINTER(ctypes.c_uint64)]
    fn.restype = None
    out = (ctypes.c_uint64 * 2)()
    fn(out)
    return int(out[0]), int(out[1])


def jit_compile(progs, z12: bool = False, arch: str = "gfx950", lib_path: str | None = None) -> None:
    lib = ctypes.CDLL(lib_path or LIB_PATH)
    fn = lib.gpu_actor_debug_jit_compile
    fn.argtypes = [ctypes.c_void_p, ctypes.c_void_p, ctypes.c_void_p, ctypes.c_uint32, ctypes.c_int,
                   ctypes.c_char_p]
    fn.restype = ctypes.c_int
    types = np.array([t for t, _ in progs], dtype=np.uint32)
    words = np.concatenate([np.asarray(w, dtype=np.uint64) for _, w in progs])
    lens = np.array([len(w) for _, w in progs], dtype=np.uint32)
    _ck("gpu_actor_debug_jit_compile", fn(types.ctypes.data, words.ctypes.data, lens.ctypes.data,
                                          len(progs), int(z12), arch.encode()))


def jit_source(progs, z12: bool = False, lib_path: str | None = None) -> str:
    lib = ctypes.CDLL(lib_path or LIB_PATH)
    fn = lib.gpu_actor_debug_jit_source
    fn.argtypes = [ctypes.c_void_p, ctypes.c_void_p, ctypes.c_void_p, ctypes.c_uint32, ctypes.c_int,
                   ctypes.c_char_p, ctypes.c_uint64]
    fn.restype = ctypes.c_int64
    types = np.array([t for t, _ in progs], dtype=np.uint32)
    words = np.concatenate([np.asarray(w, dtype=np.uint64) for _, w in progs])
    lens = np.array([len(w) for _, w in progs], dtype=np.uint32)
    args = (types.ctypes.data, words.ctypes.data, lens.ctypes.data, len(progs), int(z12))
    n = fn(*args, None, 0)
    _ck("gpu_actor_debug_jit_source", n)
    buf = ctypes.create_string_buffer(n + 1)
    _ck("gpu_actor_debug_jit_source", fn(*args, buf, n + 1))
    return buf.value.decode()


def jit_compile_mix(mask: int, z12: bool = False, arch: str = "gfx950", lib_path: str | None = None) -> None:
    lib = ctypes.CDLL(lib_path or LIB_PATH)
    fn = lib.gpu_actor_debug_jit_compile_mix
    fn.argtypes = [ctypes.c_uint32, ctypes.c_int, ctypes.c_char_p]
    fn.restype = ctypes.c_int
    _ck("gpu_actor_debug_jit_compile_mix", fn(mask, int(z12), arch.encode()))
```

Measured before the change: 85.45 billion msgs/s.

## Add compact 8-byte landing records for constant-argument two-pass actor types

Adds a parallel compact landing buffer of 8-byte records (word plus sender) used when the actor type's message argument is a compile-time constant, such as pingers. The planned emit path writes 8 B instead of 16 B per message. The zone step reads the compact records directly or expands them back to 16 B form when needed. The aim is to cut message-write memory traffic in the landing zones. In exchange it adds a second 64-bit atomic counter per reservation, overflow tracking via an lc_over flag, a host flush/expand kernel, and more complex halt and spill handling.

Result: faster. 91.94 billion msgs/s (median of 6 runs) (+7.6%).

```diff
diff --git a/ponyc_amd/csrc/engine.hip b/ponyc_amd/csrc/engine.hip
--- a/ponyc_amd/csrc/engine.hip
+++ b/ponyc_amd/csrc/engine.hip
@@ -208,6 +208,13 @@
   c_eng.stats[ST_DROPPED] += n;
 }
 
+__global__ void __launch_bounds__(kBlock) k_land8_mirror(const uint32_t* land_n,
+  unsigned long long* landc_n, uint32_t n)
+{
+  const uint32_t i = blockIdx.x * kBlock + threadIdx.x;
+  if(i < n) landc_n[i] = (unsigned long long)land_n[i] << 32;
+}
+
 __global__ void __launch_bounds__(kBlock) k_spill_need(const SpillRec* s, uint32_t n, uint32_t* need)
 {
   const uint32_t i = blockIdx.x * kBlock + threadIdx.x;
@@ -224,12 +231,49 @@
   base[c_eng.zoff[r.z] + (r.tag & kSpillPosMask)] = r.rec;
 }
 
+__global__ void __launch_bounds__(kBlock) k_land_expand(uint32_t p, uint64_t arg)
+{
+  constexpr uint32_t kWaves = kBlock / 64;
+  __shared__ uint32_t s_wave[kWaves];
+  const uint32_t z = blockIdx.x;
+  const uint32_t nlc = min((uint32_t)c_eng.landc_n[p][z], c_eng.zcapz[z]);
+  const uint32_t lane = threadIdx.x & 63u, wv = threadIdx.x >> 6;
+  uint32_t pos0 = c_eng.land_n[p][z];
+  const uint2* const Lc = c_eng.landc[p] + c_eng.zoff[z];
+  for(uint32_t i0 = 0; i0 < nlc; i0 += kBlock)
+  {
+    const uint32_t i = i0 + threadIdx.x;
+    const uint2 r = i < nlc ? Lc[i] : make_uint2(kLand8Hole, 0u);
+    const bool rec = r.x != kLand8Hole;
+    const unsigned long long m = __ballot(rec);
+    if(lane == 0) s_wave[wv] = (uint32_t)__popcll(m);
+    __syncthreads();
+    uint32_t before = 0, round = 0;
+    for(uint32_t w = 0; w < kWaves; ++w)
+    {
+      const uint32_t c = s_wave[w];
+      if(w < wv) before += c;
+      round += c;
+    }
+    if(rec)
+      land_store(p, z, pos0 + before + (uint32_t)__popcll(m & ((1ull << lane) - 1ull)),
+        make_uint4(r.x, r.y, (uint32_t)arg, (uint32_t)(arg >> 32)));
+    pos0 += round;
+    __syncthreads();
+  }
+  if(threadIdx.x == 0)
+  {
+    c_eng.land_n[p][z] = pos0;
+    c_eng.landc_n[p][z] = (unsigned long long)pos0 << 32;
+    if(z == 0) atomicAnd(c_eng.lc_over, ~(1u << p));
+  }
+}
+
 constexpr uint32_t kBigCopyCap = 4096;
 constexpr uint32_t kBigCopyBlocks = 512;
 __global__ void __launch_bounds__(kBlock) k_carry_big(uint32_t cur)
 {
-  const bool halt_now = c_eng.nranks == 1 ? (c_eng.spill_n[cur] != 0u || *c_eng.halt != 0u)
-                                          : (*c_eng.spill_flag != 0u);
+  const bool halt_now = c_eng.nranks == 1 ? step_halted(cur) : (*c_eng.spill_flag != 0u);
   if(halt_now) return;
   const unsigned long long v = c_eng.bigc_n[cur];
   const uint32_t n = min((uint32_t)(v >> 32), c_eng.bigc_cap);
@@ -288,7 +332,7 @@
 struct SpillStat {
   unsigned int spill_n[2];
   unsigned int halt;
-  unsigned int pad;
+  unsigned int lc_over;
   unsigned long long skipped;
 };
 
@@ -334,6 +378,10 @@
   DevBuf<uint32_t> d_zcap;
   DevBuf<ZRec> d_land[2], d_carry[2];
   DevBuf<uint32_t> d_land_n[2], d_carry_n[2];
+  DevBuf<uint2> d_landc[2];
+  DevBuf<unsigned long long> d_landc_n[2];
+  bool land8 = false, land8_dirty = false;
+  uint64_t land8_arg = 0;
   DevBuf<ZRec> d_S;
   DevBuf<ORec> d_O;
   uint32_t par = 0;
@@ -608,6 +656,8 @@
   return 0;
 }
 
+bool land8_table();
+
 int upload_types()
 {
   TypeDev td[GPU_ACTOR_MAX_TYPES];
@@ -675,6 +725,13 @@
   e.spill_cap = g.spill_cap;
   e.xspill = g.d_xspill; e.xspill_n = g.d_xspill_n; e.xspill_cap = g.xspill_cap;
   e.zbits = g.zbits;
+  {
+    g.land8 = land8_table() && g.d_landc[0] && g.d_landc[1] && g.d_sstat;
+    if(g.land8) g.land8_arg = pick_step_entry().plan_arg;
+    e.land8 = g.land8 ? 1u : 0u;
+    for(int p = 0; p < 2; ++p) { e.landc[p] = g.d_landc[p]; e.landc_n[p] = g.d_landc_n[p]; }
+    e.lc_over = g.d_sstat ? &g.d_sstat->lc_over : nullptr;
+  }
   g.defer_big = defer_big_wanted();
   {
     const char* f = getenv("PONYC_AMD_HOT");
@@ -744,6 +801,8 @@
 }
 
 int relayout_zones(bool geometry = false);
+int land8_flush();
+bool land8_table();
 StepEntry step_entry_for(bool z12);
 bool step_fits(const StepEntry& se, uint64_t nb);
 int upload_types();
@@ -765,11 +824,36 @@
 
 inline bool spill_pending()
 {
-  return g.h_sstat->spill_n[0] || g.h_sstat->spill_n[1] || g.h_sstat->halt;
+  return g.h_sstat->spill_n[0] || g.h_sstat->spill_n[1] || g.h_sstat->halt || g.h_sstat->lc_over;
+}
+
+bool land8_table()
+{
+  const char* f = getenv("PONYC_AMD_LAND8");
+  return pick_step_entry().const_arg && !(f && atoi(f) == 0);
+}
+
+int land8_flush()
+{
+  if(!g.land8 || !g.land8_dirty || g.n_zones == 0) return 0;
+  for(uint32_t p = 0; p < 2; ++p)
+    hipLaunchKernelGGL(k_land_expand, dim3(g.n_zones), dim3(kBlock), 0, g.stream, p, g.land8_arg);
+  HIPCK(hipGetLastError());
+  g.land8_dirty = false;
+  g.dev_epoch++;
+  return 0;
 }
 
 int fixup_spill()
 {
+  if(g.h_sstat->lc_over)
+  {
+    g.land8_dirty = true;
+    int rc = land8_flush();
+    if(rc) return rc;
+    rc = read_sstat();
+    if(rc) return rc;
+  }
   const SpillStat st = *g.h_sstat;
   g.dev_epoch++;
   if(R() == 1 && !st.spill_n[0] && !st.spill_n[1] && !st.halt) return 0;
@@ -841,6 +925,7 @@
 bool zones_empty()
 {
   if(g.n_zones == 0) return true;
+  if(land8_flush() != 0) return false;
   std::vector<uint32_t> v(g.n_zones);
   for(int p = 0; p < 2; ++p)
     for(const uint32_t* src : {g.d_land_n[p].get(), g.d_carry_n[p].get()})
@@ -856,6 +941,10 @@
 int relayout_zones(bool geometry)
 {
   bool fresh = false;
+  {
+    const int rc = land8_flush();
+    if(rc) return rc;
+  }
   {
     const uint32_t want = pick_zone_bits((g.n_actors + R() - 1) / R());
     if(geometry && want != g.zbits && g.steps_total == 0 && g.sparse_launches == 0)
@@ -938,6 +1027,18 @@
     }
     HIPCK(hipStreamSynchronize(g.stream));
   }
+  DevBuf<uint2> lc[2];
+  DevBuf<unsigned long long> lcn[2];
+  if(land8_table())
+    for(int p = 0; p < 2; ++p)
+    {
+      HIPCK(lc[p].alloc(recs));
+      HIPCK(lcn[p].alloc(nzn));
+      hipLaunchKernelGGL(k_land8_mirror, dim3(blocks_for(nzn)), dim3(kBlock), 0, g.stream,
+        (const uint32_t*)ln[p], (unsigned long long*)lcn[p], (uint32_t)nzn);
+      HIPCK(hipGetLastError());
+      HIPCK(hipStreamSynchronize(g.stream));
+    }
   HIPCK(S.alloc(3 * recs));
   HIPCK(O.alloc(recs));
   const uint64_t slots = (uint64_t)nz * za;
@@ -957,6 +1058,7 @@
   {
     g.d_land[p].swap(land[p]); g.d_carry[p].swap(carry[p]);
     g.d_land_n[p].swap(ln[p]); g.d_carry_n[p].swap(cn[p]);
+    g.d_landc[p].swap(lc[p]); g.d_landc_n[p].swap(lcn[p]);
   }
   g.d_S.swap(S);
   g.d_O.swap(O);
@@ -1045,7 +1147,7 @@
 
 __global__ void k_spill_flag(unsigned int* flag)
 {
-  *flag = c_eng.spill_n[0] + c_eng.spill_n[1];
+  *flag = c_eng.spill_n[0] + c_eng.spill_n[1] + (c_eng.land8 ? *c_eng.lc_over : 0u);
 }
 
 __global__ void __launch_bounds__(256) k_gups_apply()
@@ -1284,7 +1386,7 @@
 __global__ void k_spill_local(unsigned long long* out)
 {
   *out = (unsigned long long)c_eng.spill_n[0] + c_eng.spill_n[1] + *c_eng.halt +
-         (c_eng.nranks > 1 ? *c_eng.spill_flag : 0u);
+         (c_eng.land8 ? *c_eng.lc_over : 0u) + (c_eng.nranks > 1 ? *c_eng.spill_flag : 0u);
 }
 
 __global__ void k_xprep()
@@ -2005,6 +2107,7 @@
   g.dev_epoch++;
   const StepEntry se = pick_step_entry();
   if(se.stub) return GPU_ACTOR_EINVAL;
+  if(g.land8) g.land8_dirty = true;
   const uint64_t nb = g.n_zones + (R() > 1 ? R() : 0);
   if(!step_fits(se, nb)) return GPU_ACTOR_ERANGE;
   const size_t dyn = step_dyn_bytes(se, nb);
@@ -2734,6 +2837,10 @@
 int run_sparse(uint64_t max_steps, SparseCtl& out)
 {
   g.dev_epoch++;
+  {
+    const int rc = land8_flush();
+    if(rc) return rc;
+  }
   bool prog = false, gups = false;
   for(const HostType& t : g.types)
   {
@@ -3252,11 +3359,12 @@
   }
   HIPCK(hipMemcpyAsync(st, g.d_stats, sizeof(st), hipMemcpyDeviceToHost, g.stream));
   HIPCK(hipStreamSynchronize(g.stream));
-  const uint64_t v[21] = {g.fixups, g.sparse_launches, g.sparse_steps, g.zone_records, g.spill_cap,
+  const uint64_t v[22] = {g.fixups, g.sparse_launches, g.sparse_steps, g.zone_records, g.spill_cap,
                           g.n_zones, tn[0], tn[1], tn[2], g.zbits, hb[3], g.hot_on ? 1u : 0u,
                           g.jit_used ? 1u : 0u, g.jit_builds, gu[0], gu[1], g.peer_write ? 1u : 0u,
-                          g.gups_in_total, g.gups_out_total, gu[2], st[ST_PLAN_ZONES]};
-  for(uint64_t i = 0; i < n && i < 21; ++i) out[i] = v[i];
+                          g.gups_in_total, g.gups_out_total, gu[2], st[ST_PLAN_ZONES],
+                          st[ST_LAND8]};
+  for(uint64_t i = 0; i < n && i < 22; ++i) out[i] = v[i];
   return 0;
 }
 
diff --git a/ponyc_amd/csrc/engine_dev.h b/ponyc_amd/csrc/engine_dev.h
--- a/ponyc_amd/csrc/engine_dev.h
+++ b/ponyc_amd/csrc/engine_dev.h
@@ -39,6 +39,7 @@
   ST_SEQ_OVERFLOW = 5, ST_XCHG_OVERFLOW = 6, ST_ACTIVE = 7,
   ST_ATOMICS = 8,
   ST_PLAN_ZONES = 9,
+  ST_LAND8 = 10,
   ST_BY_TYPE = 16, ST_COUNT = 32
 };
 
@@ -176,7 +177,19 @@
   uint4* host_rec;
   unsigned int* host_n;
   const uint64_t* host_step;
-};
+  uint2* landc[2];
+  unsigned long long* landc_n[2];
+  unsigned int* lc_over;
+  uint32_t land8, pad10;
+};
+constexpr uint32_t kLand8Hole = 0xFFFFFFFFu;
+#if defined(__HIPCC_RTC__)
+constexpr bool kLand8Code = false;
+#elif defined(GPA_STEP_HT)
+constexpr bool kLand8Code = (GPA_STEP_HT) == GPU_ACTOR_HT_PINGER;
+#else
+constexpr bool kLand8Code = true;
+#endif
 constexpr uint32_t kHostShards = 64;
 constexpr uint32_t kGupsShards = 64;
 constexpr uint32_t kShards = 32;
@@ -386,6 +399,24 @@
   return 0;
 }
 
+__device__ __forceinline__ uint32_t land_reserve(uint32_t p, uint32_t b, uint32_t h)
+{
+  const uint32_t base = atomicAdd(&c_eng.land_n[p][b], h);
+  if(kLand8Code && c_eng.land8)
+  {
+    const unsigned long long o = atomicAdd(&c_eng.landc_n[p][b], (unsigned long long)h << 32);
+    const uint64_t all = (o & 0xFFFFFFFFull) + (o >> 32) + h;
+    if((uint32_t)o != 0u && all > c_eng.zcapz[b]) atomicOr(c_eng.lc_over, 1u << p);
+  }
+  return base;
+}
+
+__device__ __forceinline__ bool step_halted(uint32_t cur)
+{
+  if(c_eng.spill_n[cur] != 0u || *c_eng.halt != 0u) return true;
+  return kLand8Code && c_eng.land8 && ((*c_eng.lc_over >> cur) & 1u) != 0u;
+}
+
 __device__ __forceinline__ void land_store(uint32_t p, uint32_t z, uint32_t pos, const uint4& v)
 {
   if(pos < zone_capacity(z))
@@ -401,7 +432,7 @@
   const uint32_t b = bucket_of(to);
   if(b < nz)
   {
-    const uint32_t pos = atomicAdd(&c_eng.land_n[nxt][b], 1u);
+    const uint32_t pos = land_reserve(nxt, b, 1u);
     uint4 v;
     v.x = w | slot_in_zone(rdiv(to));
     v.y = self;
diff --git a/ponyc_amd/csrc/sparse_dev.h b/ponyc_amd/csrc/sparse_dev.h
--- a/ponyc_amd/csrc/sparse_dev.h
+++ b/ponyc_amd/csrc/sparse_dev.h
@@ -71,7 +71,7 @@
   {
     const uint32_t L = (uint32_t)(l.K[i] >> 32);
     const uint32_t z = zone_of_local(L);
-    const uint32_t pos = atomicAdd(&c_eng.land_n[p][z], 1u);
+    const uint32_t pos = land_reserve(p, z, 1u);
     uint4 v;
     v.x = l.W[i] | slot_in_zone(L);
     v.y = (uint32_t)l.K[i];
@@ -197,7 +197,8 @@
   for(uint32_t z = z0; z < z1; ++z) { const uint32_t c = s_zpre[z]; s_zpre[z] = run; run += c; }
   if(tid == 0) s_zpre[nz] = total;
   const bool pending_fixup = c_eng.spill_n[cur] != 0u || *c_eng.halt != 0u ||
-                             c_eng.trig_n[sidx % 3u] != 0u;
+                             c_eng.trig_n[sidx % 3u] != 0u ||
+                             (c_eng.land8 && *c_eng.lc_over != 0u);
   if(__syncthreads_or(carried) || total > kSpCap || pending_fixup)
   {
     if(tid == 0)
@@ -216,7 +217,11 @@
     bW[0][i] = v.x & ~zm;
     bA[0][i] = ((uint64_t)v.w << 32) | v.z;
   }
-  for(uint32_t z = z0; z < z1; ++z) c_eng.land_n[cur][z] = 0;
+  for(uint32_t z = z0; z < z1; ++z)
+  {
+    c_eng.land_n[cur][z] = 0;
+    if(c_eng.land8) c_eng.landc_n[cur][z] = 0ull;
+  }
   for(uint32_t z = z0; z < z1; ++z)
     if(c_eng.ztrig[cur ^ 1u][z])
     {
diff --git a/ponyc_amd/csrc/step_entry.h b/ponyc_amd/csrc/step_entry.h
--- a/ponyc_amd/csrc/step_entry.h
+++ b/ponyc_amd/csrc/step_entry.h
@@ -14,6 +14,8 @@
   uint32_t bucket_words;
   bool hot;
   step_kernel_t plan, rest, fused;
+  bool const_arg;
+  uint64_t plan_arg;
 };
 
 namespace gpa {
diff --git a/ponyc_amd/csrc/step_tu.h b/ponyc_amd/csrc/step_tu.h
--- a/ponyc_amd/csrc/step_tu.h
+++ b/ponyc_amd/csrc/step_tu.h
@@ -24,6 +24,10 @@
 #endif
 
 namespace {
+template <int HT> constexpr uint64_t step_plan_arg()
+{
+  if constexpr(HT >= 0 && two_pass<HT>()) return plan_const_arg<HT>(); else return 0;
+}
 hipError_t step_upload(const void* types, const void* eng, hipStream_t s)
 {
   const hipError_t e = hipMemcpyToSymbolAsync(HIP_SYMBOL(c_types), types,
@@ -35,14 +39,16 @@
 
 #if GPA_STEP_STUB
 StepEntry GPA_STEP_ENTRY() { return { k_step_stub<GPA_STEP_HT>, step_upload, true, (uint32_t)kZoneBits,
-                                      (uint32_t)kZoneThreads, kSortWork, 4u, false, nullptr, nullptr, nullptr }; }
+                                      (uint32_t)kZoneThreads, kSortWork, 4u, false, nullptr, nullptr, nullptr, false, 0 }; }
 #else
 StepEntry GPA_STEP_ENTRY() { return { k_step<GPA_STEP_HT, 0>, step_upload, false, (uint32_t)kZoneBits,
                                       (uint32_t)kZoneThreads, kSortWork,
                                       dp_table<GPA_STEP_HT>() ? 6u : 4u,
                                       GPA_STEP_HT < 0 || GPA_STEP_HT == kHtFifoPair,
                                       split_kernel<GPA_STEP_HT, 1>(), split_kernel<GPA_STEP_HT, 2>(),
-                                      split_kernel<GPA_STEP_HT, 3>() }; }
+                                      split_kernel<GPA_STEP_HT, 3>(),
+                                      GPA_STEP_HT >= 0 && two_pass<GPA_STEP_HT>(),
+                                      step_plan_arg<GPA_STEP_HT>() }; }
 #endif
 
 }
diff --git a/ponyc_amd/csrc/zone_dev.h b/ponyc_amd/csrc/zone_dev.h
--- a/ponyc_amd/csrc/zone_dev.h
+++ b/ponyc_amd/csrc/zone_dev.h
@@ -194,6 +194,10 @@
 __device__ __forceinline__ void st16(uint4* p, const uint4& v)
 {
   p->x = v.x; p->y = v.y; p->z = v.z; p->w = v.w;
+}
+__device__ __forceinline__ void st8(uint2* p, const uint2& v)
+{
+  *reinterpret_cast<uint64_t*>(p) = ((uint64_t)v.y << 32) | v.x;
 }
 __device__ __forceinline__ uint4 ld16(const uint4* p)
 {
@@ -954,19 +958,31 @@
 }
 
 constexpr uint32_t kDirect = 0x80000000u;
+constexpr uint32_t kCompact = 0x40000000u;
+template <bool C8 = false>
 __device__ __forceinline__ uint32_t chunk_dst(uint32_t b, uint32_t base, uint32_t h, uint32_t nz)
 {
   if(b < nz)
   {
     const uint64_t o = c_eng.zoff[b] + base;
-    if(base + h <= c_eng.zcapz[b] && o + h <= 0x7FFFFFFFull) return (uint32_t)o | kDirect;
+    if(base + h <= c_eng.zcapz[b] && o + h <= (C8 ? 0x3FFFFFFFull : 0x7FFFFFFFull))
+      return (uint32_t)o | kDirect;
   }
   return base;
 }
 
+template <bool C8 = false>
 __device__ __forceinline__ uint32_t emit_at(const uint4& r, uint32_t b, uint32_t d, uint32_t rel,
   uint32_t L0, uint32_t nz, uint32_t nxt)
 {
+  if constexpr(C8)
+    if((d & (kDirect | kCompact)) == (kDirect | kCompact))
+    {
+      st8(c_eng.landc[nxt] + ((d & ~(kDirect | kCompact)) + rel),
+          make_uint2((r.y & ~kZoneMask) | (rdiv(r.x) & kZoneMask),
+                     (L0 + (r.y & kZoneMask)) * c_eng.nranks + c_eng.rank));
+      return 0;
+    }
   if(d & kDirect)
   {
     uint4 v;
@@ -1013,11 +1029,12 @@
     if(idx < tcap)
       tile[idx] = r;
     else
-      xover += emit_at(tile_rec16(r, kArg), b, bs[b], idx - ((st[b] >> sh) & 0xFFFFu), L0, nz, nxt);
+      xover += emit_at<sizeof(Rec) == sizeof(uint2)>(tile_rec16(r, kArg), b, bs[b],
+                 idx - ((st[b] >> sh) & 0xFFFFu), L0, nz, nxt);
   }
 };
 
-template <int NW>
+template <int NW, bool C8 = false>
 __device__ __forceinline__ uint32_t plan_reserve(const uint32_t* rh, uint32_t* bs, uint32_t nb,
   uint32_t nz, uint32_t nxt, uint32_t tid)
 {
@@ -1036,11 +1053,29 @@
     {
       ++n_atom;
       if(b < nz)
-        base = atomicAdd(&c_eng.land_n[nxt][b], h);
+      {
+        if constexpr(C8)
+          if(c_eng.land8)
+          {
+            const unsigned long long o = atomicAdd(&c_eng.landc_n[nxt][b], (unsigned long long)h);
+            const uint32_t bc = (uint32_t)o, capb = c_eng.zcapz[b];
+            const uint64_t off = c_eng.zoff[b] + bc;
+            if((uint64_t)bc + h <= capb && off + h <= 0x3FFFFFFFull)
+            {
+              if((uint64_t)bc + h + (o >> 32) > capb) atomicOr(c_eng.lc_over, 1u << nxt);
+              bs[b] = (uint32_t)off | kDirect | kCompact;
+              continue;
+            }
+            atomicOr(c_eng.lc_over, 1u << nxt);
+            for(uint32_t q = bc; q < capb && q - bc < h; ++q)
+              c_eng.landc[nxt][c_eng.zoff[b] + q] = make_uint2(kLand8Hole, 0u);
+          }
+        base = land_reserve(nxt, b, h);
+      }
       else
         base = (uint32_t)atomicAdd(&c_eng.xcount[b - nz], (unsigned long long)h);
     }
-    bs[b] = chunk_dst(b, base, h, nz);
+    bs[b] = chunk_dst<C8>(b, base, h, nz);
   }
   return n_atom;
 }
@@ -1111,7 +1146,8 @@
       if(q < m)
       {
         const uint32_t b = bucket_of(rec[u].x);
-        xover += emit_at(tile_rec16(rec[u], kArg), b, bsr[b], q - ((rst[b] >> sh) & 0xFFFFu), L0, nz, nxt);
+        xover += emit_at<sizeof(Rec) == sizeof(uint2)>(tile_rec16(rec[u], kArg), b, bsr[b],
+                   q - ((rst[b] >> sh) & 0xFFFFu), L0, nz, nxt);
       }
     }
   }
@@ -1210,8 +1246,7 @@
   bool dp = false;
   if constexpr(PM == 2)
     if(__builtin_amdgcn_readfirstlane(c_eng.zplan[z]) == sidx + 1u) return false;
-  const bool halt_now = c_eng.nranks == 1 ? (c_eng.spill_n[cur] != 0u || *c_eng.halt != 0u)
-                                          : (*c_eng.spill_flag != 0u);
+  const bool halt_now = c_eng.nranks == 1 ? step_halted(cur) : (*c_eng.spill_flag != 0u);
   if(halt_now)
   {
     if(PM != 1 && z == 0 && tid == 0)
@@ -1267,7 +1302,27 @@
   GPA_STAMP(0);
 
   const uint32_t nc = min(rfl(c_eng.carry_n[cur][z]), cap);
-  const uint32_t nl = min(rfl(c_eng.land_n[cur][z]), cap);
+  constexpr bool kL8 = HTS >= 0 && two_pass<HTS>();
+  const uint32_t nl16 = min(rfl(c_eng.land_n[cur][z]), cap);
+  uint32_t nlc = 0;
+  if constexpr(kL8)
+    if(c_eng.land8) nlc = min(rfl((uint32_t)c_eng.landc_n[cur][z]), cap - nl16);
+  const uint32_t nl = nl16 + nlc;
+  auto expand8 = [&]() __attribute__((always_inline)) {
+    if constexpr(kL8)
+    {
+      const uint2* const Lc = c_eng.landc[cur] + zo;
+      uint4* const Lx = reinterpret_cast<uint4*>(c_eng.land[cur] + zo + nl16);
+      constexpr uint64_t kA = plan_const_arg<kL8 ? HTS : GPU_ACTOR_HT_PINGER>();
+      for(uint32_t i = tid; i < nlc; i += kZoneThreads)
+      {
+        const uint2 r = Lc[i];
+        st16(Lx + i, make_uint4(r.x, r.y, (uint32_t)kA, (uint32_t)(kA >> 32)));
+      }
+      __syncthreads();
+    }
+  };
+  if constexpr(PM == 2) { if(nlc) expand8(); }
   if(nc + nl == 0 && ztc == 0)
   {
     if constexpr(PM == 1) return false;
@@ -1289,6 +1344,7 @@
       reinterpret_cast<uint32_t*>(s_tb)[i] = 0;
   const ZRec* C = c_eng.carry[cur] + zo;
   const ZRec* Ld = c_eng.land[cur] + zo;
+  const uint2* const Lc8 = kL8 && c_eng.land8 ? c_eng.landc[cur] + zo : nullptr;
   const bool use_idx = kSimple || nc + nl <= kIdxCap;
   constexpr bool kHotTables = !kSimple && (HTS < 0 || HTS == kHtFifoPair);
   const bool hot = kHotTables && c_eng.hot_on &&
@@ -1395,7 +1451,10 @@
     for(int u = 0; u < kIdxPer; ++u)
     {
       const uint32_t i = u * kZoneThreads + tid;
-      wr[u] = i < nl ? Ld[i].w0 : 0xFFFFFFFFu;
+      if constexpr(kL8 && PM != 2)
+        wr[u] = i < nl16 ? Ld[i].w0 : i < nl ? Lc8[i - nl16].x : 0xFFFFFFFFu;
+      else
+        wr[u] = i < nl ? Ld[i].w0 : 0xFFFFFFFFu;
     }
 #pragma unroll
     for(int u = 0; u < kIdxPer; ++u)
@@ -1419,7 +1478,10 @@
     for(int u = 0; u < kUnroll; ++u)
     {
       const uint32_t i = base + u * kZoneThreads + tid;
-      w[u] = i < nl ? Ld[i].w0 : 0xFFFFFFFFu;
+      if constexpr(kL8 && PM != 2)
+        w[u] = i < nl16 ? Ld[i].w0 : i < nl ? Lc8[i - nl16].x : 0xFFFFFFFFu;
+      else
+        w[u] = i < nl ? Ld[i].w0 : 0xFFFFFFFFu;
     }
 #pragma unroll
     for(int u = 0; u < kUnroll; ++u)
@@ -1463,6 +1525,7 @@
       if constexpr(two_pass<HTS>())
         plan = PM != 2 && fast && s_tot < c_eng.seq_max && c_eng.two_pass != 0u;
     }
+  if constexpr(PM == 0 && kL8) { if(!plan && nlc) expand8(); }
   if constexpr(PM == 1)
   {
     if constexpr(kPlanSplit)
@@ -1721,7 +1784,7 @@
       }
       lds_sync();
       GPA_STAMP(3);
-      n_atom += plan_reserve<1>(s_rh, s_bs, nb, nz, nxt, tid);
+      n_atom += plan_reserve<1, true>(s_rh, s_bs, nb, nz, nxt, tid);
       GPA_STAMP(5);
 #ifdef GPA_STAMPS
       const unsigned long long t_scan = __builtin_amdgcn_s_memtime();
@@ -2229,7 +2292,7 @@
     if(h)
     {
       ++n_atom;
-      const uint32_t base = b < nz ? atomicAdd(&c_eng.land_n[nxt][b], h)
+      const uint32_t base = b < nz ? land_reserve(nxt, b, h)
                                    : (uint32_t)atomicAdd(&c_eng.xcount[b - nz], (unsigned long long)h);
       s_base[b] = chunk_dst(b, base, h, nz);
     }
@@ -2321,8 +2384,10 @@
     if(nc + nl) pend_add_z(pend_slot, z, (unsigned long long)(nc + nl));
     c_eng.carry_n[cur][z] = 0;
     c_eng.land_n[cur][z] = 0;
+    if constexpr(kL8) { if(c_eng.land8) c_eng.landc_n[cur][z] = 0ull; }
     if constexpr(PM == 1) c_eng.zplan[z] = sidx + 1u;
   }
+  if constexpr(kL8) { if(took_mail && nlc && tid == 7) stat_add_z(ST_LAND8, z, (unsigned long long)nlc); }
 #ifdef GPA_STAMPS
   if(tid == 0) c_eng.dbg[z * kDbgSlots + 12] = __builtin_amdgcn_s_memrealtime();
 #endif
@@ -2358,7 +2423,9 @@
   if(z < c_eng.n_zones)
   {
     const uint32_t cap = zone_capacity(z);
-    p = min(c_eng.carry_n[cur][z], cap) + min(c_eng.land_n[cur][z], cap);
+    const uint32_t nl16 = min(c_eng.land_n[cur][z], cap);
+    p = min(c_eng.carry_n[cur][z], cap) + nl16;
+    if(c_eng.land8) p += min((uint32_t)c_eng.landc_n[cur][z], cap - nl16);
   }
   p = wave_sum(p);
   if(__lane_id() == 0) s_red[threadIdx.x >> 6] = p;
@@ -2399,7 +2466,7 @@
     }
   __syncthreads();
   for(uint32_t b = threadIdx.x; b < nz; b += kLandThreads)
-    if(s_hist[b]) s_base[b] = atomicAdd(&c_eng.land_n[cur][b], s_hist[b]);
+    if(s_hist[b]) s_base[b] = land_reserve(cur, b, s_hist[b]);
   __syncthreads();
 #pragma unroll
   for(int u = 0; u < kLandPer; ++u)
diff --git a/ponyc_amd/engine.py b/ponyc_amd/engine.py
--- a/ponyc_amd/engine.py
+++ b/ponyc_amd/engine.py
@@ -385,7 +385,8 @@
         keys = ["fixups", "sparse_launches", "sparse_steps", "zone_records", "spill_cap", "zones",
                 "trig_n0", "trig_n1", "trig_n2", "zone_bits", "hot_missed", "hot_on", "jit",
                 "jit_builds", "gups_updates", "gups_atomics", "peer_write",
-                "gups_chunks_in", "gups_chunks_out", "gups_remote"]
+                "gups_chunks_in", "gups_chunks_out", "gups_remote", "plan_zones",
+                "land8_records"]
         out = (ctypes.c_uint64 * len(keys))()
         fn = self.lib.gpu_actor_debug_info
         fn.argtypes = [ctypes.c_void_p, ctypes.c_uint64]
```
